# timflannagan/deppy

Hardware: AMD Instinct MI355X
Metric: resolutions/sec (node) on synthetic catalogs at 1/2/4/8 GPUs; BCP HBM GB/s (higher is better)
Workload: dtype int32

## Files before the change

deppy_amd/_lib.py:

```python
from __future__ import annotations

import ctypes
import os

import numpy as np

HERE = os.path.dirname(os.path.abspath(__file__))
LIB_PATH = os.path.join(HERE, "libdeppy_hip.so")
def _hsa_up() -> bool:
    try:
        fds = os.listdir("/proc/self/fd")
    except OSError:
        return False
    for fd in fds:
        try:
            if os.readlink("/proc/self/fd/" + fd) == "/dev/kfd":
                return True
        except OSError:
            pass
    return False


def hw_queue_plan(env_value, hsa_up: bool, keep: bool = False):
    try:
        q = int(env_value) if env_value not in (None, "") else 4
    except ValueError:
        q = 4
    if hsa_up or keep or q >= 8:
        return None, q
    return "8", 8


def _plan_hw_queues() -> None:
    up = _hsa_up()
    env = os.environ.get("GPU_MAX_HW_QUEUES")
    set_to, q = hw_queue_plan(env, up, os.environ.get("DEPPY_KEEP_HW_QUEUES") == "1")
    if set_to is not None:
        os.environ["GPU_MAX_HW_QUEUES"] = set_to
    elif up and q < 8:
        import warnings
        warnings.warn("deppy_amd: HIP was initialised before the binding was imported, with %d hardware "
                      "queues; the pipeline runs %d lane streams per device (import deppy_amd first for 8)"
                      % (q, q), RuntimeWarning, stacklevel=3)
    os.environ["DEPPY_HW_QUEUES"] = "%d@%s" % (q, os.environ.get("GPU_MAX_HW_QUEUES", ""))


_plan_hw_queues()
OPT_FORCE_GROUP = 1 << 0
OPT_FORCE_HBM = 1 << 1
OPT_FORCE_MID = 1 << 2
OPT_TINY_TABLE = 1 << 3
OPT_FORCE_LDSG = 1 << 4
OPT_SHARE_ORDINAL = 1 << 5
F_TRACE_TRUNCATED = 1 << 8
if os.environ.get("DEPPY_STAMPS") == "1":
    LIB_PATH = os.path.join(HERE, os.environ.get("DEPPY_STAMPS_LIB", "libdeppy_hip_stamps.so"))
elif os.environ.get("DEPPY_VARIANT_LIB"):
    LIB_PATH = os.path.join(HERE, os.environ["DEPPY_VARIANT_LIB"])

c_i32p = ctypes.POINTER(ctypes.c_int32)
c_i64p = ctypes.POINTER(ctypes.c_int64)
c_u32p = ctypes.POINTER(ctypes.c_uint32)
c_i8p = ctypes.POINTER(ctypes.c_int8)

EXPORTS = [
    "dp_rec_validate", "dp_lower", "dp_lowered_free", "dp_lowered_num_problems",
    "dp_lowered_rec_off", "dp_lowered_rec", "dp_lowered_ident_off", "dp_lowered_ident_var",
    "dp_lowered_ident_con", "dp_lowered_error", "dp_result_layout", "dp_create", "dp_destroy",
    "dp_last_error", "dp_last_global_error", "dp_num_devices", "dp_lanes", "dp_solve", "dp_upload", "dp_run",
    "dp_launch", "dp_wait", "dp_download", "dp_resident_free", "dp_last_kernel_ms", "dp_gen_catalogs", "dp_gen_wire",
    "dp_gen_free", "dp_upload_traced", "dp_download_trace", "dp_solve_traced", "dp_lowered_errors",
    "dp_device_bytes", "dp_lower_into", "dp_lowered_new", "dp_lowered_exact_count", "dp_lowered_pinned", "dp_rec_widen", "dp_submit", "dp_job_wait", "dp_get_stats", "dp_stage_roundtrip",
    "dp_stitch_selftest", "dp_partition", "dp_build_info", "dp_get_device_stats", "dp_plan_placements",
    "dp_plan_order", "dp_dlower_new", "dp_dlower_free", "dp_lower_device", "dp_dlower_host_count",
    "dp_host_alloc", "dp_host_free",
]


class Wire(ctypes.Structure):
    _fields_ = [
        ("n_problems", ctypes.c_int32),
        ("prob_var_off", c_i64p),
        ("var_id", c_i64p),
        ("var_con_off", c_i64p),
        ("con_kind", c_i32p),
        ("con_n", c_i32p),
        ("con_arg_off", c_i64p),
        ("con_arg", c_i64p),
        ("n_strs", ctypes.c_int64),
        ("str_off", c_i64p),
        ("str_bytes", ctypes.c_char_p),
        ("interned", ctypes.c_int32),
    ]


class Wire32(ctypes.Structure):
    _fields_ = [
        ("n_problems", ctypes.c_int32),
        ("prob_var_off", c_i32p),
        ("prob_con_off", c_i32p),
        ("prob_arg_off", c_i32p),
        ("var_id", c_i32p),
        ("var_ncon", ctypes.POINTER(ctypes.c_uint16)),
        ("con_kn", c_i32p),
        ("con_nargs", ctypes.POINTER(ctypes.c_uint16)),
        ("con_arg", c_i32p),
        ("var_id16", ctypes.POINTER(ctypes.c_uint16)),
        ("con_arg16", ctypes.POINTER(ctypes.c_uint16)),
        ("n_strs", ctypes.c_int64),
        ("str_off", c_i64p),
        ("str_bytes", ctypes.c_char_p),
    ]


class Opts(ctypes.Structure):
    _fields_ = [("first_device", ctypes.c_int32), ("n_devices", ctypes.c_int32),
                ("step_budget", ctypes.c_int64), ("flags", ctypes.c_int32)]


class Stats(ctypes.Structure):
    _fields_ = [("problems", ctypes.c_int64), ("chunks", ctypes.c_int64), ("launches", ctypes.c_int64),
                ("kernel_ms", ctypes.c_double), ("h2d_bytes", ctypes.c_int64), ("d2h_bytes", ctypes.c_int64),
                ("rec_bytes", ctypes.c_int64), ("stage_ms", ctypes.c_double), ("plan_ms", ctypes.c_double), ("wait_ms", ctypes.c_double),
                ("scatter_ms", ctypes.c_double), ("direct_chunks", ctypes.c_int64),
                ("bcp_bytes", ctypes.c_int64), ("allocs", ctypes.c_int64),
                ("placed", ctypes.c_int64 * 5), ("placed_launches", ctypes.c_int64 * 5)]

PLACES = ["lds", "split", "hbm", "split4", "ldsg"]


def _stats_dict(st) -> dict:
    d = {}
    for k, _ in Stats._fields_:
        v = getattr(st, k)
        d[k] = {PLACES[m]: int(v[m]) for m in range(5)} if k.startswith("placed") else v
    return d


class Batch(ctypes.Structure):
    _fields_ = [("n_problems", ctypes.c_int32), ("rec_off", c_i64p), ("rec", c_i32p)]


class Result(ctypes.Structure):
    _fields_ = [("status", c_i8p), ("flags", c_i32p), ("installed", c_u32p),
                ("inst_off", c_i64p), ("core", c_i32p), ("core_off", c_i64p),
                ("core_len", c_i32p), ("steps", c_i64p)]


_lib = None


def build_info(L=None) -> str:
    L = L or lib()
    if not hasattr(L, "dp_build_info"):
        return ""
    L.dp_build_info.restype = ctypes.c_char_p
# ... 12 lines not shown
    got = build_info(L)
    if ("sources=%s " % want) not in got + " ":
        raise RuntimeError("deppy_amd: %s was built from other sources (%s; this tree: sources=%s); run "
                           "__graft_entry__.build() (python -m deppy_amd.build)" % (LIB_PATH, got or "no build info", want))


def lib():
    global _lib
    if _lib is not None:
        return _lib
    if not os.path.exists(LIB_PATH):
        raise RuntimeError("deppy_amd: %s is missing; run __graft_entry__.build() "
                           "(python deppy_amd/build.py)" % LIB_PATH)
    L = ctypes.CDLL(LIB_PATH)
    _check_provenance(L)
    vp = ctypes.c_void_p
    L.dp_rec_validate.argtypes = [c_i32p, ctypes.c_int64]
    L.dp_rec_widen.argtypes = [c_i32p, ctypes.c_int64, c_i32p]
    L.dp_lower.argtypes = [ctypes.POINTER(Wire), ctypes.POINTER(vp)]
    L.dp_lowered_free.argtypes = [vp]
    L.dp_lower_into.argtypes = [ctypes.POINTER(Wire), ctypes.c_int32, vp]
    L.dp_lowered_new.restype = vp
    L.dp_lowered_exact_count.argtypes = [vp]
    L.dp_lowered_exact_count.restype = ctypes.c_int64
    L.dp_lowered_pinned.argtypes = [vp]
    L.dp_lowered_pinned.restype = ctypes.c_int32
    L.dp_lowered_num_problems.argtypes = [vp]
    for f in ("dp_lowered_rec_off", "dp_lowered_ident_off"):
        getattr(L, f).argtypes = [vp]
        getattr(L, f).restype = c_i64p
    for f in ("dp_lowered_rec", "dp_lowered_ident_var", "dp_lowered_ident_con"):
        getattr(L, f).argtypes = [vp]
        getattr(L, f).restype = c_i32p
    L.dp_lowered_error.argtypes = [vp, ctypes.c_int32, ctypes.POINTER(ctypes.c_char_p)]
    L.dp_lowered_errors.argtypes = [vp, c_i32p]
    L.dp_result_layout.argtypes = [ctypes.POINTER(Batch), c_i64p, c_i64p]
    L.dp_create.argtypes = [ctypes.POINTER(Opts)]
    L.dp_create.restype = vp
    L.dp_destroy.argtypes = [vp]
    L.dp_last_error.argtypes = [vp]
    L.dp_last_error.restype = ctypes.c_char_p
    L.dp_last_global_error.restype = ctypes.c_char_p
    L.dp_num_devices.argtypes = [vp]
    if hasattr(L, "dp_lanes"):
        L.dp_lanes.argtypes = [vp]
        L.dp_lanes.restype = ctypes.c_int32
    L.dp_solve.argtypes = [vp, ctypes.POINTER(Batch), ctypes.POINTER(Result)]
    L.dp_upload.argtypes = [vp, ctypes.POINTER(Batch), ctypes.POINTER(vp)]
    L.dp_upload_traced.argtypes = [vp, ctypes.POINTER(Batch), ctypes.c_int32, ctypes.POINTER(vp)]
    L.dp_download_trace.argtypes = [vp, vp, c_i32p, c_i32p]
    L.dp_solve_traced.argtypes = [vp, ctypes.POINTER(Batch), ctypes.c_int32, ctypes.POINTER(Result),
                                  c_i32p, c_i32p]
    L.dp_submit.argtypes = [vp, ctypes.POINTER(Batch), ctypes.POINTER(Result), ctypes.POINTER(vp)]
    L.dp_job_wait.argtypes = [vp, vp]
    L.dp_get_stats.argtypes = [vp, ctypes.POINTER(Stats), ctypes.c_int32]
    L.dp_get_device_stats.argtypes = [vp, ctypes.c_int32, ctypes.POINTER(Stats), ctypes.c_int32]
    L.dp_num_devices.restype = ctypes.c_int32
    L.dp_stage_roundtrip.argtypes = [ctypes.POINTER(Batch), ctypes.c_int32, ctypes.c_int32, ctypes.c_int64,
                                     c_i32p, c_i32p, ctypes.c_int32]
    L.dp_stitch_selftest.argtypes = [ctypes.POINTER(Batch), ctypes.c_int32, ctypes.POINTER(Result)]
    L.dp_partition.argtypes = [c_i64p, ctypes.c_int32, ctypes.c_int32, c_i32p]
    L.dp_run.argtypes = [vp, vp]
    L.dp_launch.argtypes = [vp, vp]
    L.dp_wait.argtypes = [vp, vp]
    L.dp_download.argtypes = [vp, vp, ctypes.POINTER(Result)]
    L.dp_resident_free.argtypes = [vp, vp]
    L.dp_last_kernel_ms.argtypes = [vp, ctypes.POINTER(ctypes.c_double)]
    L.dp_gen_catalogs.argtypes = [ctypes.c_int32, ctypes.c_int32, ctypes.c_uint64]
    L.dp_gen_catalogs.restype = vp
    L.dp_gen_wire.argtypes = [vp]
    L.dp_gen_wire.restype = ctypes.POINTER(Wire)
    L.dp_gen_free.argtypes = [vp]
    L.dp_device_bytes.argtypes = [ctypes.POINTER(Batch), ctypes.c_int32, c_i64p, c_i64p]
    L.dp_dlower_new.argtypes = [vp]
    L.dp_dlower_new.restype = vp
    L.dp_dlower_free.argtypes = [vp]
    L.dp_lower_device.argtypes = [vp, ctypes.POINTER(Wire32), ctypes.c_int32, vp]
    L.dp_dlower_host_count.argtypes = [vp]
    L.dp_dlower_host_count.restype = ctypes.c_int64
    L.dp_host_alloc.argtypes = [ctypes.c_int64]
    L.dp_host_alloc.restype = vp
    L.dp_host_free.argtypes = [vp]
    L.dp_plan_placements.argtypes = [ctypes.POINTER(Batch), ctypes.c_int32, c_i8p]
    L.dp_plan_order.argtypes = [ctypes.POINTER(Batch), ctypes.c_int32, c_i32p, c_i32p]
    _lib = L
    return L


def _p(a, t):
    return a.ctypes.data_as(t)


class WireArrays:

    def __init__(self, prob_var_off, var_id, var_con_off, con_kind, con_n, con_arg_off, con_arg,
                 str_off, str_bytes, interned=True):
        self.a = dict(prob_var_off=np.ascontiguousarray(prob_var_off, np.int64),
                      var_id=np.ascontiguousarray(var_id, np.int64),
                      var_con_off=np.ascontiguousarray(var_con_off, np.int64),
                      con_kind=np.ascontiguousarray(con_kind, np.int32),
                      con_n=np.ascontiguousarray(con_n, np.int32),
                      con_arg_off=np.ascontiguousarray(con_arg_off, np.int64),
                      con_arg=np.ascontiguousarray(con_arg, np.int64),
                      str_off=np.ascontiguousarray(str_off, np.int64),
                      str_bytes=np.frombuffer(bytes(str_bytes) + b"\0", np.uint8))
        self.interned = interned

    @property
    def n_problems(self) -> int:
        return len(self.a["prob_var_off"]) - 1

    def slice(self, p0: int, p1: int) -> "WireArrays":
        w = WireArrays.__new__(WireArrays)
        w.a = dict(self.a)
        w.a["prob_var_off"] = self.a["prob_var_off"][p0:p1 + 1]
        w.interned = self.interned
        return w

    def struct(self) -> Wire:
        a = self.a
        for k in ("var_id", "con_kind", "con_n", "con_arg"):
            if len(a[k]) == 0:
                a[k] = np.zeros(1, a[k].dtype)
        w = Wire()
        w.n_problems = len(a["prob_var_off"]) - 1
        w.prob_var_off = _p(a["prob_var_off"], c_i64p)
        w.var_id = _p(a["var_id"], c_i64p)
        w.var_con_off = _p(a["var_con_off"], c_i64p)
        w.con_kind = _p(a["con_kind"], c_i32p)
        w.con_n = _p(a["con_n"], c_i32p)
        w.con_arg_off = _p(a["con_arg_off"], c_i64p)
        w.con_arg = _p(a["con_arg"], c_i64p)
        w.n_strs = len(a["str_off"]) - 1
        w.str_off = _p(a["str_off"], c_i64p)
        w.str_bytes = ctypes.cast(a["str_bytes"].ctypes.data, ctypes.c_char_p)
        w.interned = 1 if self.interned else 0
        return w


def wire_to_numpy(w: Wire) -> dict:
    P = w.n_problems
    pvo = np.ctypeslib.as_array(w.prob_var_off, (P + 1,)).copy()
    nv = int(pvo[-1])
    vco = np.ctypeslib.as_array(w.var_con_off, (nv + 1,)).copy() if nv else np.zeros(1, np.int64)
    nc = int(vco[-1])
    cao = np.ctypeslib.as_array(w.con_arg_off, (nc + 1,)).copy() if nc else np.zeros(1, np.int64)
    na = int(cao[-1])
    so = np.ctypeslib.as_array(w.str_off, (w.n_strs + 1,)).copy()
    sb = ctypes.string_at(w.str_bytes, int(so[-1]))
    return dict(prob_var_off=pvo,
                var_id=np.ctypeslib.as_array(w.var_id, (nv,)).copy() if nv else np.zeros(0, np.int64),
                var_con_off=vco,
                con_kind=np.ctypeslib.as_array(w.con_kind, (nc,)).copy() if nc else np.zeros(0, np.int32),
                con_n=np.ctypeslib.as_array(w.con_n, (nc,)).copy() if nc else np.zeros(0, np.int32),
                con_arg_off=cao,
                con_arg=np.ctypeslib.as_array(w.con_arg, (na,)).copy() if na else np.zeros(0, np.int64),
                str_off=so, str_bytes=np.frombuffer(sb, np.uint8))


class _LoweredHandle:

    def __init__(self, h):
        self.h = h

    def __del__(self):
        try:
# ... 340 lines not shown
            raise RuntimeError("dp_job_wait: job already waited")
        rc = lib().dp_job_wait(self.ctx.h, h)
        self._batch_arrays = None
        if rc != 0:
            raise RuntimeError("dp_job_wait: " + self.ctx.error())
        out = dict(self.out)
        for k in ("status", "flags", "core_len", "steps"):
            out[k] = out[k][:self.n]
        return out


class Resident:

    def __init__(self, ctx: Context, rec_off, rec, trace_cap: int = 0):
        self.ctx = ctx
        self.trace_cap = trace_cap
        self.rec_off = np.ascontiguousarray(rec_off, np.int64)
        self.rec = np.ascontiguousarray(rec if len(rec) else np.zeros(1, np.int32), np.int32)
        n = len(self.rec_off) - 1
        self.n = n
        b = _batch(self.rec_off, self.rec)
        self.inst_off = np.zeros(n + 1, np.int64)
        self.core_off = np.zeros(n + 1, np.int64)
        lib().dp_result_layout(ctypes.byref(b), _p(self.inst_off, c_i64p), _p(self.core_off, c_i64p))
        h = ctypes.c_void_p()
        if lib().dp_upload_traced(ctx.h, ctypes.byref(b), trace_cap, ctypes.byref(h)) != 0:
            raise RuntimeError("dp_upload: " + ctx.error())
        self.h = h

    def run(self):
        if lib().dp_run(self.ctx.h, self.h) != 0:
            raise RuntimeError("dp_run: " + self.ctx.error())

    def launch(self):
        if lib().dp_launch(self.ctx.h, self.h) != 0:
            raise RuntimeError("dp_launch: " + self.ctx.error())

    def wait(self):
        if lib().dp_wait(self.ctx.h, self.h) != 0:
            raise RuntimeError("dp_wait: " + self.ctx.error())

    def download(self) -> dict:
        n = self.n
        out = result_arrays(self.rec_off, self.rec)
        r = _result_struct(out)
        if lib().dp_download(self.ctx.h, self.h, ctypes.byref(r)) != 0:
            raise RuntimeError("dp_download: " + self.ctx.error())
        for k in ("status", "flags", "core_len", "steps"):
            out[k] = out[k][:n]
        return out

    def download_trace(self) -> dict:
        n = self.n
        tr = np.zeros((max(n, 1), max(self.trace_cap, 1)), np.int32)
        tl = np.zeros(max(n, 1), np.int32)
        if lib().dp_download_trace(self.ctx.h, self.h, _p(tr, c_i32p), _p(tl, c_i32p)) != 0:
            raise RuntimeError("dp_download_trace: " + self.ctx.error())
        return dict(trace=tr[:n], trace_len=tl[:n])

    def free(self):
        if self.h:
            lib().dp_resident_free(self.ctx.h, self.h)
            self.h = None


def device_bytes(rec_off, rec, flags: int = 0) -> tuple[int, int]:
    rec_off = np.ascontiguousarray(rec_off, np.int64)
    rec = np.ascontiguousarray(rec if len(rec) else np.zeros(1, np.int32), np.int32)
    rb, ib = ctypes.c_int64(), ctypes.c_int64()
    if lib().dp_device_bytes(ctypes.byref(_batch(rec_off, rec)), flags, ctypes.byref(rb), ctypes.byref(ib)) != 0:
        raise RuntimeError("dp_device_bytes failed")
    return rb.value, ib.value


def plan_placements(rec_off, rec, flags: int = 0) -> np.ndarray:
    rec_off = np.ascontiguousarray(rec_off, np.int64)
    rec = np.ascontiguousarray(rec if len(rec) else np.zeros(1, np.int32), np.int32)
    place = np.zeros(max(len(rec_off) - 1, 1), np.int8)
    if lib().dp_plan_placements(ctypes.byref(_batch(rec_off, rec)), flags, _p(place, c_i8p)) != 0:
        raise RuntimeError("dp_plan_placements failed")
    return place[:len(rec_off) - 1]


def plan_order(rec_off, rec, flags: int = 0):
    rec_off = np.ascontiguousarray(rec_off, np.int64)
    rec = np.ascontiguousarray(rec if len(rec) else np.zeros(1, np.int32), np.int32)
    order = np.zeros(max(len(rec_off) - 1, 1), np.int32)
    first = np.zeros(32, np.int32)
    nl = lib().dp_plan_order(ctypes.byref(_batch(rec_off, rec)), flags, _p(order, c_i32p), _p(first, c_i32p))
    if nl < 0:
        raise RuntimeError("dp_plan_order failed")
    return order, first[:nl]


def stage_roundtrip(rec_off, rec, flags: int = 0, chunk_problems: int = 0, chunk_bytes: int = 0):
    rec_off = np.ascontiguousarray(rec_off, np.int64)
    rec = np.ascontiguousarray(rec if len(rec) else np.zeros(1, np.int32), np.int32)
    out = np.zeros_like(rec)
    firsts = np.zeros(max(len(rec_off), 1), np.int32)
    k = lib().dp_stage_roundtrip(ctypes.byref(_batch(rec_off, rec)), flags, chunk_problems, chunk_bytes,
                                 _p(out, c_i32p), _p(firsts, c_i32p), len(firsts))
    if k < 0:
        raise ValueError("dp_stage_roundtrip: malformed record")
    return out, firsts[:k]


def stitch_selftest(rec_off, rec, chunk_problems: int) -> dict:
    rec_off = np.ascontiguousarray(rec_off, np.int64)
    rec = np.ascontiguousarray(rec, np.int32)
    out = result_arrays(rec_off, rec)
    out["installed"][:] = 0xdeadbeef
    r = _result_struct(out)
    if lib().dp_stitch_selftest(ctypes.byref(_batch(rec_off, rec)), chunk_problems, ctypes.byref(r)) < 0:
        raise ValueError("dp_stitch_selftest failed")
    return out


def partition(rec_off, nd: int) -> np.ndarray:
    rec_off = np.ascontiguousarray(rec_off, np.int64)
    cut = np.zeros(nd + 1, np.int32)
    if lib().dp_partition(_p(rec_off, c_i64p), len(rec_off) - 1, nd, _p(cut, c_i32p)) != 0:
        raise ValueError("dp_partition failed")
    return cut


def generate(config: int, n: int, seed: int) -> dict:
    L = lib()
    g = L.dp_gen_catalogs(config, n, seed)
    if not g:
        raise ValueError(L.dp_last_global_error().decode())
    try:
        return wire_to_numpy(L.dp_gen_wire(g).contents)
    finally:
        L.dp_gen_free(g)


def trace_events(res: dict, p: int) -> list:
    t = res["trace"][p][:int(res["trace_len"][p])]
    ev, i = [], 0
    while i < len(t):
        n = int(t[i])
        vs = [int(x) for x in t[i + 1:i + 1 + n]]
        i += 1 + n
        m = int(t[i])
        ev.append((vs, [int(x) for x in t[i + 1:i + 1 + m]]))
        i += 1 + m
    return ev


def installed_list(res: dict, p: int, nv: int) -> list[int]:
    base = int(res["inst_off"][p])
    words = res["installed"][base:base + (nv + 31) // 32]
    bits = np.unpackbits(words.view(np.uint8), bitorder="little")[:nv]
    return [int(i) for i in np.flatnonzero(bits)]


def core_list(res: dict, p: int) -> list[int]:
    base = int(res["core_off"][p])
    return [int(x) for x in res["core"][base:base + int(res["core_len"][p])]]
```

deppy_amd/csrc/kernel_api.hpp:

```cpp
#pragma once
#include <hip/hip_runtime.h>

#include <cstdint>

namespace dp {

constexpr int DP_NSTAMP = 56;

struct alignas(32) ProblemOut {
  int8_t status;
  int8_t pad[3];
  int32_t flags;
  int32_t core_len;
  int32_t core_at;
  int64_t steps;
  uint64_t bcp;
};
static_assert(sizeof(ProblemOut) == 32, "two 16-byte stores");

struct alignas(16) WorkItem {
  int64_t rec_off;
  int32_t inst_off;
  int32_t pid;
};
static_assert(sizeof(WorkItem) == 16, "one 16-byte read");

struct KernelArgs {
  const int32_t* rec;
  const WorkItem* items;
  ProblemOut* out;
  uint32_t* installed;
  int32_t* core;
  int32_t* core_pool_len;
  int64_t budget;
  int32_t* scratch;
  const int64_t* scratch_off;
  int64_t* stamps;
  int32_t* trace;
  int32_t* trace_len;
  int32_t trace_cap;
  int32_t* queue;
  int32_t n_items;
  int32_t table_cap;
  int32_t grid_cap;
};
constexpr int kQueueWords = 64;

hipError_t launch_solve(const KernelArgs& a, int mode, int n_blocks, int lds_bytes, hipStream_t stream);
hipError_t launch_watch_build(const KernelArgs& a, int mode, int n_items, hipStream_t stream);
hipError_t configure_solve_kernel(int max_lds_bytes);

}
```

deppy_amd/csrc/layout.hpp:

```cpp
#pragma once
#include <hip/hip_runtime.h>

#include <cstdint>
#include <type_traits>

#include "../../include/deppy_hip.h"

namespace dp {

__host__ __device__ inline int32_t bits_words(int32_t n) { return (n + 31) >> 5; }

constexpr int32_t L_MAX = 64;

enum Mode { M_LDS = 0, M_SPLIT = 1, M_HBM = 2, M_SPLIT4 = 3, M_LDSG = 4 };
static_assert((int)M_LDS == DP_PLACE_LDS && (int)M_SPLIT == DP_PLACE_SPLIT && (int)M_HBM == DP_PLACE_HBM &&
                  (int)M_SPLIT4 == DP_PLACE_SPLIT4 && (int)M_LDSG == DP_PLACE_LDSG,
              "enum dp_place (include/deppy_hip.h) names the placements");
__host__ __device__ constexpr bool mode_n16(int mode) { return mode == M_LDS || mode == M_LDSG; }
#ifndef DP_BIG_WAVES
#define DP_BIG_WAVES 8
#endif
constexpr int32_t BIG_WAVES = DP_BIG_WAVES;

#ifndef DP_MID_WAVES
#define DP_MID_WAVES 4
#endif
constexpr int32_t MID_WAVES = DP_MID_WAVES;
#ifndef DP_LDSG_WAVES
#define DP_LDSG_WAVES 4
#endif
constexpr int32_t LDSG_WAVES = DP_LDSG_WAVES;
__host__ __device__ constexpr int32_t mode_waves(int mode) {
  return mode == M_LDS ? 1 : mode == M_SPLIT4 ? MID_WAVES : mode == M_LDSG ? LDSG_WAVES : BIG_WAVES;
}
__host__ __device__ constexpr int32_t mode_wbuf(int mode) {
  return mode == M_LDS ? 128 : mode == M_LDSG ? 1024 : 4096;
}
__host__ __device__ constexpr int32_t mode_cq(int mode) { return mode == M_LDS ? 64 : mode == M_LDSG ? 256 : 512; }

constexpr int32_t NSCAL = 64;
__host__ __device__ constexpr int32_t mode_nscal(int mode) {
#ifdef DP_STAMPS
  return (mode == M_LDS ? 8 : NSCAL) + 64;
#else
  return mode == M_LDS ? 8 : NSCAL;
#endif
}

__host__ __device__ inline bool fmt_derived(int32_t fmt) { return fmt == DP_FMT_P16D || fmt == DP_FMT_P8D; }
__host__ __device__ inline bool fmt_packed(int32_t fmt) { return fmt == DP_FMT_P16 || fmt_derived(fmt); }
__host__ __device__ inline int64_t p16_tail_at(const int32_t* h) {
  const int64_t ch = fmt_derived(h[DP_H_FMT]) ? 0 : h[DP_H_NCHL];
  return (2 * ((int64_t)h[DP_H_NCL] + h[DP_H_NKL] + h[DP_H_NK] + ch + h[DP_H_NA]) + 15) & ~(int64_t)15;
}
__host__ __device__ inline int64_t p16_tail_bytes(const int32_t* h) {
  const int64_t vc = fmt_derived(h[DP_H_FMT]) ? 0 : (int64_t)h[DP_H_NV];
  return (int64_t)h[DP_H_NC] + h[DP_H_NK] + h[DP_H_NCH] + vc + ((int64_t)h[DP_H_NID] + 7) / 8;
}
__host__ __device__ inline int32_t p8_bytes(const int32_t* h) { return (int32_t)((uint32_t)h[DP_H_P8] >> 8); }
__host__ __device__ inline int32_t id_mask_words16(const int32_t* h) {
  return 3 * bits_words(h[DP_H_NID]) + 2;
}
__host__ __device__ inline int32_t lds_body_words(const int32_t* h) {
  int32_t b = h[DP_H_WORDS] - DP_H_SIZE;
  if (fmt_packed(h[DP_H_FMT])) b += id_mask_words16(h) - h[DP_H_NC] - h[DP_H_NK];
  return fmt_derived(h[DP_H_FMT]) ? b - 1 - h[DP_H_NCHL] : b;
}
__host__ __device__ inline int32_t p16_tail_copy(const int32_t* h) {
  return (2 * lds_body_words(h) + 15) & ~15;
}
__host__ __device__ inline int32_t p8_tail(const int32_t* h) {
  return p16_tail_copy(h) + ((p8_bytes(h) + 15) & ~15);
}

__host__ __device__ inline dp_rec_layout rec_layout(const int32_t* h) {
  dp_rec_layout L;
  int32_t o = DP_H_SIZE;
  L.clause_off = o;     o += h[DP_H_NC] + 1;
  L.clause_lits = o;    o += h[DP_H_NCL];
  L.clause_id = o;      o += h[DP_H_NC];
  L.card_off = o;       o += h[DP_H_NK] + 1;
  L.card_lits = o;      o += h[DP_H_NKL];
  L.card_bound = o;     o += h[DP_H_NK];
  L.card_id = o;        o += h[DP_H_NK];
  L.var_choice_off = o; o += h[DP_H_NV] + 1;
  L.choice_off = o;     o += h[DP_H_NCH] + 1;
  L.choice_lits = o;    o += h[DP_H_NCHL];
  L.anchors = o;        o += h[DP_H_NA];
  L.words = o;
  return L;
}


enum { DP_FMT_REJECT = 2, DP_FMT_U16_CHECKED = 16, DP_FMT_I32_CHECKED = 17 };

constexpr int32_t DEV_WATCH_VARS = 2048;
__host__ __device__ inline bool device_watches(const int32_t* h) { return h[DP_H_NV] <= DEV_WATCH_VARS; }
static_assert(2 * DEV_WATCH_VARS + 1 <= mode_wbuf(M_SPLIT) + mode_cq(M_SPLIT) &&
                  2 * DEV_WATCH_VARS + 1 <= mode_wbuf(M_SPLIT4) + mode_cq(M_SPLIT4) &&
                  2 * DEV_WATCH_VARS + 1 <= mode_wbuf(M_HBM) + mode_cq(M_HBM) && mode_wbuf(M_SPLIT) % 4 == 0,
              "build_watches_wide: the counters fit wbuf + cardq");

constexpr uint32_t ROW_INFO_NONE = 0xffffffffu;
__host__ __device__ inline uint32_t row_info(int32_t a, int32_t len) {
  return a >= 0 && a < (1 << 24) && len >= 0 && len < 255 ? ((uint32_t)a << 8) | (uint32_t)len : ROW_INFO_NONE;
}

struct ImgLayout {
  int32_t w_off, w, words;
};

__host__ __device__ inline ImgLayout img_layout(const int32_t* h) {
  ImgLayout X;
  int32_t o = h[DP_H_WORDS];
  X.w_off = o; o += 2 * h[DP_H_NV] + 1;
  X.w = o;     o += h[DP_H_NCL] + h[DP_H_NKL];
  X.words = o;
  return X;
}

__host__ __device__ inline int64_t staged_words(const int32_t* h, bool narrow) {
  const int64_t body = (int64_t)h[DP_H_WORDS] - DP_H_SIZE;
  const int64_t w = narrow ? DP_H_SIZE + (body + 1) / 2 : (int64_t)img_layout(h).words;
  return (w + 3) & ~3LL;
}

struct Layout {
  int32_t body;
  int32_t val;
  int32_t reason;
  int32_t rs;
  int32_t trail;
  int32_t touched;
  int32_t d_mark;
  int32_t imp;
  int32_t d_flip;
  int32_t inS;
  int32_t extra;
  int32_t seen;
  int32_t model;
  int32_t dset;
  int32_t fg;
  int32_t used;
  int32_t en;
  int32_t en2;
  int32_t crit;
  int32_t idt;
  int32_t l_off;
  int32_t l_lits;
  int32_t dq;
  int32_t stk;
  int32_t wbuf;
  int32_t cardq;
  int32_t scal;
  int32_t hkey;
  int32_t hrp, hrn;
  int32_t tl;
  int32_t fr;
  int32_t hc;
  int32_t wl;
  int32_t bytes;
  int32_t lds_bytes;
  int32_t cap, lcap;
};

enum Scalar { S_NTOUCHED = 0, S_NWORK = 1, S_POSROWS = 2, S_APP = 3, S_NTB = 4, S_CVB = 6, S_OVB = 8, S_SLOT = 32 };

__host__ __device__ constexpr bool mode_lds_rounds(int mode) { return mode == M_SPLIT || mode == M_SPLIT4; }
__host__ __device__ inline int32_t round_slots(int32_t nv) {
  int32_t c = 64;
  while (c < 1024 && c < nv / 8) c <<= 1;
  return c;
}

template <int MODE>
__host__ __device__ inline Layout layout_hc(const int32_t* h, int32_t hc) {
  constexpr bool N16 = mode_n16(MODE);
  using IX = typename std::conditional<N16, uint16_t, int32_t>::type;
  Layout L;
  const int32_t nv = h[DP_H_NV], nid = h[DP_H_NID];
  const int32_t nbv = bits_words(nv), nbi = bits_words(nid);
  const int32_t ix = (int32_t)sizeof(IX);
  int32_t og = 0, ol = 0;
  auto take = [&](int32_t nbytes, int kind) {
    const bool lds = N16 || kind == 2 || (kind == 1 && (MODE == M_SPLIT || MODE == M_SPLIT4));
    int32_t& o = lds ? ol : og;
    const int32_t at = o;
    o += (nbytes + 15) & ~15;
    return at;
  };
  enum { COLD = 0, HOT = 1, WORK = 2 };
  L.cap = h[DP_H_NA] + h[DP_H_NCH] + 2;
  L.lcap = nv + 64;
  const ImgLayout X = img_layout(h);
  int32_t body_bytes = (X.words - DP_H_SIZE + 8) * ix;
  if (N16) body_bytes = (lds_body_words(h) + (X.words - h[DP_H_WORDS]) + 8) * ix;
  if (N16 && fmt_packed(h[DP_H_FMT])) {
    const int32_t tail = h[DP_H_FMT] == DP_FMT_P8D ? p8_tail(h) : p16_tail_copy(h);
    const int32_t need = tail + (int32_t)((p16_tail_bytes(h) + 15) & ~15);
    body_bytes = body_bytes > need ? body_bytes : need;
  }
  L.body = N16 ? take(body_bytes, COLD) : 0;
  L.scal = take(mode_nscal(MODE) * 4, WORK);
  L.wbuf = take(mode_wbuf(MODE) * ix, WORK);
  L.cardq = take(mode_cq(MODE) * ix * (N16 ? 1 : 2), WORK);
  L.hc = mode_lds_rounds(MODE) ? hc : 0;
  L.hkey = take(L.hc * 4, WORK);
  L.hrp = take(L.hc * 4, WORK);
  L.hrn = take(L.hc * 4, WORK);
  L.tl = take(L.hc * 4, WORK);
  L.fr = take(L.hc * 4, WORK);
  L.val = take(nv, HOT);
  L.d_flip = take(nbv * 4, HOT);
  L.inS = take(nbv * 4, HOT);
  L.extra = take(nbv * 4, HOT);
  L.seen = take(nbv * 4, HOT);
  L.model = take(nbv * 4, HOT);
  L.dset = take(nbv * 4, HOT);
  L.fg = take(nbv * 4, HOT);
  L.used = take(nbi * 4, HOT);
  L.en = take(nbi * 4, HOT);
  L.en2 = take(nbi * 4, HOT);
  L.crit = take(nbi * 4, HOT);
  L.idt = N16 ? take(nbi * 4, HOT) : 0;
  L.reason = take(nv * ix, COLD);
  L.rs = take(nv * ix, COLD);
  L.trail = take(nv * ix, COLD);
  L.touched = take(2 * nv * ix, COLD);
  L.d_mark = take(nv * ix, COLD);
  L.imp = take(2 * nv * (N16 ? 2 : 4), COLD);
  L.l_off = take((L_MAX + 1) * ix, COLD);
  L.l_lits = take(L.lcap * ix, COLD);
  L.dq = take(2 * L.cap * ix, COLD);
  L.stk = take(3 * L.cap * ix, COLD);
  L.wl = !N16 && h[DP_H_FMT] == DP_FMT_I32 ? take((2 * nv + 2) * 4 + (h[DP_H_NCL] + h[DP_H_NKL]) * 8, COLD) : 0;
  L.bytes = og;
  L.lds_bytes = ol;
  return L;
}

constexpr int32_t kLdsLimitBytes = 160 * 1024;
template <int MODE>
__host__ __device__ inline Layout layout(const int32_t* h) {
  if (!mode_lds_rounds(MODE)) return layout_hc<MODE>(h, 0);
  int32_t hc = round_slots(h[DP_H_NV]);
  Layout L = layout_hc<MODE>(h, hc);
  while (hc > 64 && L.lds_bytes > kLdsLimitBytes) L = layout_hc<MODE>(h, hc >>= 1);
  return L;
}

inline bool fits16(const int32_t* h) { return dp_rec_fits16(h) != 0; }

}
```

deppy_amd/csrc/lower_device.hip:

```cpp
#include <hip/hip_runtime.h>

#include <algorithm>
#include <chrono>
#include <cstdio>
#include <cstdlib>
#include <cstring>
#include <mutex>
#include <string>
#include <vector>

#include "common.hpp"
#include "dlower.hpp"
#include "hostmem.hpp"
#include "layout.hpp"
#include "placement.hpp"
#include "pool.hpp"

namespace {

constexpr int DL_NV = 512;
constexpr int DL_C = 512;
constexpr int DL_A = 1536;
constexpr int DL_VH = 1024;
constexpr int DL_KH = 1024;
// ... 354 lines not shown
    const int crow = nc + __popcll(__ballot(isc) & lt_mask());
    const int cat = ncl + excl_scan(isc ? rlen : 0, tot);
    nc += __popcll(__ballot(isc));
    ncl += tot;
    const int krow = nk + __popcll(__ballot(isk) & lt_mask());
    const int kat = nkl + excl_scan(isk ? rlen : 0, tot);
    nk += __popcll(__ballot(isk));
    nkl += tot;
    const bool isl = act && m_list(m);
    const int k = nch + __popcll(__ballot(isl) & lt_mask());
    if (isl) S.clist[c] = (int16_t)k;
    nch += __popcll(__ballot(isl));
    (void)excl_scan(isl ? ns : 0, tot);
    nchl += tot;
    __syncthreads();
    bool far = false;
    if (isl) {
      const int d = isf || s < 0 ? 0 : k - S.clist[first];
      far = d > 255;
      S.src[k] = (uint8_t)d;
    }
    if (__ballot(far) && lane == 0) S.p16 = 1;
    if (isc) {
      S.clen[crow] = (uint8_t)rlen;
      if (kind == DP_DEPENDENCY && ns > 0) {
        S.clit[cat] = (int16_t)(2 * vi + 1);
        for (int j = 0, o = 1; j < ns; ++j) {
          const int d = S.ca[a0 + j];
          bool rep = false;
          for (int q = 0; q < j && !rep; ++q) rep = S.ca[a0 + q] == d;
          if (!rep) S.clit[cat + o++] = (int16_t)(2 * d);
        }
      } else if (rlen == 1) {
        const uint64_t key = S.kkey[s] - 1ull;
        S.clit[cat] = (int16_t)(2 * (int)(key & 0x3fffffffULL) + ((key >> 60) == K_NEG ? 1 : 0));
      } else if (rlen == 2) {
        S.clit[cat] = (int16_t)(2 * vi + 1);
        S.clit[cat + 1] = (int16_t)(2 * S.ca[a0] + 1);
      }
    }
    bool kb1 = true;
    if (isk) {
      const int n = a.ckn[cb + c] >> 3;
      S.klen[krow] = (uint8_t)rlen;
      S.kb[krow] = (int16_t)n;
      kb1 = n == 1;
      for (int j = 0; j < ns; ++j) S.kv[kat + j] = S.ca[a0 + j];
      atomicOr(&S.mask[id >> 5], 1u << (id & 31));
    }
    b1 = b1 && __ballot(!kb1) == 0;
    nib = nib && __ballot((isc || isk) && rlen > 15) == 0;
    if (isf) {
      const int last = S.klast[s];
      const int ov = S.cs[last];
      a.ivs[(int64_t)p * DL_C + id] = ov;
      a.ics[(int64_t)p * DL_C + id] = last - S.vstart[ov];
    }
  }
  __syncthreads();
  if (S.fb) return give_up();
  int na = 0;
  for (int i0 = 0; i0 < nv; i0 += DL_T) {
    const int i = i0 + lane;
    const bool f = i < nv && ((S.aflag[i >> 5] >> (i & 31)) & 1u);
    const uint64_t bm = __ballot(f);
    if (f) S.av[na + __popcll(bm & lt_mask())] = (int16_t)i;
    na += __popcll(bm);
  }

  int32_t h[DP_H_SIZE];
#pragma unroll
  for (int i = 0; i < DP_H_SIZE; ++i) h[i] = 0;
  h[DP_H_MAGIC] = DP_REC_MAGIC;
  h[DP_H_NV] = nv;
  h[DP_H_NC] = nc;
  h[DP_H_NK] = nk;
  h[DP_H_NCH] = nch;
  h[DP_H_NA] = na;
  h[DP_H_NID] = nid;
  h[DP_H_NCL] = ncl;
  h[DP_H_NKL] = nkl;
  h[DP_H_NCHL] = nchl;
  h[DP_H_WORDS] = DP_H_SIZE + (nc + 1) + ncl + nc + (nk + 1) + nkl + 2 * nk + (nv + 1) + (nch + 1) + nchl + na;
  if (!fits16_dev(h) || (int64_t)dp::layout<dp::M_LDS>(h).lds_bytes > a.group_above) return give_up();
  auto put_header = [&]() {
    for (int i = lane; i < DL_SLOT; i += DL_T) S.rec[i] = 0u;
    __syncthreads();
    if (lane < DP_H_SIZE) {
      int32_t x = 0;
#pragma unroll
      for (int i = 0; i < DP_H_SIZE; ++i)
        if (i == lane) x = h[i];
      S.rec[lane] = (uint32_t)x;
    }
  };
  auto put_out = [&](int padded) {
    __syncthreads();
    int32_t* out = a.slots + (int64_t)p * DL_SLOT;
    for (int i = lane; i < padded; i += DL_T) out[i] = (int32_t)S.rec[i];
    if (lane == 0) {
      a.words[p] = padded;
      a.nid[p] = nid;
    }
  };
  if (S.p16) {
    bool bad16 = false;
    for (int i = lane; i < nv; i += DL_T) {
      int cnt = 0;
      for (int c = S.vstart[i]; c < S.vstart[i + 1]; ++c) cnt += m_list(S.cmeta[c]) ? 1 : 0;
      bad16 = bad16 || cnt > 255;
      S.vcl[i] = (uint8_t)cnt;
    }
    const int tb = nc + nk + nv + nch + (nid + 7) / 8;
    const int at = (2 * (ncl + nkl + nk + nchl + na) + 15) & ~15;
    const int phys = DP_H_SIZE + (at + tb + 3) / 4, padded = (phys + 3) & ~3;
    if (__ballot(bad16) || tb > DP_P16_TAIL_MAX || padded > DL_SLOT) return give_up();
    h[DP_H_FMT] = DP_FMT_P16;
    put_header();
    uint16_t* const u = reinterpret_cast<uint16_t*>(S.rec + DP_H_SIZE);
    uint8_t* const t = reinterpret_cast<uint8_t*>(S.rec + DP_H_SIZE) + at;
    for (int j = lane; j < ncl; j += DL_T) u[j] = (uint16_t)S.clit[j];
    for (int j = lane; j < nkl; j += DL_T) u[ncl + j] = (uint16_t)S.kv[j];
    for (int j = lane; j < nk; j += DL_T) u[ncl + nkl + j] = (uint16_t)S.kb[j];
    int run = 0;
    for (int c0 = 0; c0 < C; c0 += DL_T) {
      const int c = c0 + lane;
      const bool isl = c < C && m_list(S.cmeta[c]);
      const int ns = isl ? S.castart[c + 1] - S.castart[c] : 0;
      int tot;
      const int ex = excl_scan(ns, tot);
      if (isl) {
        for (int j = 0; j < ns; ++j) u[ncl + nkl + nk + run + ex + j] = (uint16_t)S.ca[S.castart[c] + j];
        t[nc + nk + nv + S.clist[c]] = (uint8_t)ns;
      }
      run += tot;
    }
    for (int j = lane; j < na; j += DL_T) u[ncl + nkl + nk + nchl + j] = (uint16_t)S.av[j];
    for (int i = lane; i < nc; i += DL_T) t[i] = S.clen[i];
    for (int i = lane; i < nk; i += DL_T) t[nc + i] = S.klen[i];
    for (int i = lane; i < nv; i += DL_T) t[nc + nk + i] = S.vcl[i];
    for (int b = lane; b < ((nid + 7) >> 3); b += DL_T)
      t[nc + nk + nv + nch + b] = (uint8_t)(S.mask[b >> 2] >> ((b & 3) * 8));
    put_out(padded);
    return;
  }
  if ((int64_t)nc + nk + nch + (nid + 7) / 8 > DP_P16_TAIL_MAX) return give_up();
  const int f = (nv > 256 ? DP_P8_HI : 0) | (b1 ? DP_P8_B1 : 0) | (nib ? DP_P8_NIB : 0);
  const bool hi = f & DP_P8_HI;
  int o = 0;
  const int L_cvar = o; o += ncl;
  const int L_kvar = o; o += nkl;
  const int L_avar = o; o += na;
  const int L_bound = o; o += b1 ? 0 : nk;
  const int L_neg = o; o += (ncl + 7) >> 3;
  const int L_chi = o; o += hi ? (ncl + 7) >> 3 : 0;
  const int L_khi = o; o += hi ? (nkl + 7) >> 3 : 0;
  const int L_ahi = o; o += hi ? (na + 7) >> 3 : 0;
  const int rows = nc + nk;
  const int L_lens = o; o += nib ? (rows + 1) / 2 : rows;
  const int L_srcnz = o; o += (nch + 7) >> 3;
  const int L_srcval = o;
  int nnz = 0;
  for (int k0 = 0; k0 < nch; k0 += DL_T) nnz += __popcll(__ballot(k0 + lane < nch && S.src[k0 + lane] != 0));
  const int L_mask = L_srcval + nnz;
  const int bytes = L_mask + ((nid + 7) >> 3);
  const int phys = DP_H_SIZE + (bytes + 3) / 4, padded = (phys + 3) & ~3;
  if (padded > DL_SLOT) return give_up();
// ... 517 lines not shown
```

deppy_amd/csrc/placement.hpp:

```cpp
#pragma once
#include <algorithm>
#include <cstdint>
#include <cstdlib>
#include <vector>

#include "layout.hpp"

namespace dp {

constexpr int kMaxLdsBytes = kLdsLimitBytes;

constexpr int64_t kGroupAbove = 64 << 10;

inline int64_t group_above() {
  static const int64_t v = [] {
    const char* e = std::getenv("DEPPY_GROUP_ABOVE");
    const int64_t x = e && *e ? std::atoll(e) : 0;
    return x > 0 ? std::min<int64_t>(x, kMaxLdsBytes) : kGroupAbove;
  }();
  return v;
}

inline bool one_wave(const int32_t* h) {
  return fits16(h) && (int64_t)layout<M_LDS>(h).lds_bytes <= group_above();
}

constexpr int32_t kLdsgMaxProblems = 256;
enum { LDSG_NEVER = 0, LDSG_ALWAYS = 1, LDSG_AUTO = 2 };
inline int ldsg_env() {
  const char* e = std::getenv("DEPPY_LDSG");
  return e && *e == '0' ? LDSG_NEVER : e && *e == '1' ? LDSG_ALWAYS : LDSG_AUTO;
}
inline bool ldsg_fits(const int32_t* h) { return fits16(h) && (int64_t)layout<M_LDSG>(h).lds_bytes <= kMaxLdsBytes; }
inline bool lds_image(const int32_t* h, int ldsg) { return one_wave(h) || (ldsg == LDSG_ALWAYS && ldsg_fits(h)); }

inline int64_t build_watches_host(int32_t* r) {
  const dp_rec_layout R = dp_rec_layout_of(r);
  const ImgLayout X = img_layout(r);
  const int32_t nv = r[DP_H_NV], nc = r[DP_H_NC], nk = r[DP_H_NK];
  const int32_t* clause_off = r + R.clause_off;
  const int32_t* clause_lits = r + R.clause_lits;
  const int32_t* card_off = r + R.card_off;
  const int32_t* card_lits = r + R.card_lits;
  int32_t* wo = r + X.w_off;
  int32_t* w = r + X.w;
  std::fill(wo, wo + 2 * (int64_t)nv + 1, 0);
  for (int32_t j = 0; j < r[DP_H_NCL]; ++j) wo[(clause_lits[j] ^ 1) + 1]++;
  for (int32_t k = 0; k < nk; ++k)
    for (int32_t j = card_off[k]; j < card_off[k + 1]; ++j)
      if (j == card_off[k] || card_lits[j] != card_lits[j - 1]) wo[2 * card_lits[j] + 1]++;
  for (int64_t l = 0; l < 2 * (int64_t)nv; ++l) wo[l + 1] += wo[l];
  static thread_local std::vector<int32_t> cur;
  cur.assign(wo, wo + 2 * (int64_t)nv);
  for (int32_t rr = 0; rr < nc; ++rr)
    for (int32_t j = clause_off[rr]; j < clause_off[rr + 1]; ++j) w[cur[(size_t)(clause_lits[j] ^ 1)]++] = rr;
  for (int32_t k = 0; k < nk; ++k)
    for (int32_t j = card_off[k]; j < card_off[k + 1]; ++j)
      if (j == card_off[k] || card_lits[j] != card_lits[j - 1]) w[cur[(size_t)(2 * card_lits[j])]++] = nc + k;
  return X.words;
}

}
```

deppy_amd/csrc/runtime.cpp:

```cpp
#include <hip/hip_runtime.h>

#include <algorithm>
#include <atomic>
#include <chrono>
#include <climits>
#include <condition_variable>
#include <deque>
#include <cstdlib>
#include <cstring>
#include <fstream>
#include <functional>
#include <mutex>
#include <string>
#include <thread>
#include <vector>

#include "common.hpp"
#include "dlower.hpp"
#include "kernel_api.hpp"
#include "layout.hpp"
#include "hostmem.hpp"
#include "placement.hpp"
#include "pool.hpp"

namespace {

using dp::kMaxLdsBytes;
constexpr int64_t kDefaultBudget = 1 << 16;
constexpr int kNBuckets = 16;
struct Ceilings {
  int c[kNBuckets];
  int n;
};
const Ceilings& ceilings() {
  static const Ceilings t = [] {
    Ceilings x{};
    const char* e = std::getenv("DEPPY_CEILINGS");
    if (!e || std::strcmp(e, "fine") != 0) {
      const int coarse[] = {16 << 10, 32 << 10, 53 << 10, 80 << 10, 160 << 10};
      x.n = 5;
      for (int i = 0; i < 5; ++i) x.c[i] = coarse[i];
    } else {
      x.n = kNBuckets;
      for (int k = kNBuckets; k >= 1; --k) x.c[kNBuckets - k] = (160 * 1024 / k) / 512 * 512;
      x.c[kNBuckets - 1] = 160 * 1024;
    }
    return x;
  }();
  return t;
}
constexpr int kXcds = 8;
constexpr int kStreams = 4;
constexpr int kMaxStreams = 16;
constexpr int kMaxLanes = 2 * kMaxStreams;
constexpr double kMergeRatio = 0.5;
constexpr int32_t kMinLaunch = 512;
constexpr int32_t kMidMaxVars = 8192;
constexpr int32_t kChunkProblems = 65536;
constexpr int64_t kChunkBytes = 1ll << 30;
constexpr int32_t kChunksPerDevice = 3;
constexpr int kCostClasses = 16;
constexpr int32_t kMinSharedChunk = 4096;
constexpr int64_t kCoreWordsPerProblem = 8;

double now_ms() {
  return std::chrono::duration<double, std::milli>(std::chrono::steady_clock::now().time_since_epoch()).count();
}

int64_t env_i64(const char* name, int64_t dflt) {
  const char* e = std::getenv(name);
  return e && *e ? std::atoll(e) : dflt;
}

bool forced_of(int32_t opt_flags) {
  return opt_flags & (DP_OPT_FORCE_GROUP | DP_OPT_FORCE_HBM | DP_OPT_FORCE_MID | DP_OPT_FORCE_LDSG);
}

bool header_ok(const int32_t* h, int64_t avail) {
  if (avail < DP_H_SIZE || h[DP_H_MAGIC] != DP_REC_MAGIC) return false;
  for (int i = DP_H_NV; i <= DP_H_NCHL; ++i)
    if (h[i] < 0 || h[i] > (1 << 28)) return false;
  const int32_t fmt = h[DP_H_FMT];
  if (fmt != DP_FMT_I32 && fmt != DP_FMT_I32W && ((fmt != DP_FMT_U16 && !dp_fmt_packed(fmt)) || !dp_rec_fits16(h)))
    return false;
  if (dp_fmt_packed(fmt) && dp_p16_tail_bytes(h) > DP_P16_TAIL_MAX) return false;
  const int64_t w = dp_rec_layout_of(h).words;
  return w == h[DP_H_WORDS] && dp_rec_phys_words(h) <= avail;
}

}

namespace dp {

struct Launch {
  int first, count, mode, lds;
  bool dev_lists;
};

struct Head {
  int8_t place;
  bool ldsg_ok;
  int8_t bucket;
  bool direct;
  int32_t lds, inst_words, nid;
  int64_t sw, rec_bytes;
  uint8_t cls;
};

constexpr int32_t kPlanBlock = 512;
constexpr int32_t kPlanPoolMin = 32768;
struct PlanBlock {
  int64_t img = 0, inst = 0, core = 0, rbytes = 0, other = 0;
  int32_t ndirect = 0, nother = 0, nok = 0;
  int32_t bcount[kNBuckets] = {}, bmax[kNBuckets] = {};
};

struct Plan {
  int32_t n = 0;
  int32_t n_ldsg = 0;
  std::vector<int64_t> img_off;
  std::vector<uint8_t> narrow;
  std::vector<int32_t> order;
  std::vector<Launch> launches;
  int big_base = 0;
  std::vector<int64_t> scratch_off;
  int64_t scratch_words = 0;
  std::vector<int32_t> skip;
  std::vector<int32_t> skip_flags;
  std::vector<int64_t> inst_off;
  int64_t core_cap = 0;
  int64_t rec_bytes = 0;
  std::vector<int64_t> dev_off;
  int64_t img_words = 0;
  std::vector<uint8_t> direct;
  int32_t n_direct = 0;
  int64_t other_words = 0;
  std::vector<Head> head;
  std::vector<PlanBlock> blk;
  std::vector<int32_t> segcnt;
  std::vector<int64_t> segpos, segxs;
  std::vector<int32_t> big[5], cnt, tmp, grp;
};

void place_ldsg(Head& H, const int32_t* h, bool aligned) {
  H.lds = layout<M_LDSG>(h).lds_bytes;
  H.sw = staged_words(h, true);
  H.rec_bytes = dp_fmt_packed(h[DP_H_FMT]) ? 4 * dp_rec_phys_words(h)
                                           : 4 * DP_H_SIZE + 2 * ((int64_t)h[DP_H_WORDS] - DP_H_SIZE);
  H.place = M_LDSG;
  H.direct = aligned && (h[DP_H_FMT] == DP_FMT_U16 || dp_fmt_packed(h[DP_H_FMT]));
}

void read_head(Head& H, const int32_t* h, int64_t avail, int32_t opt_flags, bool aligned) {
  H = Head{};
  if (!header_ok(h, avail)) { H.place = -1; return; }
  H.inst_words = bits_words(h[DP_H_NV]);
  H.nid = h[DP_H_NID];
  H.cls = (uint8_t)std::min<int32_t>(h[DP_H_NA], kCostClasses - 1);
  bool nar = false;
  if (dp::fits16(h)) {
    if (!forced_of(opt_flags)) {
      H.lds = layout<M_LDS>(h).lds_bytes;
      nar = H.lds <= dp::group_above();
    }
    if (!nar && (!forced_of(opt_flags) || (opt_flags & DP_OPT_FORCE_LDSG)) && dp::ldsg_fits(h)) {
      if (opt_flags & DP_OPT_FORCE_LDSG) {
        place_ldsg(H, h, aligned);
        return;
      }
      H.ldsg_ok = true;
    }
  }
  H.sw = staged_words(h, nar);
  H.rec_bytes = nar ? (dp_fmt_packed(h[DP_H_FMT]) ? 4 * dp_rec_phys_words(h)
                                                 : 4 * DP_H_SIZE + 2 * ((int64_t)h[DP_H_WORDS] - DP_H_SIZE))
                    : 4 * (int64_t)h[DP_H_WORDS];
  if (nar) {
    H.place = M_LDS;
    int k = 0;
    const Ceilings& C = ceilings();
    while (k < C.n - 1 && H.lds > C.c[k]) ++k;
    H.bucket = (int8_t)k;
    H.direct = aligned && (h[DP_H_FMT] == DP_FMT_U16 || dp_fmt_packed(h[DP_H_FMT]));
    return;
  }
  H.direct = aligned && (h[DP_H_FMT] == DP_FMT_I32W || h[DP_H_FMT] == DP_FMT_I32);
  const bool forced = forced_of(opt_flags);
  const bool sized = h[DP_H_NV] < (1 << 24) && h[DP_H_NID] < (1 << 26) && h[DP_H_WORDS] < (1 << 28);
  if (sized && layout<M_SPLIT>(h).lds_bytes <= kMaxLdsBytes && !(opt_flags & DP_OPT_FORCE_HBM))
    H.place = (opt_flags & DP_OPT_FORCE_MID) || (!forced && h[DP_H_NV] < kMidMaxVars) ? M_SPLIT4 : M_SPLIT;
  else if (sized && layout<M_HBM>(h).lds_bytes <= kMaxLdsBytes)
    H.place = M_HBM;
  else
    H.place = -2;
}

void plan_chunk(Plan& P, const int32_t* rec, const int64_t* rec_off, int32_t p0, int32_t n,
                int32_t opt_flags, std::vector<uint8_t>* bad, Pool* pool = nullptr, int32_t ldsg_busy = 0) {
  P.n = n;
  P.n_ldsg = 0;
  P.img_off.resize((size_t)n + 1);
  P.inst_off.resize((size_t)n + 1);
  P.narrow.resize((size_t)n);
  P.direct.resize((size_t)n);
  P.head.resize((size_t)n);
  P.order.clear();
  P.launches.clear();
  P.scratch_off.clear();
  P.skip.clear();
  P.skip_flags.clear();
  P.scratch_words = P.core_cap = P.rec_bytes = P.other_words = 0;
  P.n_direct = 0;
  P.big_base = 0;
  Head* head = P.head.data();
  const int32_t nblk = (n + kPlanBlock - 1) / kPlanBlock;
  P.blk.resize((size_t)std::max(nblk, 1));
  auto over_blocks_if = [&](bool par, const std::function<void(int64_t)>& fn) {
    if (pool && nblk > 1 && par) pool->run(nblk, fn, 1);
    else for (int32_t b = 0; b < nblk; ++b) fn(b);
  };
  const bool wide = n >= kPlanPoolMin;
  auto over_blocks = [&](const std::function<void(int64_t)>& fn) { over_blocks_if(wide, fn); };
  over_blocks_if(n > 256, [&](int64_t b) {
    const int32_t i0 = (int32_t)b * kPlanBlock, i1 = std::min(n, i0 + kPlanBlock);
    int32_t nok = 0;
    for (int32_t i = i0; i < i1; ++i) {
      if (i + 8 < i1) {
        const int32_t* h8 = rec + rec_off[p0 + i + 8];
        __builtin_prefetch(h8);
        __builtin_prefetch(h8 + 15);
      }
      read_head(head[i], rec + rec_off[p0 + i], rec_off[p0 + i + 1] - rec_off[p0 + i], opt_flags,
                (rec_off[p0 + i] & 3) == 0);
      nok += head[i].ldsg_ok;
    }
    P.blk[(size_t)b].nok = nok;
  });
  {
    const int lm = dp::ldsg_env();
    int32_t n_ok = 0;
    for (int32_t b = 0; b < nblk; ++b) n_ok += P.blk[(size_t)b].nok;
    if (n_ok > 0 && (lm == dp::LDSG_ALWAYS || (lm == dp::LDSG_AUTO && n_ok + ldsg_busy <= dp::kLdsgMaxProblems))) {
      for (int32_t i = 0; i < n; ++i)
        if (head[i].ldsg_ok) place_ldsg(head[i], rec + rec_off[p0 + i], (rec_off[p0 + i] & 3) == 0);
      P.n_ldsg = n_ok;
    }
  }
  const bool rec_aligned = ((uintptr_t)rec & 15) == 0;
  over_blocks([&](int64_t b) {
    PlanBlock& B = P.blk[(size_t)b];
    const int32_t nok = B.nok;
    B = PlanBlock{};
    B.nok = nok;
    const int32_t i0 = (int32_t)b * kPlanBlock, i1 = std::min(n, i0 + kPlanBlock);
    for (int32_t i = i0; i < i1; ++i) {
      const Head& H = head[i];
      const bool d = rec_aligned && H.direct;
      B.ndirect += d;
      B.other += d ? 0 : rec_off[p0 + i + 1] - rec_off[p0 + i];
      if (H.place == M_LDS) {
        B.bcount[H.bucket]++;
        B.bmax[H.bucket] = std::max(B.bmax[H.bucket], H.lds);
      } else {
        B.nother++;
      }
      if (H.place != -1) {
        B.img += H.sw;
        B.inst += H.inst_words;
        B.core += H.nid;
        B.rbytes += H.rec_bytes;
      }
    }
  });
  for (auto& v : P.big) v.clear();
  int32_t bcount[kNBuckets] = {}, bmax[kNBuckets] = {};
  int64_t img = 0, inst = 0;
  bool others = false;
  for (int32_t b = 0; b < nblk; ++b) {
    PlanBlock& B = P.blk[(size_t)b];
    const int64_t bi = B.img, bn = B.inst;
    B.img = img;
    B.inst = inst;
    img += bi;
    inst += bn;
    P.n_direct += B.ndirect;
    P.other_words += B.other;
    P.core_cap += B.core;
    P.rec_bytes += B.rbytes;
    others |= B.nother > 0;
    for (int k = 0; k < kNBuckets; ++k) {
      bcount[k] += B.bcount[k];
      bmax[k] = std::max(bmax[k], B.bmax[k]);
    }
  }
  P.dev_off.resize((size_t)n);
  P.img_off[0] = P.inst_off[0] = 0;
  over_blocks([&](int64_t b) {
    const PlanBlock& B = P.blk[(size_t)b];
    int64_t im = B.img, in = B.inst;
    const int32_t i0 = (int32_t)b * kPlanBlock, i1 = std::min(n, i0 + kPlanBlock);
    for (int32_t i = i0; i < i1; ++i) {
      const Head& H = head[i];
      P.direct[(size_t)i] = rec_aligned && H.direct;
      P.narrow[(size_t)i] = H.place == M_LDS || H.place == M_LDSG;
      P.dev_off[(size_t)i] = im;
      if (H.place != -1) {
        im += H.sw;
        in += H.inst_words;
      }
      P.img_off[(size_t)i + 1] = im;
      P.inst_off[(size_t)i + 1] = in;
    }
  });
  if (others)
    for (int32_t i = 0; i < n; ++i) {
      const Head& H = head[i];
      if (H.place == M_LDS) continue;
      if (H.place >= 0) {
        P.big[(size_t)H.place].push_back(i);
      } else {
        if (H.place == -1 && bad) (*bad)[(size_t)i] = 1;
        P.skip.push_back(i);
        P.skip_flags.push_back(H.place == -1 ? DP_F_MALFORMED : DP_F_TOO_LARGE);
      }
    }
  P.img_words = img;
  auto cost = [&](int32_t i) { return P.img_off[(size_t)i + 1] - P.img_off[(size_t)i]; };
  auto lpt = [&](int32_t* v, size_t m) {
    if (m < 2) return;
    int64_t lo = INT64_MAX, hi = 0;
    for (size_t j = 0; j < m; ++j) { lo = std::min(lo, cost(v[j])); hi = std::max(hi, cost(v[j])); }
    if (hi - lo > 4 * (int64_t)m + 65536) {
      std::stable_sort(v, v + m, [&](int32_t x, int32_t y) { return cost(x) > cost(y); });
      return;
    }
    P.cnt.assign((size_t)(hi - lo) + 2, 0);
    for (size_t j = 0; j < m; ++j) P.cnt[(size_t)(hi - cost(v[j])) + 1]++;
    for (size_t k = 1; k < P.cnt.size(); ++k) P.cnt[k] += P.cnt[k - 1];
    P.tmp.resize(m);
    for (size_t j = 0; j < m; ++j) P.tmp[(size_t)P.cnt[(size_t)(hi - cost(v[j]))]++] = v[j];
    std::copy(P.tmp.begin(), P.tmp.begin() + (int64_t)m, v);
  };
  for (int mode : {(int)M_LDSG, (int)M_SPLIT4, (int)M_SPLIT, (int)M_HBM}) {
    auto& bg = P.big[(size_t)mode];
    if (bg.empty()) continue;
    lpt(bg.data(), bg.size());
    int mx = 0;
    Launch L{(int)P.order.size(), (int)bg.size(), mode, 0, false};
    for (int32_t i : bg) {
      const int32_t* h = rec + rec_off[p0 + i];
      L.dev_lists |= h[DP_H_FMT] == DP_FMT_I32 && !dp::device_watches(h);
      const Layout Y = mode == M_SPLIT    ? layout<M_SPLIT>(h)
                       : mode == M_SPLIT4 ? layout<M_SPLIT4>(h)
                       : mode == M_LDSG   ? layout<M_LDSG>(h)
                                          : layout<M_HBM>(h);
      mx = std::max(mx, Y.lds_bytes);
      if (P.scratch_words == 0) P.scratch_words = dp::kQueueWords;
      P.scratch_off.push_back(P.scratch_words);
      P.scratch_words += ((int64_t)Y.bytes + 15) / 16 * 4;
    }
    L.lds = mx;
    P.launches.push_back(L);
    P.order.insert(P.order.end(), bg.begin(), bg.end());
  }
  P.big_base = 0;
  static const double merge = [] {
    const char* m = std::getenv("DEPPY_BUCKET_MERGE");
    return m ? std::atof(m) : kMergeRatio;
  }();
  int group_of[kNBuckets];
  Launch bl[kNBuckets];
  int64_t gsize[kNBuckets] = {};
  int ng = 0;
  for (int k = kNBuckets - 1; k >= 0; --k) {
    if (!bcount[k]) continue;
    const bool join = ng > 0 && (bcount[k] < kMinLaunch ||
                                 (merge > 0 && (double)(kMaxLdsBytes / bl[ng - 1].lds) >=
                                                   merge * (double)(kMaxLdsBytes / bmax[k])));
    if (!join) bl[ng++] = Launch{0, 0, M_LDS, bmax[k]};
    group_of[k] = ng - 1;
    gsize[ng - 1] += bcount[k];
  }
  int ix[kNBuckets];
  for (int g = 0; g < ng; ++g) ix[g] = g;
  std::stable_sort(ix, ix + ng, [&](int x, int y) { return gsize[x] > gsize[y]; });
  int64_t o = (int64_t)P.order.size();
  for (int r = 0; r < ng; ++r) {
    const int g = ix[r];
    bl[g].first = (int)o;
    bl[g].count = (int)gsize[g];
    o += gsize[g];
  }
  P.order.resize((size_t)o);
  static const int64_t xcd_order = env_i64("DEPPY_XCD_ORDER", kMaxLdsBytes);
  static const bool anchor_order = env_i64("DEPPY_ANCHOR_ORDER", 1) != 0;
  if (ng > 0) {
    int rank_of[kNBuckets];
    bool xo[kNBuckets];
    for (int r = 0; r < ng; ++r) {
      rank_of[ix[r]] = r;
      xo[ix[r]] = xcd_order && bl[ix[r]].lds <= xcd_order;
    }
    const int nseg = ng * kCostClasses;
    auto seg_of = [&](const Head& H) {
      const int g = group_of[H.bucket];
      const int c = anchor_order && xo[g] ? H.cls : 0;
      return rank_of[g] * kCostClasses + (kCostClasses - 1 - c);
    };
    P.segcnt.assign((size_t)nblk * nseg, 0);
    over_blocks([&](int64_t b) {
      int32_t* c = P.segcnt.data() + (size_t)b * nseg;
      const int32_t i0 = (int32_t)b * kPlanBlock, i1 = std::min(n, i0 + kPlanBlock);
      for (int32_t i = i0; i < i1; ++i)
        if (head[i].place == M_LDS) c[seg_of(head[i])]++;
    });
    P.segpos.resize((size_t)nseg + 1);
    int64_t run = bl[ix[0]].first;
    for (int sg = 0; sg < nseg; ++sg) {
      P.segpos[(size_t)sg] = run;
      for (int32_t b = 0; b < nblk; ++b) {
        int32_t& c = P.segcnt[(size_t)b * nseg + sg];
        const int32_t x = c;
        c = (int32_t)run;
        run += x;
      }
    }
    P.segpos[(size_t)nseg] = run;
    P.tmp.resize((size_t)o);
    over_blocks([&](int64_t b) {
      int32_t* c = P.segcnt.data() + (size_t)b * nseg;
      const int32_t i0 = (int32_t)b * kPlanBlock, i1 = std::min(n, i0 + kPlanBlock);
      for (int32_t i = i0; i < i1; ++i)
        if (head[i].place == M_LDS) P.tmp[(size_t)c[seg_of(head[i])]++] = i;
    });
    P.segxs.resize((size_t)nseg * kXcds);
    auto first_on = [&](int sg, int64_t pos, int x) {
      const int64_t rel = pos - bl[ix[sg / kCostClasses]].first;
      return pos + ((x - rel % kXcds) % kXcds + kXcds) % kXcds;
    };
    for (int sg = 0; sg < nseg; ++sg) {
      const int64_t pos = P.segpos[(size_t)sg], end = P.segpos[(size_t)sg + 1];
      int64_t st = pos;
      for (int x = 0; x < kXcds; ++x) {
        P.segxs[(size_t)sg * kXcds + x] = st;
        const int64_t first = first_on(sg, pos, x);
        st += first < end ? (end - 1 - first) / kXcds + 1 : 0;
      }
    }
    const int64_t o0 = bl[ix[0]].first, nslot = o - o0;
    const int32_t sblk = (int32_t)((nslot + kPlanBlock - 1) / kPlanBlock);
    auto deal = [&](int64_t b) {
      const int64_t s0 = o0 + b * kPlanBlock, s1 = std::min<int64_t>(o, s0 + kPlanBlock);
      int sg = (int)(std::upper_bound(P.segpos.begin(), P.segpos.end(), s0) - P.segpos.begin()) - 1;
      for (int64_t t = s0; t < s1; ++t) {
        while (P.segpos[(size_t)sg + 1] <= t) ++sg;
        const int g = ix[sg / kCostClasses];
        if (!xo[g]) {
          P.order[(size_t)t] = P.tmp[(size_t)t];
          continue;
        }
        const int x = (int)((t - bl[g].first) % kXcds);
        const int64_t first = first_on(sg, P.segpos[(size_t)sg], x);
        P.order[(size_t)t] = P.tmp[(size_t)(P.segxs[(size_t)sg * kXcds + x] + (t - first) / kXcds)];
      }
    };
    if (pool && sblk > 1 && wide) pool->run(sblk, std::function<void(int64_t)>(deal), 1);
    else for (int32_t b = 0; b < sblk; ++b) deal(b);
    for (int r = 0; r < ng; ++r) {
      const int g = ix[r];
      if (!xo[g]) lpt(P.order.data() + bl[g].first, (size_t)bl[g].count);
      P.launches.push_back(bl[g]);
    }
  }
  static const int pad_kb = (int)env_i64("DEPPY_LDS_PAD_KB", 0);
  if (pad_kb > 0)
    for (auto& L : P.launches)
// ... 284 lines not shown
  return a;
}

std::atomic<int64_t> g_buf_allocs{0};

struct Buf {
  char* p = nullptr;
  size_t cap = 0;
  bool host = false;
  hipError_t reserve(size_t n) {
    if (n <= cap) return hipSuccess;
    release();
    n = std::max<size_t>(al(n + n / 8), 4096);
    hipError_t e = host ? hipHostMalloc(reinterpret_cast<void**>(&p), n,
                                        hipHostMallocPortable | hipHostMallocMapped | hipHostMallocCoherent)
                        : hipMalloc(reinterpret_cast<void**>(&p), n);
    if (e != hipSuccess) { p = nullptr; cap = 0; return e; }
    g_buf_allocs.fetch_add(1, std::memory_order_relaxed);
    dev = p;
    if (host && hipHostGetDevicePointer(reinterpret_cast<void**>(&dev), p, 0) != hipSuccess) dev = p;
    cap = n;
    return hipSuccess;
  }
  char* dev = nullptr;
  void release() {
    if (p) (void)(host ? hipHostFree(p) : hipFree(p));
    p = nullptr;
    cap = 0;
  }
};

}

struct dp_job;

constexpr int kMaxSpread = 4;
struct Spread {
  hipStream_t s[kMaxSpread] = {};
  int n = 0;
  hipEvent_t start = nullptr, fin[kMaxSpread] = {};
  int create() {
    if (hipEventCreateWithFlags(&start, hipEventDisableTiming) != hipSuccess) return -1;
    for (auto& e : fin)
      if (hipEventCreateWithFlags(&e, hipEventDisableTiming) != hipSuccess) return -1;
    return 0;
  }
  void destroy() {
    if (start) (void)hipEventDestroy(start);
    for (auto& e : fin)
      if (e) (void)hipEventDestroy(e);
    start = nullptr;
    for (auto& e : fin) e = nullptr;
  }
};

struct Lane {
  int device = 0;
  hipStream_t s = nullptr;
  hipEvent_t k0 = nullptr, k1 = nullptr, done = nullptr;
  hipStream_t cs = nullptr;
  hipEvent_t copied = nullptr;
  Spread spread;
  Buf h_in{nullptr, 0, true}, d_in, h_out{nullptr, 0, true}, d_out, scratch;
  bool zc_out = false;
  dp_job* job = nullptr;
  int32_t p0 = 0;
  dp_job* fjob = nullptr;
  bool scattering = false;
  Plan plan;
  OutLayout ol{};
  std::vector<uint8_t> bad;
};

struct Task {
  dp_job* job;
  int32_t p0, n;
};

struct FastLane {
  std::mutex mu;
  hipStream_t s = nullptr;
  hipEvent_t done = nullptr;
  Buf h_in{nullptr, 0, true}, h_out{nullptr, 0, true};
  Plan plan;
  std::vector<uint8_t> bad;
};
constexpr int32_t kFastProblems = 16;
constexpr int64_t kFastWords = 1 << 16;

struct Device {
  int ordinal = 0;
  Lane lanes[kMaxLanes];
  int nstreams = kStreams, nlanes = 2 * kStreams;
  hipEvent_t last_copied = nullptr;
  int fill_left = 0;
  int next = 0;
  FastLane fast;
  std::thread worker;
  std::mutex qmu;
  std::condition_variable qcv;
  std::deque<Task> q;
  bool stop = false;
  int cursor = 0;
  std::deque<Lane*> inflight;
  dp::Pool* pool = nullptr;
  bool own_pool = false;
  std::thread finisher;
  std::mutex fmu;
  std::condition_variable fcv;
  std::deque<Lane*> fq;
  bool fstop = false;
  dp::Pool* fpool = nullptr;
  std::mutex smu;
  dp_stats st{};
};

struct dp_job {
  int32_t n = 0;
  const int32_t* rec = nullptr;
  const int64_t* rec_off = nullptr;
  bool pinned = false;
  dp_result res{};
  std::mutex m;
  std::condition_variable cv;
  int chunks_left = 0;
  std::atomic<bool> waiting{false};
  int rc = 0;
  std::string err;
};

struct dp_ctx {
  std::deque<Device> dev;
  int64_t budget = kDefaultBudget;
  int32_t flags = 0;
  std::string err;
  std::atomic<double> last_ms{0.0};
  std::mutex mu;
  dp::Pool* pool = nullptr;
  mutable std::mutex err_mu;
  int next_dev = 0;
  bool zc_in = false, zc_out = true;
  bool copy_streams = false;
  bool direct = true;
  int32_t chunk_problems = kChunkProblems;
  int64_t chunk_bytes = kChunkBytes;
  int32_t min_shared_chunk = kMinSharedChunk;
  int32_t grid_cap = 0;
  bool fast_path = true;
  bool spread = false;
  std::mutex sqmu;
  std::deque<Task> sq;
  dp_stats st{};
  ~dp_ctx() { delete pool; }
};

struct Slice {
  int d = 0;
  int ordinal = 0;
  int32_t p0 = 0, p1 = 0;
  Plan plan;
  InLayout il{};
  OutLayout ol{};
  Buf d_in, d_out, scratch;
  int32_t* trace = nullptr;
  int32_t* trace_len = nullptr;
  int64_t* stamps = nullptr;
  hipStream_t stream = nullptr;
  hipEvent_t k0 = nullptr, k1 = nullptr;
  Spread spread;
};

struct dp_resident {
  int32_t n = 0;
  int32_t trace_cap = 0;
  bool inflight = false;
  std::vector<Slice> slices;
};

namespace {

thread_local std::string t_err;
#define HIP_OK(expr)                                                         \
  do {                                                                       \
    hipError_t e_ = (expr);                                                  \
    if (e_ != hipSuccess) {                                                  \
      (void)ctx;                                                             \
      t_err = std::string(#expr) + ": " + hipGetErrorString(e_);             \
      return -1;                                                             \
    }                                                                        \
  } while (0)
void set_err(dp_ctx* ctx, std::string e) {
  std::lock_guard<std::mutex> lk(ctx->err_mu);
  ctx->err = std::move(e);
}
int api_fail(dp_ctx* ctx) {
  set_err(ctx, t_err);
  return -1;
}
#define API_OK(expr)                                                         \
  do {                                                                       \
    if (hipError_t e_ = (expr); e_ != hipSuccess) {                          \
      set_err(ctx, std::string(#expr) + ": " + hipGetErrorString(e_));       \
      return -1;                                                             \
    }                                                                        \
  } while (0)

void add_stats(dp_stats& a, const dp_stats& b) {
  a.problems += b.problems; a.chunks += b.chunks; a.launches += b.launches; a.kernel_ms += b.kernel_ms;
  a.h2d_bytes += b.h2d_bytes; a.d2h_bytes += b.d2h_bytes; a.rec_bytes += b.rec_bytes; a.stage_ms += b.stage_ms;
  a.plan_ms += b.plan_ms; a.wait_ms += b.wait_ms; a.scatter_ms += b.scatter_ms; a.direct_chunks += b.direct_chunks;
  a.bcp_bytes += b.bcp_bytes; a.allocs += b.allocs;
  for (int m = 0; m < 5; ++m) {
    a.placed[m] += b.placed[m];
    a.placed_launches[m] += b.placed_launches[m];
  }
}
void add_device_stats(Device& D, const dp_stats& b) {
  std::lock_guard<std::mutex> lk(D.smu);
  add_stats(D.st, b);
}

int enqueue_launches(dp_ctx* ctx, const Plan& P, const dp::KernelArgs& base, hipStream_t s, dp_stats& st,
                     Spread* sp = nullptr) {
  static const bool no_queue = [] {
    const char* e = std::getenv("DEPPY_NO_QUEUE");
    return e && *e && *e != '0';
  }();
  if (!P.scratch_off.empty()) HIP_OK(hipMemsetAsync(base.scratch, 0, 4 * dp::kQueueWords, s));
  int nlds = 0;
  for (const auto& L : P.launches) nlds += L.mode == dp::M_LDS;
  const bool spread = sp && sp->n > 0 && nlds > 1;
  if (spread) HIP_OK(hipEventRecord(sp->start, s));
  int q = 0, jl = 0, nf = 0;
  for (const auto& L : P.launches) {
    hipStream_t t = s;
    if (spread && L.mode == dp::M_LDS && jl++ > 0 && nf < kMaxSpread) {
      t = sp->s[(jl - 2) % sp->n];
      HIP_OK(hipStreamWaitEvent(t, sp->start, 0));
    }
    dp::KernelArgs a = base;
    a.items = base.items + L.first;
    if (L.mode != dp::M_LDS) {
      a.scratch_off = base.scratch_off + (L.first - P.big_base);
      a.queue = no_queue ? nullptr : base.scratch + q;
      a.n_items = L.count;
      if (ctx->flags & DP_OPT_TINY_TABLE) a.table_cap = 4;
      a.grid_cap = ctx->grid_cap;
      ++q;
      if (L.dev_lists) HIP_OK(dp::launch_watch_build(a, L.mode, L.count, s));
    }
    HIP_OK(dp::launch_solve(a, L.mode, L.count, L.lds, t));
    if (t != s) {
      HIP_OK(hipEventRecord(sp->fin[nf], t));
      HIP_OK(hipStreamWaitEvent(s, sp->fin[nf], 0));
      ++nf;
    }
    st.launches++;
    st.placed[L.mode] += L.count;
    st.placed_launches[L.mode]++;
  }
  return 0;
}

void set_siblings(const Device& D, int i, Spread& sp, bool on) {
  sp.n = 0;
  if (!on) return;
  for (int j = 1; j < D.nstreams && sp.n < kMaxSpread; ++j) sp.s[sp.n++] = D.lanes[(i + j) % D.nstreams].s;
}

int finish_lane(dp_ctx* ctx, Device& D, Lane& L) {
  if (!L.job) return 0;
  dp_job* job = L.job;
  L.job = nullptr;
  dp_stats st{};
  HIP_OK(hipSetDevice(L.device));
  const double t0 = now_ms();
  HIP_OK(hipEventSynchronize(L.done));
  const double t1 = now_ms();
  st.wait_ms += t1 - t0;
  float ms = 0.f;
  if (!L.plan.launches.empty() && hipEventElapsedTime(&ms, L.k0, L.k1) == hipSuccess) {
    st.kernel_ms += ms;
    ctx->last_ms.store(ms);
  }
  const int32_t used = L.zc_out ? 0 : *at<int32_t>(L.h_out.p, L.ol.pool_len);
  const size_t need = L.ol.pool + (size_t)used * 4;
  if (!L.zc_out && need > L.ol.d2h) {
    HIP_OK(hipMemcpyAsync(L.h_out.p + L.ol.d2h, L.d_out.p + L.ol.d2h, need - L.ol.d2h, hipMemcpyDeviceToHost, L.s));
    HIP_OK(hipStreamSynchronize(L.s));
    st.d2h_bytes += (int64_t)(need - L.ol.d2h);
  }
  add_device_stats(D, st);
  {
    std::lock_guard<std::mutex> lk(D.fmu);
    L.fjob = job;
    L.scattering = true;
    D.fq.push_back(&L);
  }
  D.fcv.notify_all();
  return 0;
}

void chunk_done(dp_job* job, int rc);

void wait_scatter(Device& D, Lane& L) {
  std::unique_lock<std::mutex> lk(D.fmu);
  D.fcv.wait(lk, [&] { return !L.scattering; });
}

void finisher_main(dp_ctx* ctx, Device* Dp) {
  Device& D = *Dp;
  std::unique_lock<std::mutex> lk(D.fmu);
  for (;;) {
    if (D.fq.empty()) {
      if (D.fstop) return;
      D.fcv.wait(lk);
      continue;
    }
    Lane* L = D.fq.front();
    D.fq.pop_front();
    lk.unlock();
    dp_stats st{};
    const double t0 = now_ms();
    dp_job* job = L->fjob;
    st.bcp_bytes += (int64_t)scatter(L->plan, L->ol, L->h_out.p, L->p0, &job->res, D.fpool);
    st.scatter_ms += now_ms() - t0;
    add_device_stats(D, st);
    lk.lock();
    L->scattering = false;
    L->fjob = nullptr;
    lk.unlock();
    D.fcv.notify_all();
    chunk_done(job, 0);
    lk.lock();
// ... 209 lines not shown
  bool failed;
  {
    std::lock_guard<std::mutex> lk(job->m);
    failed = job->rc != 0;
  }
  if (failed) {
    chunk_done(job, 0);
    return;
  }
  Lane& L = D.lanes[D.cursor];
  D.cursor = (D.cursor + 1) % D.nlanes;
  deliver(ctx, D, L);
  wait_scatter(D, L);
  if (start_chunk(ctx, D, L, job, t.p0, t.n)) {
    L.job = nullptr;
    chunk_done(job, -1);
    return;
  }
  D.inflight.push_back(&L);
}

bool take_shared(dp_ctx* ctx, Device& D, Task& t) {
  if ((int)D.inflight.size() >= D.nlanes) return false;
  std::lock_guard<std::mutex> g(ctx->sqmu);
  if (ctx->sq.empty()) return false;
  t = ctx->sq.front();
  ctx->sq.pop_front();
  return true;
}

void worker_main(dp_ctx* ctx, Device* Dp) {
  Device& D = *Dp;
  (void)hipSetDevice(D.ordinal);
  std::unique_lock<std::mutex> lk(D.qmu);
  for (;;) {
    Task t;
    if (!D.q.empty()) {
      t = D.q.front();
      D.q.pop_front();
      lk.unlock();
      run_task(ctx, D, t);
      lk.lock();
      continue;
    }
    if (take_shared(ctx, D, t)) {
      lk.unlock();
      run_task(ctx, D, t);
      lk.lock();
      continue;
    }
    if (!D.inflight.empty()) {
      Lane* o = D.inflight.front();
      const bool now = D.stop || o->job->waiting.load(std::memory_order_acquire) ||
                       hipEventQuery(o->done) != hipErrorNotReady;
      if (now) {
        lk.unlock();
        deliver(ctx, D, *o);
        lk.lock();
      } else {
        D.qcv.wait_for(lk, std::chrono::microseconds(50));
      }
      continue;
    }
    if (D.stop) {
      std::lock_guard<std::mutex> g(ctx->sqmu);
      if (ctx->sq.empty()) return;
      continue;
    }
    D.qcv.wait(lk);
  }
}

int fast_solve(dp_ctx* ctx, Device& D, const dp_batch* b, dp_result* res) {
  FastLane& F = D.fast;
  std::lock_guard<std::mutex> lk(F.mu);
  const int32_t n = b->n_problems;
  F.bad.assign((size_t)n, 0);
  dp::plan_chunk(F.plan, b->rec, b->rec_off, 0, n, ctx->flags, &F.bad, nullptr);
  const Plan& P = F.plan;
  if (!P.skip.empty() || !P.scratch_off.empty()) return 1;
  if (hipSetDevice(D.ordinal) != hipSuccess) return 1;
  const InLayout il = in_layout(P);
  const OutLayout ol = out_layout(P);
  if (F.h_in.reserve(il.end) != hipSuccess || F.h_out.reserve(ol.end) != hipSuccess) return 1;
  int32_t* img = at<int32_t>(F.h_in.p, il.img);
  for (int32_t i = 0; i < n; ++i)
    if (!dp::stage_one(P, b->rec, b->rec_off, 0, i, img, true)) F.bad[(size_t)i] = 1;
  fill_in_tables(P, il, F.h_in.p);
  *at<int32_t>(F.h_out.p, ol.pool_len) = 0;
  dp::KernelArgs a = kernel_args(il, ol, F.h_in.dev, F.h_out.dev, nullptr, ctx->budget);
  dp_stats st{};
  if (enqueue_launches(ctx, P, a, F.s, st) || hipEventRecord(F.done, F.s) != hipSuccess) return api_fail(ctx);
  hipError_t e;
  while ((e = hipEventQuery(F.done)) == hipErrorNotReady) __builtin_ia32_pause();
  if (e != hipSuccess) {
    set_err(ctx, std::string("dp_solve (latency path): ") + hipGetErrorString(e));
    return -1;
  }
  scatter(P, ol, F.h_out.p, 0, res);
  return 0;
}

void cut_chunks(const dp_ctx* ctx, const dp_job* job, std::vector<std::pair<int32_t, int32_t>>& out) {
  const int32_t P = job->n;
  const int nd = (int)ctx->dev.size();
  int32_t cp = ctx->chunk_problems;
  if (nd > 1 && P >= nd)
    cp = std::min<int32_t>(cp, std::max<int32_t>((P + kChunksPerDevice * nd - 1) / (kChunksPerDevice * nd),
                                                 std::min<int32_t>(ctx->min_shared_chunk, (P + nd - 1) / nd)));
  for (int32_t p = 0; p < P;) {
    const int32_t q = next_chunk(job->rec_off, p, P, cp, ctx->chunk_bytes);
    out.emplace_back(p, q - p);
    p = q;
  }
}

int lane_streams() {
  int64_t hwq = env_i64("GPU_MAX_HW_QUEUES", kStreams);
  if (const char* e = std::getenv("DEPPY_HW_QUEUES")) {
    const char* at = std::strchr(e, '@');
    const char* g = std::getenv("GPU_MAX_HW_QUEUES");
    if (!at || std::strcmp(at + 1, g ? g : "") == 0) hwq = std::atoll(e);
  }
  return (int)std::min<int64_t>(kMaxStreams,
                                std::max<int64_t>(1, env_i64("DEPPY_STREAMS", std::min<int64_t>(hwq, 8))));
}

}

namespace dp {
int ctx_first_ordinal(const dp_ctx* ctx) { return ctx && !ctx->dev.empty() ? ctx->dev[0].ordinal : -1; }
}

extern "C" {

dp_ctx* dp_create(const dp_opts* opts) {
  int n = 0;
  hipError_t e = hipGetDeviceCount(&n);
  if (e != hipSuccess || n == 0) {
    dp::set_global_error(std::string("dp_create: no HIP device (") + hipGetErrorString(e) + ")");
    return nullptr;
  }
  int first = opts ? opts->first_device : 0;
  int cnt = opts && opts->n_devices > 0 ? opts->n_devices : n - first;
  const bool share = opts && (opts->flags & DP_OPT_SHARE_ORDINAL) && opts->n_devices > 0;
  if (first < 0 || cnt <= 0 || (share ? first >= n || cnt > 8 : first + cnt > n)) {
    dp::set_global_error("dp_create: device range out of bounds");
    return nullptr;
  }
  auto* ctx = new dp_ctx;
  for (int i = 0; i < cnt; ++i) ctx->dev.emplace_back();
  for (int i = 0; i < cnt; ++i) {
    const int d = share ? first : first + i;
    hipDeviceProp_t prop;
    if (hipGetDeviceProperties(&prop, d) != hipSuccess || std::strncmp(prop.gcnArchName, "gfx950", 6) != 0) {
      dp::set_global_error(std::string("dp_create: device ") + std::to_string(d) + " is not gfx950 (" +
                           prop.gcnArchName + ")");
      dp_destroy(ctx);
      return nullptr;
    }
    if (hipSetDevice(d) != hipSuccess || dp::configure_solve_kernel(kMaxLdsBytes) != hipSuccess) {
      dp::set_global_error("dp_create: cannot configure the solve kernel");
      dp_destroy(ctx);
      return nullptr;
    }
    Device& D = ctx->dev[(size_t)i];
    D.ordinal = d;
    ctx->copy_streams = env_i64("DEPPY_COPY_STREAM", 0) != 0;
    D.nstreams = lane_streams();
    D.nlanes = 2 * D.nstreams;
    for (int li = 0; li < D.nlanes; ++li) {
      Lane& L = D.lanes[li];
      L.device = d;
      if (li >= D.nstreams) {
        L.s = D.lanes[li % D.nstreams].s;
        L.cs = D.lanes[li % D.nstreams].cs;
      }
      if ((li < D.nstreams && (hipStreamCreateWithFlags(&L.s, hipStreamNonBlocking) != hipSuccess ||
                             (ctx->copy_streams && hipStreamCreateWithFlags(&L.cs, hipStreamNonBlocking) != hipSuccess))) ||
          hipEventCreateWithFlags(&L.copied, hipEventDisableTiming) != hipSuccess ||
          hipEventCreate(&L.k0) != hipSuccess || hipEventCreate(&L.k1) != hipSuccess ||
          hipEventCreateWithFlags(&L.done, hipEventDisableTiming) != hipSuccess || L.spread.create() != 0) {
        dp::set_global_error("dp_create: cannot create streams");
        dp_destroy(ctx);
        return nullptr;
      }
    }
  }
  if (opts && opts->step_budget > 0) ctx->budget = opts->step_budget;
  if (opts) ctx->flags = opts->flags;
  ctx->chunk_problems = (int32_t)std::max<int64_t>(1, env_i64("DEPPY_CHUNK_PROBLEMS", kChunkProblems));
  ctx->chunk_bytes = std::max<int64_t>(1, env_i64("DEPPY_CHUNK_BYTES", kChunkBytes));
  ctx->min_shared_chunk = (int32_t)std::max<int64_t>(1, env_i64("DEPPY_MIN_SHARED_CHUNK", kMinSharedChunk));
  ctx->zc_in = env_i64("DEPPY_ZC_IN", 0) != 0;
  ctx->zc_out = env_i64("DEPPY_ZC_OUT", 1) != 0;
  ctx->direct = env_i64("DEPPY_DIRECT", 1) != 0;
  ctx->grid_cap = (int32_t)std::max<int64_t>(0, env_i64("DEPPY_GRID_CAP", 0));
  ctx->fast_path = env_i64("DEPPY_FAST_PATH", 1) != 0;
  ctx->spread = env_i64("DEPPY_SPREAD", 0) != 0;
  const int ht = dp::host_threads();
  ctx->pool = new dp::Pool(ht);
  const int per = std::max(2, ht / cnt);
  for (auto& D : ctx->dev) {
    if (hipSetDevice(D.ordinal) != hipSuccess || hipStreamCreateWithFlags(&D.fast.s, hipStreamNonBlocking) != hipSuccess ||
        hipEventCreateWithFlags(&D.fast.done, hipEventDisableTiming) != hipSuccess) {
      dp::set_global_error("dp_create: cannot create the latency stream");
      dp_destroy(ctx);
      return nullptr;
    }
    D.own_pool = cnt > 1;
    D.pool = D.own_pool ? new dp::Pool(per) : ctx->pool;
    D.fpool = new dp::Pool(std::max(2, std::min(4, per / 4)));
    D.worker = std::thread(worker_main, ctx, &D);
    D.finisher = std::thread(finisher_main, ctx, &D);
  }
  return ctx;
}

void dp_destroy(dp_ctx* ctx) {
  if (!ctx) return;
  for (auto& D : ctx->dev) {
    if (!D.worker.joinable()) continue;
    {
      std::lock_guard<std::mutex> lk(D.qmu);
      D.stop = true;
    }
    D.qcv.notify_all();
    D.worker.join();
    if (D.finisher.joinable()) {
      {
        std::lock_guard<std::mutex> lk(D.fmu);
        D.fstop = true;
      }
      D.fcv.notify_all();
      D.finisher.join();
    }
    delete D.fpool;
    D.fpool = nullptr;
    if (D.own_pool) delete D.pool;
    D.pool = nullptr;
  }
  for (auto& D : ctx->dev) {
    (void)hipSetDevice(D.ordinal);
    if (D.fast.s) (void)hipStreamSynchronize(D.fast.s);
    D.fast.h_in.release();
    D.fast.h_out.release();
    if (D.fast.done) (void)hipEventDestroy(D.fast.done);
    if (D.fast.s) (void)hipStreamDestroy(D.fast.s);
  }
  for (auto& D : ctx->dev) {
    (void)hipSetDevice(D.ordinal);
    for (int li = 0; li < D.nstreams; ++li)
      if (D.lanes[li].s) (void)hipStreamSynchronize(D.lanes[li].s);
    for (int li = 0; li < D.nlanes; ++li) {
      Lane& L = D.lanes[li];
      for (Buf* b : {&L.h_in, &L.d_in, &L.h_out, &L.d_out, &L.scratch}) b->release();
      if (L.k0) (void)hipEventDestroy(L.k0);
      if (L.k1) (void)hipEventDestroy(L.k1);
      if (L.done) (void)hipEventDestroy(L.done);
      if (L.copied) (void)hipEventDestroy(L.copied);
      L.spread.destroy();
    }
    for (int li = 0; li < D.nstreams; ++li) {
      if (D.lanes[li].s) (void)hipStreamDestroy(D.lanes[li].s);
      if (D.lanes[li].cs) (void)hipStreamDestroy(D.lanes[li].cs);
    }
  }
  delete ctx;
}

const char* dp_last_error(const dp_ctx* ctx) {
  if (!ctx) return dp_last_global_error();
  static thread_local std::string copy;
  std::lock_guard<std::mutex> lk(ctx->err_mu);
  copy = ctx->err;
  return copy.c_str();
}
int32_t dp_num_devices(const dp_ctx* ctx) { return ctx ? (int32_t)ctx->dev.size() : 0; }
int32_t dp_lanes(const dp_ctx* ctx) { return ctx && !ctx->dev.empty() ? (int32_t)ctx->dev[0].nlanes : 0; }
void* dp_host_alloc(int64_t bytes) { return bytes > 0 ? dp::pinned_alloc((size_t)bytes) : nullptr; }
void dp_host_free(void* p) {
  if (p) dp::pinned_free(p);
}

int dp_result_layout(const dp_batch* b, int64_t* inst_off, int64_t* core_off) {
  if (!b || !inst_off || !core_off || b->n_problems < 0) return -1;
  inst_off[0] = core_off[0] = 0;
  for (int32_t i = 0; i < b->n_problems; ++i) {
    const int32_t* r = b->rec + b->rec_off[i];
    inst_off[i + 1] = inst_off[i] + dp::bits_words(r[DP_H_NV]);
    core_off[i + 1] = core_off[i] + r[DP_H_NID];
  }
  return 0;
}

int dp_device_bytes(const dp_batch* b, int32_t opt_flags, int64_t* rec_bytes, int64_t* img_bytes) {
  if (!b || (b->n_problems > 0 && (!b->rec || !b->rec_off))) return -1;
  Plan P;
  dp::plan_chunk(P, b->rec, b->rec_off, 0, b->n_problems, opt_flags, nullptr);
  if (rec_bytes) *rec_bytes = P.rec_bytes;
  if (img_bytes) *img_bytes = 4 * P.img_words;
  return 0;
}

int dp_plan_order(const dp_batch* b, int32_t opt_flags, int32_t* order, int32_t* launch_first) {
  if (!b || !order || b->n_problems < 0 || (b->n_problems > 0 && (!b->rec || !b->rec_off))) return -1;
  static thread_local Plan P;
  dp::plan_chunk(P, b->rec, b->rec_off, 0, b->n_problems, opt_flags, nullptr, &dp::host_pool());
  std::copy(P.order.begin(), P.order.end(), order);
  if (launch_first)
    for (size_t k = 0; k < P.launches.size(); ++k) launch_first[k] = P.launches[k].first;
  return (int)P.launches.size();
}

int dp_plan_placements(const dp_batch* b, int32_t opt_flags, int8_t* place) {
  if (!b || !place || b->n_problems < 0 || (b->n_problems > 0 && (!b->rec || !b->rec_off))) return -1;
  static thread_local Plan P;
  dp::plan_chunk(P, b->rec, b->rec_off, 0, b->n_problems, opt_flags, nullptr, &dp::host_pool());
  for (int32_t i = 0; i < b->n_problems; ++i) place[i] = (int8_t)P.head[(size_t)i].place;
  return 0;
}


int dp_submit(dp_ctx* ctx, const dp_batch* b, dp_result* res, dp_job** out) {
  if (!ctx || !b || !res || !out || b->n_problems < 0 || (b->n_problems > 0 && (!b->rec || !b->rec_off)))
    return -1;
  auto* job = new dp_job;
  job->n = b->n_problems;
  job->rec = b->rec;
  job->rec_off = b->rec_off;
  job->pinned = ctx->direct && job->n > 0 && pinned_range(b->rec, 4 * (size_t)b->rec_off[job->n]);
  job->res = *res;
  std::vector<std::pair<int32_t, int32_t>> chunks;
  cut_chunks(ctx, job, chunks);
  job->chunks_left = (int)chunks.size();
  const int nd = (int)ctx->dev.size();
  if (nd == 1) {
    Device& D = ctx->dev[0];
    {
      std::lock_guard<std::mutex> lk(D.qmu);
      for (const auto& c : chunks) D.q.push_back(Task{job, c.first, c.second});
    }
    D.qcv.notify_one();
    *out = job;
    return 0;
  }
  std::stable_sort(chunks.begin(), chunks.end(), [&](const auto& x, const auto& y) {
    return b->rec_off[x.first + x.second] - b->rec_off[x.first] > b->rec_off[y.first + y.second] - b->rec_off[y.first];
  });
  {
    std::lock_guard<std::mutex> g(ctx->sqmu);
    for (const auto& c : chunks) ctx->sq.push_back(Task{job, c.first, c.second});
  }
  for (auto& D : ctx->dev) {
    { std::lock_guard<std::mutex> lk(D.qmu); }
    D.qcv.notify_one();
  }
  *out = job;
  return 0;
}

int dp_job_wait(dp_ctx* ctx, dp_job* job) {
  if (!ctx || !job) return -1;
  job->waiting.store(true, std::memory_order_release);
  for (auto& D : ctx->dev) {
    std::lock_guard<std::mutex> lk(D.qmu);
    D.qcv.notify_all();
  }
  int rc;
  {
    std::unique_lock<std::mutex> lk(job->m);
    job->cv.wait(lk, [&] { return job->chunks_left == 0; });
    rc = job->rc;
  }
  if (rc) {
    std::lock_guard<std::mutex> lk(ctx->mu);
    set_err(ctx, job->err);
  }
  delete job;
  return rc;
}

int dp_solve(dp_ctx* ctx, const dp_batch* b, dp_result* res) {
  if (!ctx || !b || !res || b->n_problems < 0 || (b->n_problems > 0 && (!b->rec || !b->rec_off))) return -1;
  if (b->n_problems > 0 && b->n_problems <= kFastProblems && b->rec_off[b->n_problems] <= kFastWords &&
      ctx->fast_path) {
    const int r = fast_solve(ctx, ctx->dev[0], b, res);
    if (r <= 0) return r;
  }
  dp_job* job = nullptr;
  if (dp_submit(ctx, b, res, &job)) return -1;
  return dp_job_wait(ctx, job);
}

int dp_get_device_stats(dp_ctx* ctx, int32_t device, dp_stats* out, int32_t reset) {
  if (!ctx || !out || device < 0 || device >= (int32_t)ctx->dev.size()) return -1;
  Device& D = ctx->dev[(size_t)device];
  std::lock_guard<std::mutex> dl(D.smu);
  *out = D.st;
  if (reset) D.st = dp_stats{};
  return 0;
}

int dp_get_stats(dp_ctx* ctx, dp_stats* out, int32_t reset) {
// ... 343 lines not shown
```

deppy_amd/csrc/solve_kernel.hpp:

```cpp
#pragma once
#include <hip/hip_runtime.h>

#include <cstdio>
#include <cstdlib>
#include <map>
#include <mutex>
#include <type_traits>
#include <utility>

#include "kernel_api.hpp"
#include "layout.hpp"

namespace dp {


namespace {

constexpr int32_t INF = 0x7fffffff;
constexpr int32_t R_DEC = -1;
constexpr int32_t R_EXTRA = -2;
enum { CK_NONE = 0, CK_ROW, CK_VAR, CK_ASSUME, CK_EXTRA };
enum { RS_SAT = 1, RS_UNSAT = -1, RS_BUDGET = 2 };

#define DP_VIS_ADD(x) vis_add(x)
// ... 20 lines not shown

__device__ __forceinline__ int wave_incl_max(int x) {
  int y = x;
  y = max(y, __builtin_amdgcn_update_dpp(0, x, 0x111, 0xf, 0xf, true));
  y = max(y, __builtin_amdgcn_update_dpp(0, x, 0x112, 0xf, 0xf, true));
  y = max(y, __builtin_amdgcn_update_dpp(0, x, 0x113, 0xf, 0xf, true));
  y = max(y, __builtin_amdgcn_update_dpp(0, y, 0x114, 0xf, 0xe, false));
  y = max(y, __builtin_amdgcn_update_dpp(0, y, 0x118, 0xf, 0xc, false));
  y = max(y, __builtin_amdgcn_update_dpp(0, y, 0x142, 0xa, 0xf, false));
  y = max(y, __builtin_amdgcn_update_dpp(0, y, 0x143, 0xc, 0xf, false));
  return y;
}

__device__ __forceinline__ int wave_min(int x) {
  constexpr int I = 0x7fffffff;
  int y = x;
  y = min(y, __builtin_amdgcn_update_dpp(I, x, 0x111, 0xf, 0xf, false));
  y = min(y, __builtin_amdgcn_update_dpp(I, x, 0x112, 0xf, 0xf, false));
  y = min(y, __builtin_amdgcn_update_dpp(I, x, 0x113, 0xf, 0xf, false));
  y = min(y, __builtin_amdgcn_update_dpp(I, y, 0x114, 0xf, 0xe, false));
  y = min(y, __builtin_amdgcn_update_dpp(I, y, 0x118, 0xf, 0xc, false));
  y = min(y, __builtin_amdgcn_update_dpp(I, y, 0x142, 0xa, 0xf, false));
  y = min(y, __builtin_amdgcn_update_dpp(I, y, 0x143, 0xc, 0xf, false));
  return __builtin_amdgcn_readlane(y, 63);
}
__device__ __forceinline__ int wave_sum(int x) { return __builtin_amdgcn_readlane(wave_incl_scan(x), 63); }

__device__ __forceinline__ bool getb(const uint32_t* b, int i) { return (b[i >> 5] >> (i & 31)) & 1u; }

}
#ifdef DP_STAMPS
__device__ __forceinline__ int64_t stamp() {
  int64_t t;
  __builtin_amdgcn_sched_barrier(0);
  asm volatile("s_memtime %0\n\ts_waitcnt lgkmcnt(0)" : "=s"(t)::"memory");
  __builtin_amdgcn_sched_barrier(0);
  return t;
}
__device__ __forceinline__ int64_t wallclock() {
  int64_t t;
  asm volatile("s_memrealtime %0\n\ts_waitcnt lgkmcnt(0)" : "=s"(t)::"memory");
  return t;
}
#define DP_STAMP(i) t[i] = stamp()
#else
#define DP_STAMP(i) (void)0
#endif
#if defined(DP_STAMPS) && defined(DP_CHECKS)
#define DP_CHK(x, lo, hi, code) chk((x), (lo), (hi), (code))
#else
#define DP_CHK(x, lo, hi, code) (x)
#endif
namespace {

template <int MODE, int MINW = 1>
struct Group {
  static constexpr bool N16 = mode_n16(MODE);
  using IX = typename std::conditional<N16, uint16_t, int32_t>::type;
  static constexpr bool NO_VIS = MODE == M_LDS && MINW > 1;
  static constexpr int NW = mode_waves(MODE);
  static constexpr int NT = 64 * NW;
  static constexpr int WBUF = mode_wbuf(MODE);
  static constexpr int CQ = mode_cq(MODE);

  static constexpr bool IMP16 = N16;
  using IMP = typename std::conditional<IMP16, uint16_t, uint32_t>::type;
  static constexpr uint32_t IMP_NONE = IMP16 ? 0xffffu : (uint32_t)INF;
  static constexpr int G_SKIP = N16 ? 0x8000 : 0x40000000;

  __device__ __forceinline__ int dec(IX x) const {
    if constexpr (!N16) return x;
    else return (int)x >= dthr ? (int)x - 0x10000 : (int)x;
  }
  __device__ __forceinline__ static IX enc(int x) { return (IX)x; }

  __device__ __forceinline__ static uint32_t ld_imp(const IMP* p) {
    if constexpr (N16) return *p;
    else return __hip_atomic_load(p, __ATOMIC_RELAXED, __HIP_MEMORY_SCOPE_AGENT);
  }
  __device__ __forceinline__ static uint32_t ld_bits(const uint32_t* p) {
    if constexpr (MODE != M_HBM) return *p;
    else return __hip_atomic_load(p, __ATOMIC_RELAXED, __HIP_MEMORY_SCOPE_AGENT);
  }

  int nv, nc, nk, nid, nrows, nbv, nbi, na, nch, ncl, nkl, nchl;
  const IX *clause_off, *clause_lits, *clause_id;
  const IX *card_off, *card_lits, *card_bound, *card_id;
  const IX *var_choice_off, *choice_off, *choice_lits, *anchors;
  const IX* rowref;
  bool rowspace;
  const uint32_t* idmask;
  const uint16_t* idpc;
  uint32_t* idt;
  __device__ __forceinline__ int row_of(int id) const {
    const uint32_t m = idmask[id >> 5];
    const int sh = id & 31;
    const int r1 = (int)idpc[id >> 5] + __popc(m & ((1u << sh) - 1u));
    return (m >> sh) & 1u ? nc + r1 : id - r1;
  }
  __device__ __forceinline__ int row_key(int r) const { return rowspace ? r : row_ident(r); }
  const IX *w_off, *w;
  const int2* w8;
  int nwatch, dthr;
  uint32_t vis;
  __device__ __forceinline__ void vis_add(uint32_t x) {
    if constexpr (!NO_VIS) vis += x;
  }
  __device__ __forceinline__ uint32_t vis_total() {
    if constexpr (NO_VIS) return 0u;
    else return (uint32_t)g_sum((int)vis);
  }
  int8_t* val;
  IX *reason, *rs, *trail, *touched, *d_mark, *l_off, *l_lits, *dq, *stk;
  IMP* imp;
  uint32_t *d_flip, *inS, *extra, *seen, *model, *used, *en, *en2, *crit, *dset, *fg;
  IX *wbuf, *cardq;
  int32_t* scal;
  static constexpr bool LR = mode_lds_rounds(MODE);
  int32_t *hkey, *fr;
  uint32_t *hrp, *hrn;
  uint16_t* tl;
  int hmask;
  bool hmode;
  int rb;
  int cap, lcap;
  int tid, lane, wid;
  int tlen, qhead;
  int64_t steps, budget;
  bool budget_hit;
  int ck, c_row, c_var, c_rp, c_rn;
  bool collect_guess;
  int learn_lo;
  int nl;
  const uint32_t* enabled;
  bool extra_mode;
  int extra_w;
  int32_t* tr;
  int tr_cap, tr_len;
  bool tr_stop;
#ifdef DP_STAMPS
  unsigned long long* lacc;
  int64_t sub[6];
  unsigned long long* dbg;
  __device__ __noinline__ int chk_fail(int x, int hi, int code) {
    if (dbg) {
      if (atomicCAS(&dbg[0], 0ull, (unsigned long long)code) == 0ull) {
        dbg[1] = (unsigned long long)(long long)x;
        dbg[2] = (unsigned long long)(long long)hi;
      }
      atomicAdd(&dbg[3], 1ull);
    }
    return 0;
  }
  __device__ __forceinline__ int chk(int x, int lo, int hi, int code) {
    return (x < lo || x >= hi) ? (chk_fail(x, hi, code), lo) : x;
  }
#define DP_ACC(i, x) do { if (tid == 0) atomicAdd(&lacc[i], (unsigned long long)(x)); } while (0)
#else
#define DP_ACC(i, x) (void)0
#endif

  bool lds_sync;
  __device__ __forceinline__ void bar() const {
    if constexpr (mode_lds_rounds(MODE)) {
      if (lds_sync) {
        __syncthreads();
        return;
      }
    }
    __builtin_amdgcn_s_waitcnt(0);
    __syncthreads();
  }
  __device__ __forceinline__ void gsync() {
    if constexpr (NW == 1) wsync();
    else bar();
  }
  int sbank;
  static_assert(NW == 1 || S_SLOT + 2 * NW <= NSCAL, "two banks of per-wave slots");
  __device__ __forceinline__ const int32_t* exchange(int v, bool writer) {
    int32_t* sl = scal + S_SLOT + sbank * NW;
    if (writer) sl[wid] = v;
    bar();
    sbank ^= 1;
    return sl;
  }
  __device__ __forceinline__ bool g_any(bool b) {
    const bool w = __ballot(b) != 0;
    if constexpr (NW == 1) {
      return w;
    } else {
      const int32_t* sl = exchange(w, lane == 0);
      int r = 0;
#pragma unroll
      for (int i = 0; i < NW; ++i) r |= sl[i];
      return r != 0;
    }
  }
  __device__ __forceinline__ int g_min(int x) {
    x = wave_min(x);
    if constexpr (NW == 1) {
      return x;
    } else {
      const int32_t* sl = exchange(x, lane == 0);
      int r = INF;
#pragma unroll
      for (int i = 0; i < NW; ++i) r = min(r, sl[i]);
      return r;
    }
  }
  __device__ __forceinline__ int g_sum(int x) {
    x = wave_sum(x);
    if constexpr (NW == 1) {
      return x;
    } else {
      const int32_t* sl = exchange(x, lane == 0);
      int r = 0;
#pragma unroll
      for (int i = 0; i < NW; ++i) r += sl[i];
      return r;
    }
  }
  __device__ __forceinline__ int claim(bool f, int& run) {
    const uint64_t m = __ballot(f);
    if constexpr (NW == 1) {
      const int at = run + __popcll(m & lanemask_lt());
      run += __popcll(m);
      return at;
    } else {
      int b = 0;
      if (m && lane == 0) b = atomicAdd(&scal[S_APP], __popcll(m));
      b = __builtin_amdgcn_readlane(b, 0);
      return run + b + __popcll(m & lanemask_lt());
    }
  }
  __device__ __forceinline__ void claim_end(int& run) {
    if constexpr (NW > 1) {
      bar();
      run += scal[S_APP];
      bar();
      if (tid == 0) scal[S_APP] = 0;
      bar();
    }
  }

  __device__ __forceinline__ bool init(char* lds, char* hbm, const int32_t* __restrict__ grec) {
    tid = (int)threadIdx.x;
    lane = lane_id();
    wid = tid >> 6;
    int4 hv = make_int4(0, 0, 0, 0);
    if (lane < 4) hv = reinterpret_cast<const int4*>(grec)[lane];
    int32_t h[DP_H_SIZE];
#pragma unroll
    for (int q = 0; q < 4; ++q) {
      h[4 * q + 0] = __builtin_amdgcn_readlane(hv.x, q);
      h[4 * q + 1] = __builtin_amdgcn_readlane(hv.y, q);
      h[4 * q + 2] = __builtin_amdgcn_readlane(hv.z, q);
      h[4 * q + 3] = __builtin_amdgcn_readlane(hv.w, q);
    }
    if (h[DP_H_FMT] == DP_FMT_REJECT) return false;
#ifdef DP_STAMPS
    const int64_t ti0 = stamp();
#endif
    const Layout L = layout<MODE>(h);
    const dp_rec_layout R = rec_layout(h);
    const ImgLayout X = img_layout(h);
    scal = reinterpret_cast<int32_t*>(lds + L.scal);
    sbank = 0;
    ncl = h[DP_H_NCL]; nkl = h[DP_H_NKL]; nchl = h[DP_H_NCHL];
    nv = h[DP_H_NV]; nc = h[DP_H_NC]; nk = h[DP_H_NK]; nid = h[DP_H_NID]; na = h[DP_H_NA];
    nch = h[DP_H_NCH];
    nrows = nc + nk;
    nbv = bits_words(nv); nbi = bits_words(nid);
    const IX* body;
    bool packed = false;
    rowref = nullptr;
    rowspace = false;
    if constexpr (N16) {
      IX* b = reinterpret_cast<IX*>(lds + L.body);
      const int4* src = reinterpret_cast<const int4*>(grec + DP_H_SIZE);
      const int fmt = h[DP_H_FMT];
      packed = fmt_packed(fmt);
      if (!packed && fmt != DP_FMT_U16 && fmt != DP_FMT_U16_CHECKED) return false;
      const bool p8 = fmt == DP_FMT_P8D;
      const int land = p8 ? p16_tail_copy(h) : 0;
      const int groups = p8 ? (p8_bytes(h) + 15) >> 4
                            : packed ? (int)((p16_tail_at(h) + p16_tail_bytes(h) + 15) >> 4)
                                     : (h[DP_H_WORDS] - DP_H_SIZE + 7) >> 3;
      if (L.body == 0 && land + ((groups + 63) >> 6) * 1024 <= L.lds_bytes) {
        for (int c = 64 * wid; c < groups; c += NT) {
          const int i = min(c + lane, groups - 1);
          __builtin_amdgcn_global_load_lds((__attribute__((address_space(1))) void*)(src + i),
                                           (__attribute__((address_space(3))) void*)(lds + land + 16 * c), 16, 0, 0);
        }
        __builtin_amdgcn_s_waitcnt(0);
        gsync();
      } else {
        for (int i = tid; i < groups; i += NT) reinterpret_cast<int4*>(reinterpret_cast<char*>(b) + land)[i] = src[i];
        gsync();
      }
      body = b;
      if (packed) {
        const bool derived = fmt_derived(fmt);
        IX* q = b;
        clause_lits = q; q += ncl;
        card_lits = q;   q += nkl;
        card_bound = q;  q += nk;
        if (!derived) { choice_lits = q; q += nchl; }
        anchors = q;     q += na;
        clause_off = q;  q += nc + 1;
        card_off = q;    q += nk + 1;
        var_choice_off = q; q += nv + 1;
        if (derived) { rowref = q; q += nch; }
        else { choice_off = q; q += nch + 1; }
        q += (q - b) & 1;
        idmask = reinterpret_cast<const uint32_t*>(q); q += 2 * nbi;
        idpc = reinterpret_cast<const uint16_t*>(q);   q += nbi + 1;
        rowspace = true;
        auto decode = [&] {
          uint8_t* raw = reinterpret_cast<uint8_t*>(b) + land;
          uint8_t* ex = reinterpret_cast<uint8_t*>(b) + p8_tail(h);
          const bool ok8 = !p8 || expand8(raw, h[DP_H_P8] & 0xff, p8_bytes(h), ex);
          const bool ok16 = unpack16(p8 ? reinterpret_cast<const char*>(ex)
                                        : reinterpret_cast<const char*>(b) + p16_tail_at(h),
                                     (int)p16_tail_bytes(h), derived, lds + L.reason,
                                     p8 ? ex : reinterpret_cast<uint8_t*>(b) + p16_tail_copy(h));
          return ok8 && ok16;
        };
        bool ok;
        if constexpr (NW == 1) {
          ok = decode();
        } else {
          ok = true;
          if (wid == 0) ok = decode();
          ok = !g_any(!ok);
        }
        if (!ok) return false;
      }
    } else {
      body = reinterpret_cast<const IX*>(grec + DP_H_SIZE);
    }
    auto rv = [&](int32_t word_off) { return body + (word_off - DP_H_SIZE); };
    if (!packed) {
      clause_off = rv(R.clause_off); clause_lits = rv(R.clause_lits); clause_id = rv(R.clause_id);
      card_off = rv(R.card_off); card_lits = rv(R.card_lits); card_bound = rv(R.card_bound);
      card_id = rv(R.card_id); var_choice_off = rv(R.var_choice_off); choice_off = rv(R.choice_off);
      choice_lits = rv(R.choice_lits); anchors = rv(R.anchors);
    }
    nwatch = h[DP_H_NCL] + h[DP_H_NKL];
    dthr = nrows + L_MAX;
    char* hot = MODE == M_HBM ? hbm : lds;
    char* cold = N16 ? lds : hbm;
    val = reinterpret_cast<int8_t*>(hot + L.val);
    reason = reinterpret_cast<IX*>(cold + L.reason);
    rs = reinterpret_cast<IX*>(cold + L.rs);
    trail = reinterpret_cast<IX*>(cold + L.trail);
    touched = reinterpret_cast<IX*>(cold + L.touched);
    d_mark = reinterpret_cast<IX*>(cold + L.d_mark);
    imp = reinterpret_cast<IMP*>(cold + L.imp);
    w8 = nullptr;
    d_flip = reinterpret_cast<uint32_t*>(hot + L.d_flip);
    inS = reinterpret_cast<uint32_t*>(hot + L.inS);
    extra = reinterpret_cast<uint32_t*>(hot + L.extra);
    seen = reinterpret_cast<uint32_t*>(hot + L.seen);
    model = reinterpret_cast<uint32_t*>(hot + L.model);
    dset = reinterpret_cast<uint32_t*>(hot + L.dset);
    fg = reinterpret_cast<uint32_t*>(hot + L.fg);
    used = reinterpret_cast<uint32_t*>(hot + L.used);
    en = reinterpret_cast<uint32_t*>(hot + L.en);
    en2 = reinterpret_cast<uint32_t*>(hot + L.en2);
    crit = reinterpret_cast<uint32_t*>(hot + L.crit);
    idt = reinterpret_cast<uint32_t*>(lds + L.idt);
    l_off = reinterpret_cast<IX*>(cold + L.l_off);
    l_lits = reinterpret_cast<IX*>(cold + L.l_lits);
    dq = reinterpret_cast<IX*>(cold + L.dq);
    stk = reinterpret_cast<IX*>(cold + L.stk);
    wbuf = reinterpret_cast<IX*>(lds + L.wbuf);
    cardq = reinterpret_cast<IX*>(lds + L.cardq);
    hkey = reinterpret_cast<int32_t*>(lds + L.hkey);
    hrp = reinterpret_cast<uint32_t*>(lds + L.hrp);
    hrn = reinterpret_cast<uint32_t*>(lds + L.hrn);
    tl = reinterpret_cast<uint16_t*>(lds + L.tl);
    fr = reinterpret_cast<int32_t*>(lds + L.fr);
    hmask = L.hc - 1;
    hmode = LR;
    lds_sync = false;
    rb = 0;
#ifdef DP_STAMPS
    lacc = reinterpret_cast<unsigned long long*>(scal + (MODE == M_LDS ? 8 : NSCAL));
#endif
    cap = L.cap; lcap = L.lcap;
    tlen = qhead = 0;
    pre_lo = -1;
    steps = 0;
    vis = 0;
    budget_hit = false;
    ck = CK_NONE; c_row = c_var = c_rp = c_rn = 0;
    collect_guess = false;
    learn_lo = 0;
    nl = 0;
    enabled = nullptr;
    extra_mode = false;
    extra_w = 0;
    tr = nullptr;
    tr_cap = tr_len = 0;
    tr_stop = false;
#ifdef DP_STAMPS
    dbg = nullptr;
#endif
#ifdef DP_STAMPS
    const int64_t ti1 = stamp();
    sub[0] = ti1 - ti0;
#endif
    if constexpr (N16)
      if ((h[DP_H_FMT] == DP_FMT_U16 || packed) && !valid_record(body, packed, fmt_derived(h[DP_H_FMT]))) return false;
    if constexpr (!N16)
      if ((h[DP_H_FMT] == DP_FMT_I32W || h[DP_H_FMT] == DP_FMT_I32) && !valid_wide(R, X, h[DP_H_FMT] == DP_FMT_I32W))
        return false;
#ifdef DP_STAMPS
    const int64_t ti2 = stamp();
    sub[1] = ti2 - ti1;
#endif
    if constexpr (N16) {
      IX* wo = const_cast<IX*>(body) + lds_body_words(h);
      build_watches(wo, wo + 2 * nv + 1, reinterpret_cast<uint32_t*>(lds + L.reason));
      w_off = wo; w = wo + 2 * nv + 1;
    } else {
      if (h[DP_H_FMT] == DP_FMT_I32) {
        IX* wo = reinterpret_cast<IX*>(hbm + L.wl);
        if (device_watches(h)) build_watches_wide(wo, wo + 2 * nv + 2, reinterpret_cast<uint32_t*>(lds + L.wbuf));
        w_off = wo; w = nullptr;
        w8 = reinterpret_cast<const int2*>(wo + 2 * nv + 2);
      } else {
        w_off = rv(X.w_off); w = rv(X.w);
      }
    }
#ifdef DP_STAMPS
    sub[2] = stamp() - ti2;
#endif

    if constexpr (N16) {
      for (int v = tid; v < nv; v += NT) val[v] = 0;
    } else {
      for (int v = tid; v < (nv + 3) / 4; v += NT) reinterpret_cast<uint32_t*>(val)[v] = 0;
    }
    for (int l = tid; l < 2 * nv; l += NT) imp[l] = (IMP)IMP_NONE;
    if constexpr (LR)
      for (int i = tid; i <= hmask; i += NT) { hkey[i] = -1; hrp[i] = (uint32_t)INF; hrn[i] = (uint32_t)INF; }
    for (int i = tid; i < nbv; i += NT) {
      d_flip[i] = 0; inS[i] = 0; extra[i] = 0; seen[i] = 0; model[i] = 0; dset[i] = 0; fg[i] = 0;
    }
    for (int i = tid; i < mode_nscal(MODE); i += NT) scal[i] = 0;
    if (tid == 0) {
      l_off[0] = 0;
      scal[S_POSROWS] = h[DP_H_NVU] > 0;
    }
    gsync();
    return true;
  }

  __device__ __forceinline__ bool valid_record(const IX* base, bool packed, bool derived) {
    static_assert(N16, "16-bit records run on the LDS image");
    const uint32_t* b32 = reinterpret_cast<const uint32_t*>(base);
    bool bad = false;
    auto range = [&](const IX* arr, int n, int hi) {
      const int a = (int)(arr - base), e = a + n;
      for (int q0 = (a >> 1); 2 * q0 < e; q0 += 4 * NT) {
        uint32_t x[4];
#pragma unroll
        for (int i = 0; i < 4; ++i) {
          const int q = q0 + i * NT + tid;
          x[i] = 2 * q < e ? b32[q] : 0u;
        }
#pragma unroll
        for (int i = 0; i < 4; ++i) {
          const int q = q0 + i * NT + tid;
          bad |= 2 * q < e && ((2 * q >= a && (int)(x[i] & 0xffffu) >= hi) || (2 * q + 1 < e && (int)(x[i] >> 16) >= hi));
        }
      }
    };
    auto offsets = [&](const IX* arr, int n, int total) {
      const int a = (int)(arr - base), e = a + n + 1;
      for (int q = (a >> 1) + tid; 2 * q < e; q += NT) {
        const uint32_t x = b32[q];
        const int i0 = 2 * q, x0 = (int)(x & 0xffffu), x1 = (int)(x >> 16);
        const int prev = i0 > a ? (int)(b32[q - 1] >> 16) : 0;
        if (i0 >= a) bad |= i0 == a ? x0 != 0 : x0 < prev;
        if (i0 + 1 < e) bad |= i0 + 1 == a ? x1 != 0 : x1 < x0;
        bad |= (i0 == e - 1 && x0 != total) || (i0 + 1 == e - 1 && x1 != total);
      }
    };
    if (packed) {
      if (tid == 0)
        bad = (int)clause_off[nc] != ncl || (int)card_off[nk] != nkl || (int)var_choice_off[nv] != nch ||
              (!derived && (int)choice_off[nch] != nchl);
    } else {
      offsets(clause_off, nc, ncl);
      range(clause_id, nc, nid);
      offsets(card_off, nk, nkl);
      range(card_id, nk, nid);
      offsets(var_choice_off, nv, nch);
      offsets(choice_off, nch, nchl);
    }
    range(clause_lits, ncl, 2 * nv);
    range(card_lits, nkl, nv);
    if (!derived) range(choice_lits, nchl, nv);
    range(anchors, na, nv);
    if (g_any(bad)) return false;
    for (int k = tid; k < nk; k += NT) {
      const int a = card_off[k], len = (int)card_off[k + 1] - a;
      if (len <= 16) {
        int v[16];
#pragma unroll
        for (int i = 0; i < 16; ++i) v[i] = i < len ? (int)card_lits[a + i] : -1 - i;
#pragma unroll
        for (int j = 2; j < 16; ++j) {
          bool dup = false;
#pragma unroll
          for (int i = 0; i < j - 1; ++i) dup |= v[i] == v[j];
          bad |= dup && v[j] != v[j - 1];
        }
      } else {
        for (int j = a + 1; j < a + len; ++j) {
          const int x = card_lits[j];
          if (x != (int)card_lits[j - 1])
            for (int i = a; i < j - 1; ++i) bad |= (int)card_lits[i] == x;
        }
      }
    }
    return !g_any(bad);
  }

  __device__ __forceinline__ bool valid_wide(const dp_rec_layout& R, const ImgLayout& X, bool watches) {
    static_assert(!N16, "the int32 form runs on the HBM-read multi-wave groups");
    const int32_t* r = reinterpret_cast<const int32_t*>(clause_off) - R.clause_off;
    bool bad = false;
    constexpr int VU = 8;
    auto offsets = [&](int at, int n, int total, bool exact) {
      for (int i0 = tid; i0 <= n; i0 += VU * NT) {
// ... 400 lines not shown
    }
  }
  __device__ __forceinline__ void note_lds(int l, int r) {
    const int v = l >> 1;
    int h = (int)(((uint32_t)v * 2654435761u) >> 16) & hmask;
    for (int probe = 0;; ++probe) {
      const int k = hkey[h];
      if (k == v) break;
      if (k < 0) {
        const int old = atomicCAS(&hkey[h], -1, v);
        if (old < 0 || old == v) break;
      }
      if (probe == 32 || probe == hmask) {
        scal[S_OVB + rb] = 1;
        return;
      }
      h = (h + 1) & hmask;
    }
    uint32_t* rr = (l & 1) ? hrn : hrp;
    if (atomicMin(&rr[h], (uint32_t)r) == (uint32_t)INF) {
      tl[atomicAdd(&scal[S_NTB + rb], 1)] = (uint16_t)((h << 1) | (l & 1));
      const uint32_t* ro = (l & 1) ? hrp : hrn;
      if (ro[h] != (uint32_t)INF) atomicMax(&scal[S_CVB + rb], INF - v);
    }
  }
  __device__ __forceinline__ int slot_of(int v) const {
    int h = (int)(((uint32_t)v * 2654435761u) >> 16) & hmask;
    while (hkey[h] != v) h = (h + 1) & hmask;
    return h;
  }
  __device__ __forceinline__ void put_trail(int i, int l) {
    trail[DP_CHK(i, 0, nv, 9)] = enc(l);
    if constexpr (LR) fr[i & hmask] = l;
  }

  __device__ __forceinline__ void note(int l, int r) {
    l = DP_CHK(l, 0, 2 * nv, 1);
    if constexpr (LR) {
      if (hmode) {
        note_lds(l, r);
        return;
      }
    }
    if (imp_min(l, r))
      touched[DP_CHK(atomicAdd(&scal[S_NTOUCHED], 1), 0, 2 * nv, 2)] = enc(l);
  }

  __device__ __forceinline__ void note_all(int l, int r) {
    if (l >= 0) note(l, r);
  }

#ifndef DP_EVAL_UNROLL
#define DP_EVAL_UNROLL 4
#endif
  __device__ __forceinline__ int eval_clause(int r, const IX* lits, int a, int b, int& crow) {
    int nun = 0, ul = -1;
    DP_VIS_ADD(2 * sizeof(IX) + (uint32_t)(b - a) * (sizeof(IX) + 1));
    constexpr int U = DP_EVAL_UNROLL;
    for (int j = a; j < b; j += U) {
      int l[U];
#pragma unroll
      for (int k = 0; k < U; ++k) l[k] = j + k < b ? (int)lits[j + k] : -1;
      int x[U];
#pragma unroll
      for (int k = 0; k < U; ++k) x[k] = l[k] >= 0 ? lit_val(l[k]) : -1;
#pragma unroll
      for (int k = 0; k < U; ++k) {
        if (x[k] > 0) return -1;
        if (x[k] == 0) { ++nun; ul = l[k]; }
      }
    }
    if (nun == 0) crow = min(crow, r);
    return nun == 1 ? ul : -1;
  }
  __device__ __forceinline__ int clause_unit(int r, int& crow, uint32_t info = ROW_INFO_NONE) {
    if constexpr (!N16) {
      if (r < nc && info != ROW_INFO_NONE) {
        const int a = (int)(info >> 8);
        return eval_clause(r, clause_lits, a, a + (int)(info & 255u), crow);
      }
    }
    if (r < nc) return eval_clause(r, clause_lits, clause_off[r], clause_off[r + 1], crow);
    const int j = r - nrows;
    return eval_clause(r, l_lits, DP_CHK((int)l_off[j], 0, lcap + 1, 33), DP_CHK((int)l_off[j + 1], 0, lcap + 1, 34), crow);
  }

  __device__ __forceinline__ void card_serial(int r, int& crow) {
    const int k = r - nc, a = card_off[k], b = card_off[k + 1];
    int cnt = 0, nun = 0;
    DP_VIS_ADD(3 * sizeof(IX) + (uint32_t)(b - a) * (sizeof(IX) + 1));
    for (int j = a; j < b; ++j) {
      const int x = val[card_lits[j]];
      cnt += (x > 0);
      nun += (x == 0);
    }
    const int bound = card_bound[k];
    if (cnt > bound) crow = min(crow, r);
    else if (nun > 0) {
      for (int j = a; j < b;) {
        const int v = card_lits[j];
        int e = j + 1;
        while (e < b && (int)card_lits[e] == v) ++e;
        if (val[v] == 0 && cnt + (e - j) > bound) note(2 * v + 1, r);
        j = e;
      }
    }
  }

  static constexpr int CQW = CQ / NW;
  __device__ __forceinline__ void visit(int r, int& crow, int& ncq, uint32_t info = ROW_INFO_NONE) {
    DP_VIS_ADD(r >= 0 ? sizeof(IX) : 0);
    const bool ok = r >= 0 && row_on(r);
    const bool card = ok && r >= nc && r < nrows;
    const uint64_t m = __ballot(card);
    const bool q = ncq + __popcll(m) <= CQW;
    const int pos = wid * CQW + ncq + __popcll(m & lanemask_lt());
    if (card && q) {
      cardq[pos] = enc(r);
      if constexpr (NW > 1 && !N16) cardq[CQ + pos] = (IX)info;
    } else if (card) card_serial(r, crow);
    else if (ok) {
      const int ul = clause_unit(r, crow, info);
      if (ul >= 0) note(ul, r);
    }
    if (q) ncq += __popcll(m);
  }

  __device__ __forceinline__ void flush_cards(int& crow, int ncq) {
    if (ncq == 0) return;
    wsync();
    for (int q = wid * CQW; q < wid * CQW + ncq; ++q) {
      const int r = DP_CHK((int)cardq[q], nc, nrows, 3), k = r - nc;
      int a, len;
      const uint32_t info = NW > 1 && !N16 ? (uint32_t)cardq[CQ + q] : ROW_INFO_NONE;
      if (info != ROW_INFO_NONE) {
        a = (int)(info >> 8);
        len = (int)(info & 255u);
      } else {
        a = card_off[k];
        len = (int)card_off[k + 1] - a;
      }
      const int bound = card_bound[k];
      if (len > 64) {
        card_long(r, a, len, bound, crow);
        continue;
      }
      const int v = lane < len ? (int)card_lits[a + lane] : -1;
      const int x = v >= 0 ? val[v] : 0;
      DP_VIS_ADD((v >= 0 ? sizeof(IX) + 1 : 0) + (lane == 0 ? 3 * sizeof(IX) : 0));
      const int cnt = __popcll(__ballot(v >= 0 && x > 0));
      if (cnt > bound) { crow = min(crow, r); continue; }
      if (!__ballot(v >= 0 && x == 0)) continue;
      const bool start = v >= 0 && (lane == 0 || (int)card_lits[a + lane - 1] != v);
      const uint64_t ms = __ballot(start);
      const uint64_t after = lane < 63 ? ms >> (lane + 1) : 0ull;
      const int run = (after ? lane + 1 + __ffsll((unsigned long long)after) - 1 : len) - lane;
      note_all(start && x == 0 && cnt + run > bound ? 2 * v + 1 : -1, r);
    }
  }
  __device__ __forceinline__ void card_long(int r, int a, int len, int bound, int& crow) {
    int cnt = 0;
    bool any = false;
    for (int j0 = 0; j0 < len; j0 += 64) {
      const int j = j0 + lane;
      const int v = j < len ? (int)card_lits[a + j] : -1;
      const int x = v >= 0 ? val[v] : 0;
      DP_VIS_ADD(v >= 0 ? sizeof(IX) + 1 : 0);
// ... 349 lines not shown
        best = max(best, run);
      }
      return best > bound;
    }
    for (int j = a; j < b;) {
      int e = j + 1;
      while (e < b && card_lits[e] == card_lits[j]) ++e;
      if (e - j > bound) return true;
      j = e;
    }
    return false;
  }

  __device__ __forceinline__ int base_propagate() {
    const int r = run_round([&](int& crow) {
      int ncq = 0;
      for (int i0 = 0; i0 < nrows; i0 += NT) {
        const int row = i0 + tid;
        const bool f = row < nc ? (int)clause_off[row + 1] - (int)clause_off[row] <= 1
                                : row < nrows && card_fires(row - nc);
        visit(f ? row : -1, crow, ncq);
      }
      flush_cards(crow, ncq);
      eval_learned(crow);
    });
    if (r < 0) return -1;
    return propagate();
  }

  __device__ __forceinline__ void truncate_to(int mark) {
#ifdef DP_STAMPS
    const int64_t t0 = stamp();
    truncate_to_(mark);
    DP_ACC(19, stamp() - t0);
  }
  __device__ __forceinline__ void truncate_to_(int mark) {
#endif
    gsync();
    for (int i = mark + tid; i < tlen; i += NT) val[DP_CHK((int)trail[i], 0, 2 * nv, 14) >> 1] = 0;
    tlen = qhead = mark;
    gsync();
  }

  __device__ __forceinline__ int untest_to(int mark) {
    truncate_to(mark);
    if (nl > learn_lo) {
      if (run_round([&](int& crow) { eval_learned(crow); }) < 0) return -1;
      return propagate();
    }
    return tlen == nv ? 1 : 0;
  }

  __device__ __forceinline__ void assign_one(int l, int why, int decision) {
    if constexpr (NW > 1) bar();
    if (tid == 0) {
      const int v = DP_CHK(l, 0, 2 * nv, 30) >> 1;
      val[v] = (l & 1) ? -1 : 1; reason[v] = enc(decision >= 0 ? -3 - decision : why);
      rs[v] = enc(tlen); put_trail(tlen, l);
    }
    ++tlen;
    gsync();
  }

  __device__ __forceinline__ int test_assume(int l, int xv = 2, int wa = 0, int we = -1) {
    ++steps;
    const int x = xv == 2 ? lit_val(l) : ((l & 1) ? -xv : xv);
    if (x > 0) return propagate();
    if (x < 0) { ck = CK_ASSUME; c_var = l >> 1; return -1; }
    if (we >= 0) { pre_lo = tlen; pre_a = wa; pre_e = we; }
    assign_one(l, R_DEC, -1);
    return propagate();
  }

  __device__ __forceinline__ void mark_push(int v) {
    const uint32_t bit = 1u << (v & 31);
    const uint32_t old = atomicOr(&seen[v >> 5], bit);
    if (!(old & bit)) touched[atomicAdd(&scal[S_NWORK], 1)] = enc(v);
  }
  __device__ __forceinline__ void set_bit_atomic(uint32_t* b, int i) { atomicOr(&b[i >> 5], 1u << (i & 31)); }

  __device__ __forceinline__ void ante_serial(int r, int u, int bound) {
    r = DP_CHK(r, 0, nrows + nl, 15);
    if (r < nc || r >= nrows) {
      const IX* lits = clause_lits;
      int a, b;
      if (r < nc) { a = clause_off[r]; b = clause_off[r + 1]; set_bit_atomic(used, row_key(r)); }
      else {
        lits = l_lits;
        a = DP_CHK((int)l_off[r - nrows], 0, lcap + 1, 35);
        b = DP_CHK((int)l_off[r - nrows + 1], 0, lcap + 1, 36);
      }
      for (int j = a; j < b; ++j) {
        const int v = (int)lits[j] >> 1;
        if (v != u) mark_push(v);
      }
    } else {
      const int k = r - nc;
      set_bit_atomic(used, row_key(r));
      for (int j = card_off[k]; j < card_off[k + 1]; ++j) {
        const int v = card_lits[j];
        if (v != u && val[v] > 0 && (int)rs[v] < bound) mark_push(v);
      }
    }
  }
  __device__ __forceinline__ void extra_serial(int u, int bound) {
    for (int v = 0; v < nv; ++v)
      if (v != u && getb(extra, v) && val[v] > 0 && (int)rs[v] < bound) mark_push(v);
  }

  __device__ __forceinline__ void analyze() {
#ifdef DP_STAMPS
    const int64_t t0 = stamp();
    analyze_();
    DP_ACC(17, stamp() - t0);
    DP_ACC(22, 1);
  }
  __device__ __forceinline__ void analyze_() {
#endif
    gsync();
    if (tid == 0) {
      scal[S_NWORK] = 0;
      if (ck == CK_ROW) ante_serial(c_row, -1, INF);
      else if (ck == CK_VAR) { ante_serial(c_rp, c_var, c_row); ante_serial(c_rn, c_var, c_row); }
      else if (ck == CK_EXTRA) extra_serial(-1, INF);
      else if (ck == CK_ASSUME) mark_push(c_var);
    }
    gsync();
    int head = 0;
    for (;;) {
      const int nw = scal[S_NWORK];
      if constexpr (NW > 1) bar();
      if (head >= nw) break;
      for (int i = head + tid; i < nw; i += NT) {
        const int u = DP_CHK((int)touched[i], 0, nv, 16);
        const int r = dec(reason[u]);
        if (r >= 0) ante_serial(r, u, rs[u]);
        else if (r == R_EXTRA) extra_serial(u, rs[u]);
        else if (r <= -3) set_bit_atomic(dset, DP_CHK(-3 - r, 0, nv, 32));
        else if (collect_guess && getb(inS, u)) set_bit_atomic(fg, u);
      }
      head = nw;
      gsync();
    }
    const int nw = scal[S_NWORK];
    for (int i = tid; i < nw; i += NT) {
      const int v = touched[i];
      atomicAnd(&seen[v >> 5], ~(1u << (v & 31)));
    }
    gsync();
  }

  __device__ __forceinline__ bool violated(int c, int& fu, uint32_t info = ROW_INFO_NONE) const {
    fu = -1;
    int ja, jb;
    if (!N16 && info != ROW_INFO_NONE) {
      ja = (int)(info >> 8);
      jb = ja + (int)(info & 255u);
    } else {
      ja = clause_off[c];
      jb = clause_off[c + 1];
    }
    for (int j = ja; j < jb; ++j) {
      const int l = clause_lits[j];
      const int x = val[l >> 1];
      if (l & 1) {
        if (x != 1) return false;
      } else {
        if (x == 1) return false;
        if (x == 0 && fu < 0) fu = l;
      }
    }
    return true;
  }

  __device__ __forceinline__ int first_violated() {
#ifdef DP_STAMPS
    const int64_t t0 = stamp();
    const int r = first_violated_();
    DP_ACC(16, stamp() - t0);
    DP_ACC(18, 1);
    return r;
  }
  __device__ __forceinline__ int first_violated_() {
#endif
    int best = INF;
    if (nc <= 4 * NT || scal[S_POSROWS]) {
      for (int c = tid; c < nc; c += NT) {
        int fu;
        if (row_on(c) && violated(c, fu)) { best = c; break; }
      }
      best = g_min(best);
      if (best == INF) return -1;
      int fu;
      violated(best, fu);
      return fu;
    }
    for (int i0 = 64 * wid; i0 < tlen; i0 += NT) {
      const int i = i0 + lane;
      const int l = i < tlen ? (int)trail[i] : 1;
      int s = 0, n = 0;
      if (!(l & 1)) { s = (int)w_off[l]; n = (int)w_off[l + 1] - s; }
      const int inc = wave_incl_scan(n);
      const int total = __builtin_amdgcn_readlane(inc, 63);
      for (int base = 0; base < total; base += 64) {
        const int f = base + lane;
        int j = 0;
        for (int step = 32; step; step >>= 1)
          if (__shfl(inc, j + step - 1) <= f) j += step;
        const int sj = __shfl(s, j), ej = __shfl(inc, j) - __shfl(n, j);
        if (f < total) {
          const int2 e = went(sj + f - ej);
          const int c = e.x;
          int fu;
          if (c < nc && c < best && row_on(c) && violated(c, fu, (uint32_t)e.y)) best = c;
        }
      }
    }
    best = g_min(best);
    if (best == INF) return -1;
    int fu;
    violated(best, fu);
    return fu;
  }

  __device__ __forceinline__ void save_model() {
#ifdef DP_STAMPS
    const int64_t t0 = stamp();
    save_model_();
    DP_ACC(20, stamp() - t0);
  }
  __device__ __forceinline__ void save_model_() {
#endif
    for (int b = 0; b < nv; b += NT) {
      const int v = b + tid;
      const uint64_t m = __ballot(v < nv && val[v] > 0);
      const int wd = (b + 64 * wid) >> 5;
      if (lane == 0 && wd < nbv) {
        model[wd] = (uint32_t)m;
        if (wd + 1 < nbv) model[wd + 1] = (uint32_t)(m >> 32);
      }
    }
    gsync();
  }

  __device__ __forceinline__ void clear_bits(uint32_t* bs, int n) {
    for (int i = tid; i < bits_words(n); i += NT) bs[i] = 0;
    gsync();
  }

  __device__ __forceinline__ int dlit(int i) const {
    return (int)trail[(int)d_mark[i]] ^ (int)getb(d_flip, i);
  }

  __device__ __forceinline__ int dpll() {
    const int root = tlen, nl0 = nl;
    int nd = 0, r;
    bool decide = true;
    for (;;) {
      if (decide) {
        const int l = first_violated();
        if (l < 0) { save_model(); r = RS_SAT; break; }
        if (++steps > budget) { budget_hit = true; r = RS_BUDGET; break; }
        if (tid == 0) {
          d_mark[nd] = enc(tlen);
          d_flip[nd >> 5] &= ~(1u << (nd & 31));
        }
        assign_one(l, R_DEC, nd);
        ++nd;
      }
      if (propagate() >= 0) { decide = true; continue; }
      decide = false;
      clear_bits(dset, nd);
      analyze();
      int h = -1, b = -1, n = 0;
      for (int wi = bits_words(nd) - 1; wi >= 0 && b < 0; --wi) {
        uint32_t x = ld_bits(&dset[wi]);
        while (x && b < 0) {
          const int i = wi * 32 + 31 - __clz(x);
          x &= ~(1u << (i & 31));
          if (h < 0) h = i; else b = i;
        }
      }
      for (int wi = 0; wi < bits_words(nd); ++wi) n += __popc(ld_bits(&dset[wi]));
      if (h < 0) { r = RS_UNSAT; break; }
      if (++steps > budget) { budget_hit = true; r = RS_BUDGET; break; }
      const int lat = DP_CHK((int)l_off[nl], 0, lcap + 1, 26);
      if (nl < L_MAX && lat + n <= lcap) {
        int run = lat;
        for (int base = 0; base < nd; base += NT) {
          const int i = base + tid;
          const bool in = i < nd && ((ld_bits(&dset[i >> 5]) >> (i & 31)) & 1u);
          const int at = claim(in, run);
          if (in) l_lits[DP_CHK(at, 0, lcap, 27)] = enc(dlit(i) ^ 1);
        }
        claim_end(run);
        if (tid == 0) l_off[nl + 1] = enc(run);
        ++nl;
        gsync();
        const int lh = dlit(h);
        nd = b + 1;
        truncate_to(DP_CHK((int)d_mark[nd], 0, nv + 1, 24));
        assign_one(lh ^ 1, nrows + nl - 1, -1);
      } else {
        while (nd > 0 && getb(d_flip, nd - 1)) --nd;
        if (nd == 0) { r = RS_UNSAT; break; }
        const int lf = dlit(nd - 1);
        truncate_to(DP_CHK((int)d_mark[nd - 1], 0, nv + 1, 25));
        if (tid == 0) d_flip[(nd - 1) >> 5] |= 1u << ((nd - 1) & 31);
        gsync();
        assign_one(lf ^ 1, R_DEC, nd - 1);
      }
    }
    truncate_to(root);
    nl = nl0;
    return r;
  }

  int dq_head, dq_n, ng, result;
  int pre_lo, pre_a, pre_e;
  bool class_b, solve_unsat, last_solve;
  bool final_from_solve;

  __device__ __forceinline__ int list_len(int list) const {
    if (list >= nch) return 1;
    if (rowref) {
      const int r = rowref[list];
      return (int)clause_off[r + 1] - (int)clause_off[r] - 1;
    }
    return (int)choice_off[list + 1] - (int)choice_off[list];
  }
  __device__ __forceinline__ int list_at(int list, int i) const {
    if (list >= nch) return list - nch;
    if (rowref) return (int)clause_lits[(int)clause_off[rowref[list]] + 1 + i] >> 1;
    return (int)choice_lits[(int)choice_off[list] + i];
  }
  __device__ __forceinline__ void dq_push_back(int list, int idx) {
    int at = dq_head + dq_n;
    if (at >= cap) at -= cap;
    if (tid == 0) { dq[2 * at] = enc(list); dq[2 * at + 1] = enc(idx); }
    ++dq_n;
  }
  __device__ __forceinline__ void dq_push_front(int list, int idx) {
    dq_head = dq_head == 0 ? cap - 1 : dq_head - 1;
    if (tid == 0) { dq[2 * dq_head] = enc(list); dq[2 * dq_head + 1] = enc(idx); }
    ++dq_n;
  }

  __device__ __forceinline__ int guess_m(int list, int idxf) const {
    const int idx = idxf & ~G_SKIP;
    return !(idxf & G_SKIP) && idx < list_len(list) ? list_at(list, idx) : -1;
  }

  __device__ __forceinline__ void push_guess() {
#ifdef DP_STAMPS
    const int64_t tpg = stamp();
#endif
    gsync();
    const int list = DP_CHK((int)dq[2 * dq_head], 0, nch + nv, 17), idx = DP_CHK((int)dq[2 * dq_head + 1], 0, nv + 1, 18);
    dq_head = dq_head + 1 == cap ? 0 : dq_head + 1;
    --dq_n;
    const bool single = list >= nch;
    int len = 1, base = 0, sh = 0;
    const IX* src = clause_lits;
    if (!single) {
      if (rowref) {
        const int r = rowref[list];
        base = (int)clause_off[r] + 1;
        len = (int)clause_off[r + 1] - base;
        sh = 1;
      } else {
        base = choice_off[list];
        len = (int)choice_off[list + 1] - base;
        src = choice_lits;
      }
    }
    auto entry = [&](int i) { return single ? list - nch : (int)src[base + i] >> sh; };
    int m = idx < len ? entry(idx) : -1;
    const int mc = m >= 0 ? m : 0;
    const int c0 = var_choice_off[mc], c1 = var_choice_off[mc + 1], xm = val[mc];
    const int wa = w_off[2 * mc], we = w_off[2 * mc + 1];
    bool any = false;
    for (int i = tid; i < len; i += NT) any |= getb(inS, entry(i));
    const bool skip = g_any(any);
    if (skip) m = -1;
    else if (idx >= len) class_b = true;
    const int nchild = m >= 0 ? c1 - c0 : 0;
    for (int k = tid; k < nchild; k += NT) {
      int at = dq_head + dq_n + k;
      if (at >= cap) at -= cap;
      dq[2 * at] = enc(c0 + k); dq[2 * at + 1] = enc(0);
    }
    dq_n += nchild;
    if (tid == 0) {
      IX* g = stk + 3 * ng;
      g[0] = enc(list); g[1] = enc(idx | (skip ? G_SKIP : 0)); g[2] = enc(tlen);
      if (m >= 0) atomicOr(&inS[m >> 5], 1u << (m & 31));
    }
    ++ng;
    gsync();
    if (m < 0) return;
    if (steps >= budget) { budget_hit = true; result = 0; return; }
#ifdef DP_STAMPS
    DP_ACC(21, stamp() - tpg);
#endif
    result = test_assume(2 * m, xm, wa, we);
    last_solve = false;
  }

  __device__ __forceinline__ void pop_guess() {
    gsync();
    --ng;
    const IX* g = stk + 3 * ng;
    const int list = DP_CHK((int)g[0], 0, nch + nv, 19), idxf = (int)g[1],
              mark = DP_CHK((int)g[2], 0, nv + 1, 23);
    const int idx = DP_CHK(idxf & ~G_SKIP, 0, nv + 1, 20);
    int m = -1;
    if (!(idxf & G_SKIP)) {
      if (list >= nch) {
        m = idx < 1 ? list - nch : -1;
      } else if (rowref) {
        const int r = rowref[list];
        const int a = (int)clause_off[r] + 1, len = (int)clause_off[r + 1] - a;
        if (idx < len) m = (int)clause_lits[a + idx] >> 1;
      } else {
        const int a = choice_off[list], len = (int)choice_off[list + 1] - a;
        if (idx < len) m = choice_lits[a + idx];
      }
    }
    m = DP_CHK(m, -1, nv, 21);
    const int children = m >= 0 ? (int)var_choice_off[m + 1] - (int)var_choice_off[m] : 0;
    gsync();
    if (m >= 0) {
      if (tid == 0) inS[m >> 5] &= ~(1u << (m & 31));
      gsync();
      result = untest_to(mark);
      last_solve = false;
    }
    dq_n -= children;
    dq_push_front(list, idx + (m >= 0 ? 1 : 0));
    gsync();
  }

  __device__ __forceinline__ int search_solve() {
    clear_bits(fg, nv);
    collect_guess = true;
    const int r = dpll();
    collect_guess = false;
    if (r == RS_UNSAT) {
      int n = 0;
      for (int wi = tid; wi < nbv; wi += NT) n += __popc(ld_bits(&fg[wi]));
      n = g_sum(n);
      const int lat = l_off[nl];
      if (nl < L_MAX && lat + n <= lcap) {
        int run = lat;
        for (int b = 0; b < nv; b += NT) {
          const int v = b + tid;
          const bool in = v < nv && ((ld_bits(&fg[v >> 5]) >> (v & 31)) & 1u);
          const int at = claim(in, run);
          if (in) l_lits[at] = enc(2 * v + 1);
        }
        claim_end(run);
        if (tid == 0) l_off[nl + 1] = enc(run);
        ++nl;
        gsync();
      }
    }
    return r;
  }

  __device__ __forceinline__ int search() {
    dq_head = dq_n = ng = 0;
    result = 0;
    class_b = solve_unsat = last_solve = false;
    for (int i = 0; i < na; ++i) dq_push_back(nch + (int)anchors[i], 0);
    fill_bits(used, nid, false);
    fill_bits(en, nid, false);
    bool from_solve = false;
#ifdef DP_STAMPS
    const int64_t tloop = stamp();
    int64_t tgap = tloop;
#endif
    for (;;) {
#ifdef DP_STAMPS
      DP_ACC(24, stamp() - tgap);
#endif
      if (dq_n == 0 && result == 0) {
        if (tr) {
          or_bits(en, used, nid);
          fill_bits(used, nid, false);
        }
#ifdef DP_STAMPS
        const int64_t ts = stamp();
        const int r = search_solve();
        DP_ACC(5, stamp() - ts);
#else
        const int r = search_solve();
#endif
        from_solve = true;
        if (r == RS_BUDGET) { result = RS_BUDGET; break; }
        result = r;
        last_solve = (r == RS_SAT);
        if (r == RS_UNSAT) solve_unsat = true;
      }
      if (result < 0) {
        if (tr) trace_event(from_solve);
        if (ng == 0) break;
#ifdef DP_STAMPS
        const int64_t tq = stamp();
        pop_guess();
        DP_ACC(6, stamp() - tq);
#else
        pop_guess();
#endif
        from_solve = false;
        continue;
      }
      if (dq_n == 0) break;
#ifdef DP_STAMPS
      const int64_t tp = stamp();
      push_guess();
      tgap = stamp();
      DP_ACC(4, tgap - tp);
      DP_ACC(7, 1);
#else
      push_guess();
#endif
      from_solve = false;
      if (budget_hit) { result = RS_BUDGET; break; }
    }
#ifdef DP_STAMPS
    DP_ACC(23, stamp() - tloop);
#endif
    final_from_solve = from_solve;
    or_bits(used, en, nid);
    if (result == 1 && !last_solve) save_model();
    return result;
  }

  __device__ __forceinline__ void reset_all() { truncate_to(0); }

  __device__ __forceinline__ int emit_bits(const uint32_t* bits, int nw, int32_t* out) {
    int len = 0;
    for (int b = 0; b < nw; b += NT) {
      const int i = b + tid;
      const uint32_t x = i < nw ? ld_bits(&bits[i]) : 0u;
      const int c = __popc(x);
// ... 267 lines not shown
    if (base_propagate() < 0) return DP_ERROR;
    const int start = tlen;
    bool bad = false;
    int run = tlen;
    for (int b = 0; b < nv; b += NT) {
      const int v = b + tid;
      bool f = false;
      int l = 0;
      if (v < nvu && !getb(extra, v)) {
        const int want = getb(inS, v) ? 1 : -1;
        if (val[v] == -want) bad = true;
        if (val[v] == 0) { f = true; l = 2 * v + (want < 0 ? 1 : 0); }
      }
      const int at = claim(f, run);
      if (f) {
        val[v] = (l & 1) ? -1 : 1; reason[v] = enc(R_DEC); rs[v] = enc(start);
        put_trail(at, l);
      }
    }
    claim_end(run);
    tlen = run;
    gsync();
    if (g_any(bad)) return DP_ERROR;
    if (propagate() < 0) return DP_ERROR;
    const int mark = tlen;
    int f = 0;
    for (int v = tid; v < nv; v += NT) f += getb(extra, v) && val[v] > 0;
    f = g_sum(f);
    extra_mode = true;
    for (int wv = f; wv <= ne; ++wv) {
      truncate_to(mark);
      extra_w = wv;
      if (propagate() < 0) continue;
      const int r = dpll();
      if (r == RS_SAT) {
        extra_mode = false;
        for (int i = tid; i < nbv; i += NT) out[i] = model[i] & ubits(i);
        return DP_SAT;
      }
      if (r == RS_BUDGET) { extra_mode = false; return DP_INCOMPLETE; }
    }
    extra_mode = false;
    return DP_ERROR;
  }
};

}

#ifndef DP_LDS_MIN_WAVES
#define DP_LDS_MIN_WAVES 5
#endif
__device__ __forceinline__ void put_out(ProblemOut* o, int status, int32_t flags, int32_t clen, int32_t cat,
                                        int64_t steps, uint64_t bcp) {
  uint4 x, y;
  x.x = (uint32_t)(uint8_t)(int8_t)status;
  x.y = (uint32_t)flags;
  x.z = (uint32_t)clen;
  x.w = (uint32_t)cat;
  y.x = (uint32_t)(uint64_t)steps;
  y.y = (uint32_t)((uint64_t)steps >> 32);
  y.z = (uint32_t)bcp;
  y.w = (uint32_t)(bcp >> 32);
  uint4* p = reinterpret_cast<uint4*>(o);
  p[0] = x;
  p[1] = y;
}

__device__ __forceinline__ int nvu_of(const int32_t* grec, int nv) {
  const int u = grec[DP_H_NVU];
  return u > 0 && u < nv ? u : nv;
}

template <int MODE, int MINW>
__device__ __forceinline__ void solve_item(const KernelArgs& a, int k, int4* lds4) {
#ifdef DP_STAMPS
  int64_t t[6];
  const int64_t wall0 = wallclock();
#endif
  DP_STAMP(0);
  const WorkItem it = a.items[k];
  const int pid = it.pid;
  const int32_t* grec = a.rec + it.rec_off;
  Group<MODE, MINW> W;
  char* hbm = mode_n16(MODE) ? nullptr : reinterpret_cast<char*>(a.scratch + a.scratch_off[k]);
  if (!W.init(reinterpret_cast<char*>(lds4), hbm, grec)) {
    if (threadIdx.x == 0) {
      put_out(a.out + pid, DP_ERROR, DP_F_MALFORMED, 0, 0, 0, 0);
      if (a.trace) a.trace_len[pid] = 0;
    }
    uint32_t* inst0 = a.installed + it.inst_off;
    for (int i = threadIdx.x; i < bits_words(grec[DP_H_NV]); i += blockDim.x) inst0[i] = 0;
    return;
  }
#ifdef DP_STAMPS
  if (a.stamps) W.dbg = reinterpret_cast<unsigned long long*>(a.stamps + (int64_t)DP_NSTAMP * pid + 12);
#endif
  W.budget = a.budget;
  if constexpr (Group<MODE, MINW>::LR)
    if (a.table_cap > 0 && a.table_cap - 1 < W.hmask) W.hmask = a.table_cap - 1;
  if (a.trace) {
    W.tr = a.trace + (int64_t)a.trace_cap * pid;
    W.tr_cap = a.trace_cap;
  }
  uint32_t* inst = a.installed + it.inst_off;
  int32_t flags = 0;
  int status;
  for (int i = W.tid; i < W.nbv; i += Group<MODE, MINW>::NT) inst[i] = 0;
  DP_STAMP(1);
  const int base = W.base_propagate();
  DP_STAMP(2);
  DP_STAMP(3);
  if (base < 0) {
    flags |= DP_F_BASE_UNSAT;
    status = DP_UNSAT;
    W.fill_bits(W.used, W.nid, false);
    W.analyze();
  } else if (base == 1) {
    flags |= DP_F_SEARCH_SKIPPED;
    W.save_model();
    status = W.epilogue(flags, inst, nvu_of(grec, W.nv));
  } else {
    const int r = W.search();
    DP_STAMP(3);
    if (W.class_b) flags |= DP_F_CLASS_B;
    if (W.solve_unsat) flags |= DP_F_SOLVE_UNSAT;
    if (r == RS_BUDGET) {
      flags |= DP_F_BUDGET;
      status = DP_INCOMPLETE;
    } else if (r < 0) {
      status = DP_UNSAT;
      if (!W.final_from_solve) W.analyze();
    } else {
      status = W.epilogue(flags, inst, nvu_of(grec, W.nv));
      if (status == DP_INCOMPLETE) flags |= DP_F_BUDGET;
    }
  }
  DP_STAMP(4);
  int clen = 0, cat = 0;
  if (status == DP_UNSAT) clen = W.core(a.core, a.core_pool_len, flags, cat);
  DP_STAMP(5);
#ifdef DP_STAMPS
  if (W.tid == 0 && a.stamps) {
    int64_t* o = a.stamps + (int64_t)DP_NSTAMP * pid;
    for (int i = 0; i < 5; ++i) o[i] = t[i + 1] - t[i];
    for (int i = 0; i < 5; ++i) o[5 + i] = (int64_t)W.lacc[i];
    o[10] = wall0;
    o[11] = wallclock();
    for (int i = 5; i < 16; ++i) o[11 + i] = (int64_t)W.lacc[i];
    for (int i = 0; i < 3; ++i) o[27 + i] = W.sub[i];
    for (int i = 3; i < 6; ++i) o[45 + i] = W.sub[i];
    for (int i = 16; i < 32; ++i) o[16 + i] = (int64_t)W.lacc[i];
  }
#endif
  if (W.tr_stop) flags |= DP_F_TRACE_TRUNCATED;
  const uint64_t bcp = W.vis_total();
  if (W.tid == 0) {
    if (a.trace) a.trace_len[pid] = W.tr_len;
    put_out(a.out + pid, status, flags, clen, cat, W.steps, bcp);
  }
}

template <int MODE, int MINW>
__global__ void __launch_bounds__(64 * mode_waves(MODE), MINW)
solve_kernel(KernelArgs a) {
  extern __shared__ int4 lds4[];
  if constexpr (MODE != M_LDS) {
    if (a.queue) {
      int32_t* slot = reinterpret_cast<int32_t*>(lds4);
      for (;;) {
        __syncthreads();
        if (threadIdx.x == 0) *slot = atomicAdd(a.queue, 1);
        __syncthreads();
        const int k = *slot;
        __syncthreads();
        if (k >= a.n_items) return;
        solve_item<MODE, MINW>(a, k, lds4);
      }
    }
  }
  solve_item<MODE, MINW>(a, (int)blockIdx.x, lds4);
}

struct GridCache {
  std::mutex mu;
  std::map<std::pair<int, int>, int> per_cu;
  int cus[64] = {};
};
template <int MODE, int MINW>
int resident_grid(int lds_bytes) {
  static GridCache c;
  int dev = 0;
  if (hipGetDevice(&dev) != hipSuccess || dev < 0 || dev >= 64) return 0;
  std::lock_guard<std::mutex> lk(c.mu);
  if (c.cus[dev] == 0 && hipDeviceGetAttribute(&c.cus[dev], hipDeviceAttributeMultiprocessorCount, dev) != hipSuccess)
    c.cus[dev] = 0;
  auto it = c.per_cu.find({dev, lds_bytes});
  if (it == c.per_cu.end()) {
    int per = 0;
    if (hipOccupancyMaxActiveBlocksPerMultiprocessor(&per, solve_kernel<MODE, MINW>, 64 * mode_waves(MODE),
                                                     lds_bytes) != hipSuccess)
      per = 0;
    it = c.per_cu.emplace(std::make_pair(dev, lds_bytes), per).first;
  }
  return it->second * c.cus[dev];
}
inline bool debug_grid() {
  static const bool on = std::getenv("DEPPY_DEBUG_GRID") != nullptr;
  return on;
}

#define DP_DEFINE_MODE(MODE, MINW, NAME)                                                    \
  hipError_t NAME(const KernelArgs& a, int n_blocks, int lds_bytes, hipStream_t stream) {   \
    if (n_blocks <= 0) return hipSuccess;                                                   \
    int grid = n_blocks;                                                                    \
    if (a.queue) {                                                                          \
      const int res = resident_grid<MODE, MINW>(lds_bytes);                                 \
      if (res > 0 && res < grid) grid = res;                                                \
      if (a.grid_cap > 0 && a.grid_cap < grid) grid = a.grid_cap;                           \
      if (debug_grid())                                                                     \
        fprintf(stderr, "solve launch mode %d: %d items, resident %d -> grid %d\n", MODE, n_blocks, res, grid); \
    }                                                                                       \
    hipLaunchKernelGGL((solve_kernel<MODE, MINW>), dim3((unsigned)grid), dim3(64 * mode_waves(MODE)), \
                       (size_t)lds_bytes, stream, a);                                       \
    return hipGetLastError();                                                               \
  }                                                                                         \
  hipError_t NAME##_configure(int max_lds_bytes) {                                          \
    return hipFuncSetAttribute(reinterpret_cast<const void*>(&solve_kernel<MODE, MINW>),          \
                               hipFuncAttributeMaxDynamicSharedMemorySize, max_lds_bytes);  \
  }

}
```

deppy_amd/csrc/solve_launch.cpp:

```cpp
#include <cstdlib>

#include "kernel_api.hpp"
#include "layout.hpp"

namespace dp {

hipError_t launch_lds(const KernelArgs&, int, int, hipStream_t);
hipError_t launch_lds_dense(const KernelArgs&, int, int, hipStream_t);
hipError_t launch_split(const KernelArgs&, int, int, hipStream_t);
hipError_t launch_split4(const KernelArgs&, int, int, hipStream_t);
hipError_t launch_hbm(const KernelArgs&, int, int, hipStream_t);
hipError_t launch_ldsg(const KernelArgs&, int, int, hipStream_t);
hipError_t launch_lds_configure(int);
hipError_t launch_lds_dense_configure(int);
hipError_t launch_split_configure(int);
hipError_t launch_split4_configure(int);
hipError_t launch_hbm_configure(int);
hipError_t launch_ldsg_configure(int);

constexpr int kUnboundedWavesPerCU = 16;
constexpr int kLdsPerCU = 160 * 1024;

hipError_t launch_solve(const KernelArgs& a, int mode, int n_blocks, int lds_bytes, hipStream_t stream) {
  if (mode == M_LDS) {
    static const bool no_dense = [] {
      const char* e = std::getenv("DEPPY_NO_DENSE");
      return e && *e && *e != '0';
    }();
    const bool dense = !no_dense && lds_bytes > 0 && kLdsPerCU / lds_bytes > kUnboundedWavesPerCU;
    return dense ? launch_lds_dense(a, n_blocks, lds_bytes, stream) : launch_lds(a, n_blocks, lds_bytes, stream);
  }
  if (mode == M_SPLIT) return launch_split(a, n_blocks, lds_bytes, stream);
  if (mode == M_SPLIT4) return launch_split4(a, n_blocks, lds_bytes, stream);
  if (mode == M_LDSG) return launch_ldsg(a, n_blocks, lds_bytes, stream);
  return launch_hbm(a, n_blocks, lds_bytes, stream);
}

hipError_t configure_solve_kernel(int max_lds_bytes) {
  hipError_t e = launch_lds_configure(max_lds_bytes);
  if (e == hipSuccess) e = launch_lds_dense_configure(max_lds_bytes);
  if (e == hipSuccess) e = launch_split_configure(max_lds_bytes);
  if (e == hipSuccess) e = launch_split4_configure(max_lds_bytes);
  if (e == hipSuccess) e = launch_hbm_configure(max_lds_bytes);
  if (e == hipSuccess) e = launch_ldsg_configure(max_lds_bytes);
  return e;
}

}
```

include/deppy_hip.h:

```cpp
#ifndef DEPPY_HIP_H
#define DEPPY_HIP_H

#include <stdint.h>

#ifdef __cplusplus
extern "C" {
#endif

#define DP_ABI_VERSION 1


enum dp_kind {
  DP_MANDATORY = 1,
  DP_PROHIBITED = 2,
  DP_DEPENDENCY = 3,
  DP_CONFLICT = 4,
  DP_ATMOST = 5
};

typedef struct dp_wire {
  int32_t n_problems;
  const int64_t* prob_var_off;
  const int64_t* var_id;
  const int64_t* var_con_off;
// ... 200 lines not shown
typedef struct dp_ctx dp_ctx;

typedef struct dp_batch {
  int32_t n_problems;
  const int64_t* rec_off;
  const int32_t* rec;
} dp_batch;

typedef struct dp_result {
  int8_t* status;
  int32_t* flags;
  uint32_t* installed;
  const int64_t* inst_off;
  int32_t* core;
  const int64_t* core_off;
  int32_t* core_len;
  int64_t* steps;
} dp_result;

int dp_result_layout(const dp_batch* b, int64_t* inst_off, int64_t* core_off);

dp_ctx* dp_create(const dp_opts* opts);
void dp_destroy(dp_ctx* ctx);
const char* dp_last_error(const dp_ctx* ctx);
const char* dp_last_global_error(void);
int32_t dp_num_devices(const dp_ctx* ctx);
int32_t dp_lanes(const dp_ctx* ctx);

int dp_solve(dp_ctx* ctx, const dp_batch* b, dp_result* res);

typedef struct dp_job dp_job;
int dp_submit(dp_ctx* ctx, const dp_batch* b, dp_result* res, dp_job** job);
int dp_job_wait(dp_ctx* ctx, dp_job* job);

typedef struct dp_stats {
  int64_t problems;
  int64_t chunks;
  int64_t launches;
  double kernel_ms;
  int64_t h2d_bytes;
  int64_t d2h_bytes;
  int64_t rec_bytes;
  double stage_ms;
  double plan_ms;
  double wait_ms;
  double scatter_ms;
  int64_t direct_chunks;
  int64_t bcp_bytes;
  int64_t allocs;
  int64_t placed[5];
  int64_t placed_launches[5];
} dp_stats;
int dp_get_stats(dp_ctx* ctx, dp_stats* out, int32_t reset);
int dp_get_device_stats(dp_ctx* ctx, int32_t device, dp_stats* out, int32_t reset);

typedef struct dp_resident dp_resident;
int dp_upload(dp_ctx* ctx, const dp_batch* b, dp_resident** out);
int dp_run(dp_ctx* ctx, dp_resident* r);
int dp_launch(dp_ctx* ctx, dp_resident* r);
int dp_wait(dp_ctx* ctx, dp_resident* r);
int dp_download(dp_ctx* ctx, dp_resident* r, dp_result* res);
void dp_resident_free(dp_ctx* ctx, dp_resident* r);
int dp_upload_traced(dp_ctx* ctx, const dp_batch* b, int32_t trace_cap, dp_resident** out);
int dp_download_trace(dp_ctx* ctx, dp_resident* r, int32_t* trace, int32_t* trace_len);
int dp_solve_traced(dp_ctx* ctx, const dp_batch* b, int32_t trace_cap, dp_result* res,
                    int32_t* trace, int32_t* trace_len);

int dp_device_bytes(const dp_batch* b, int32_t opt_flags, int64_t* rec_bytes, int64_t* img_bytes);

int dp_stage_roundtrip(const dp_batch* b, int32_t opt_flags, int32_t chunk_problems, int64_t chunk_bytes,
                       int32_t* out_rec, int32_t* chunk_first, int32_t cap);
int dp_stitch_selftest(const dp_batch* b, int32_t chunk_problems, dp_result* res);
int dp_partition(const int64_t* rec_off, int32_t n_problems, int32_t nd, int32_t* cut);
enum dp_place {
  DP_PLACE_LDS = 0,
  DP_PLACE_SPLIT = 1,
  DP_PLACE_HBM = 2,
  DP_PLACE_SPLIT4 = 3,
  DP_PLACE_LDSG = 4,
  DP_PLACE_MALFORMED = -1,
  DP_PLACE_TOO_LARGE = -2
};
int dp_plan_placements(const dp_batch* b, int32_t opt_flags, int8_t* place);
int dp_plan_order(const dp_batch* b, int32_t opt_flags, int32_t* order, int32_t* launch_first);

int dp_last_kernel_ms(const dp_ctx* ctx, double* ms);


typedef struct dp_gen dp_gen;
dp_gen* dp_gen_catalogs(int32_t config, int32_t n_problems, uint64_t base_seed);
const dp_wire* dp_gen_wire(const dp_gen* g);
void dp_gen_free(dp_gen* g);

const char* dp_build_info(void);

#ifdef __cplusplus
}
#endif
#endif
```

Before: 30.30 million.

## Evict CDCL learnt-clause arrays from LDS to global scratch in LDS mode

Moves the d_mark, l_off and l_lits arrays of the single-wave LDS solve mode out of shared memory into a per-problem global scratch region. The aim is to shrink the LDS footprint so more blocks fit per CU. Placement and density decisions now count LDS plus scratch bytes, and a new scratch buffer is allocated per launch. This adds global-memory traffic and waitcnt drains on conflict analysis, and also exposes footprint and occupancy query APIs.

```diff
diff --git a/deppy_amd/_lib.py b/deppy_amd/_lib.py
--- a/deppy_amd/_lib.py
+++ b/deppy_amd/_lib.py
@@ -72,6 +72,7 @@
     "dp_gen_free", "dp_upload_traced", "dp_download_trace", "dp_solve_traced", "dp_lowered_errors",
     "dp_device_bytes", "dp_lower_into", "dp_lowered_new", "dp_lowered_exact_count", "dp_lowered_pinned", "dp_rec_widen", "dp_submit", "dp_job_wait", "dp_get_stats", "dp_stage_roundtrip",
     "dp_stitch_selftest", "dp_partition", "dp_build_info", "dp_get_device_stats", "dp_plan_placements",
+    "dp_plan_footprints", "dp_lds_occupancy",
     "dp_plan_order", "dp_dlower_new", "dp_dlower_free", "dp_lower_device", "dp_dlower_host_count",
     "dp_host_alloc", "dp_host_free",
 ]
@@ -250,6 +251,8 @@
     L.dp_host_alloc.restype = vp
     L.dp_host_free.argtypes = [vp]
     L.dp_plan_placements.argtypes = [ctypes.POINTER(Batch), ctypes.c_int32, c_i8p]
+    L.dp_plan_footprints.argtypes = [ctypes.POINTER(Batch), ctypes.c_int32, c_i32p, c_i32p]
+    L.dp_lds_occupancy.argtypes = [ctypes.c_int32, ctypes.c_int32]
     L.dp_plan_order.argtypes = [ctypes.POINTER(Batch), ctypes.c_int32, c_i32p, c_i32p]
     _lib = L
     return L
@@ -756,6 +759,24 @@
     return place[:len(rec_off) - 1]
 
 
+def plan_footprints(rec_off, rec, flags: int = 0):
+    rec_off = np.ascontiguousarray(rec_off, np.int64)
+    rec = np.ascontiguousarray(rec if len(rec) else np.zeros(1, np.int32), np.int32)
+    n = len(rec_off) - 1
+    lds = np.zeros(max(n, 1), np.int32)
+    scratch = np.zeros(max(n, 1), np.int32)
+    if lib().dp_plan_footprints(ctypes.byref(_batch(rec_off, rec)), flags, _p(lds, c_i32p), _p(scratch, c_i32p)) != 0:
+        raise RuntimeError("dp_plan_footprints failed")
+    return lds[:n], scratch[:n]
+
+
+def lds_occupancy(lds_bytes: int, capped: bool = False) -> int:
+    r = lib().dp_lds_occupancy(int(lds_bytes), int(bool(capped)))
+    if r < 0:
+        raise RuntimeError("dp_lds_occupancy failed")
+    return r
+
+
 def plan_order(rec_off, rec, flags: int = 0):
     rec_off = np.ascontiguousarray(rec_off, np.int64)
     rec = np.ascontiguousarray(rec if len(rec) else np.zeros(1, np.int32), np.int32)
diff --git a/deppy_amd/csrc/kernel_api.hpp b/deppy_amd/csrc/kernel_api.hpp
--- a/deppy_amd/csrc/kernel_api.hpp
+++ b/deppy_amd/csrc/kernel_api.hpp
@@ -35,6 +35,8 @@
   int64_t budget;
   int32_t* scratch;
   const int64_t* scratch_off;
+  int64_t lds_scratch_off;
+  int64_t lds_scratch_stride;
   int64_t* stamps;
   int32_t* trace;
   int32_t* trace_len;
@@ -46,7 +48,9 @@
 };
 constexpr int kQueueWords = 64;
 
-hipError_t launch_solve(const KernelArgs& a, int mode, int n_blocks, int lds_bytes, hipStream_t stream);
+hipError_t launch_solve(const KernelArgs& a, int mode, int n_blocks, int lds_bytes, bool dense, hipStream_t stream);
+bool lds_dense(int full_bytes);
+int lds_occupancy(int lds_bytes, bool dense);
 hipError_t launch_watch_build(const KernelArgs& a, int mode, int n_items, hipStream_t stream);
 hipError_t configure_solve_kernel(int max_lds_bytes);
 
diff --git a/deppy_amd/csrc/layout.hpp b/deppy_amd/csrc/layout.hpp
--- a/deppy_amd/csrc/layout.hpp
+++ b/deppy_amd/csrc/layout.hpp
@@ -17,6 +17,7 @@
                   (int)M_SPLIT4 == DP_PLACE_SPLIT4 && (int)M_LDSG == DP_PLACE_LDSG,
               "enum dp_place (include/deppy_hip.h) names the placements");
 __host__ __device__ constexpr bool mode_n16(int mode) { return mode == M_LDS || mode == M_LDSG; }
+__host__ __device__ constexpr bool mode_evict(int mode) { return mode == M_LDS; }
 #ifndef DP_BIG_WAVES
 #define DP_BIG_WAVES 8
 #endif
@@ -123,6 +124,19 @@
   const int64_t body = (int64_t)h[DP_H_WORDS] - DP_H_SIZE;
   const int64_t w = narrow ? DP_H_SIZE + (body + 1) / 2 : (int64_t)img_layout(h).words;
   return (w + 3) & ~3LL;
+}
+
+struct CdclLayout {
+  int32_t d_mark, l_off, l_lits, bytes;
+};
+__host__ __device__ inline CdclLayout cdcl_layout(int32_t nv) {
+  CdclLayout C;
+  int32_t o = 0;
+  C.d_mark = o; o += (nv * 2 + 15) & ~15;
+  C.l_off = o;  o += ((L_MAX + 1) * 2 + 15) & ~15;
+  C.l_lits = o; o += ((nv + 64) * 2 + 15) & ~15;
+  C.bytes = o;
+  return C;
 }
 
 struct Layout {
@@ -173,8 +187,9 @@
   return c;
 }
 
-template <int MODE>
+template <int MODE, bool EV = mode_evict(MODE)>
 __host__ __device__ inline Layout layout_hc(const int32_t* h, int32_t hc) {
+  static_assert(!EV || mode_evict(MODE), "only an evicting mode has the evicting layout");
   constexpr bool N16 = mode_n16(MODE);
   using IX = typename std::conditional<N16, uint16_t, int32_t>::type;
   Layout L;
@@ -182,6 +197,9 @@
   const int32_t nbv = bits_words(nv), nbi = bits_words(nid);
   const int32_t ix = (int32_t)sizeof(IX);
   int32_t og = 0, ol = 0;
+  static_assert(!EV || N16, "cdcl_layout is the 16-bit image's");
+  const CdclLayout C = cdcl_layout(nv);
+  enum { COLD = 0, HOT = 1, WORK = 2 };
   auto take = [&](int32_t nbytes, int kind) {
     const bool lds = N16 || kind == 2 || (kind == 1 && (MODE == M_SPLIT || MODE == M_SPLIT4));
     int32_t& o = lds ? ol : og;
@@ -189,7 +207,6 @@
     o += (nbytes + 15) & ~15;
     return at;
   };
-  enum { COLD = 0, HOT = 1, WORK = 2 };
   L.cap = h[DP_H_NA] + h[DP_H_NCH] + 2;
   L.lcap = nv + 64;
   const ImgLayout X = img_layout(h);
@@ -227,22 +244,22 @@
   L.rs = take(nv * ix, COLD);
   L.trail = take(nv * ix, COLD);
   L.touched = take(2 * nv * ix, COLD);
-  L.d_mark = take(nv * ix, COLD);
+  L.d_mark = EV ? C.d_mark : take(nv * ix, COLD);
   L.imp = take(2 * nv * (N16 ? 2 : 4), COLD);
-  L.l_off = take((L_MAX + 1) * ix, COLD);
-  L.l_lits = take(L.lcap * ix, COLD);
+  L.l_off = EV ? C.l_off : take((L_MAX + 1) * ix, COLD);
+  L.l_lits = EV ? C.l_lits : take(L.lcap * ix, COLD);
   L.dq = take(2 * L.cap * ix, COLD);
   L.stk = take(3 * L.cap * ix, COLD);
   L.wl = !N16 && h[DP_H_FMT] == DP_FMT_I32 ? take((2 * nv + 2) * 4 + (h[DP_H_NCL] + h[DP_H_NKL]) * 8, COLD) : 0;
-  L.bytes = og;
+  L.bytes = EV ? C.bytes : og;
   L.lds_bytes = ol;
   return L;
 }
 
 constexpr int32_t kLdsLimitBytes = 160 * 1024;
-template <int MODE>
+template <int MODE, bool EV = mode_evict(MODE)>
 __host__ __device__ inline Layout layout(const int32_t* h) {
-  if (!mode_lds_rounds(MODE)) return layout_hc<MODE>(h, 0);
+  if (!mode_lds_rounds(MODE)) return layout_hc<MODE, EV>(h, 0);
   int32_t hc = round_slots(h[DP_H_NV]);
   Layout L = layout_hc<MODE>(h, hc);
   while (hc > 64 && L.lds_bytes > kLdsLimitBytes) L = layout_hc<MODE>(h, hc >>= 1);
diff --git a/deppy_amd/csrc/lower_device.hip b/deppy_amd/csrc/lower_device.hip
--- a/deppy_amd/csrc/lower_device.hip
+++ b/deppy_amd/csrc/lower_device.hip
@@ -460,7 +460,8 @@
   h[DP_H_NKL] = nkl;
   h[DP_H_NCHL] = nchl;
   h[DP_H_WORDS] = DP_H_SIZE + (nc + 1) + ncl + nc + (nk + 1) + nkl + 2 * nk + (nv + 1) + (nch + 1) + nchl + na;
-  if (!fits16_dev(h) || (int64_t)dp::layout<dp::M_LDS>(h).lds_bytes > a.group_above) return give_up();
+  const dp::Layout wl = dp::layout<dp::M_LDS>(h);
+  if (!fits16_dev(h) || (int64_t)wl.lds_bytes + wl.bytes > a.group_above) return give_up();
   auto put_header = [&]() {
     for (int i = lane; i < DL_SLOT; i += DL_T) S.rec[i] = 0u;
     __syncthreads();
diff --git a/deppy_amd/csrc/placement.hpp b/deppy_amd/csrc/placement.hpp
--- a/deppy_amd/csrc/placement.hpp
+++ b/deppy_amd/csrc/placement.hpp
@@ -22,7 +22,9 @@
 }
 
 inline bool one_wave(const int32_t* h) {
-  return fits16(h) && (int64_t)layout<M_LDS>(h).lds_bytes <= group_above();
+  if (!fits16(h)) return false;
+  const Layout L = layout<M_LDS>(h);
+  return (int64_t)L.lds_bytes + L.bytes <= group_above();
 }
 
 constexpr int32_t kLdsgMaxProblems = 256;
diff --git a/deppy_amd/csrc/runtime.cpp b/deppy_amd/csrc/runtime.cpp
--- a/deppy_amd/csrc/runtime.cpp
+++ b/deppy_amd/csrc/runtime.cpp
@@ -95,6 +95,7 @@
 struct Launch {
   int first, count, mode, lds;
   bool dev_lists;
+  bool dense = false;
 };
 
 struct Head {
@@ -105,6 +106,7 @@
   int32_t lds, inst_words, nid;
   int64_t sw, rec_bytes;
   uint8_t cls;
+  int32_t scratch;
 };
 
 constexpr int32_t kPlanBlock = 512;
@@ -113,6 +115,8 @@
   int64_t img = 0, inst = 0, core = 0, rbytes = 0, other = 0;
   int32_t ndirect = 0, nother = 0, nok = 0;
   int32_t bcount[kNBuckets] = {}, bmax[kNBuckets] = {};
+  int32_t smax = 0;
+  int32_t bfull[kNBuckets] = {};
 };
 
 struct Plan {
@@ -124,6 +128,7 @@
   std::vector<Launch> launches;
   int big_base = 0;
   std::vector<int64_t> scratch_off;
+  int64_t lds_scratch_base = 0, lds_scratch_stride = 0, lds_first = 0;
   int64_t scratch_words = 0;
   std::vector<int32_t> skip;
   std::vector<int32_t> skip_flags;
@@ -160,8 +165,10 @@
   bool nar = false;
   if (dp::fits16(h)) {
     if (!forced_of(opt_flags)) {
-      H.lds = layout<M_LDS>(h).lds_bytes;
-      nar = H.lds <= dp::group_above();
+      const Layout Y = layout<M_LDS>(h);
+      H.lds = Y.lds_bytes;
+      H.scratch = Y.bytes;
+      nar = (int64_t)Y.lds_bytes + Y.bytes <= dp::group_above();
     }
     if (!nar && (!forced_of(opt_flags) || (opt_flags & DP_OPT_FORCE_LDSG)) && dp::ldsg_fits(h)) {
       if (opt_flags & DP_OPT_FORCE_LDSG) {
@@ -212,6 +219,7 @@
   P.scratch_words = P.core_cap = P.rec_bytes = P.other_words = 0;
   P.n_direct = 0;
   P.big_base = 0;
+  P.lds_scratch_base = P.lds_scratch_stride = P.lds_first = 0;
   Head* head = P.head.data();
   const int32_t nblk = (n + kPlanBlock - 1) / kPlanBlock;
   P.blk.resize((size_t)std::max(nblk, 1));
@@ -261,6 +269,8 @@
       if (H.place == M_LDS) {
         B.bcount[H.bucket]++;
         B.bmax[H.bucket] = std::max(B.bmax[H.bucket], H.lds);
+        B.smax = std::max(B.smax, H.scratch);
+        B.bfull[H.bucket] = std::max(B.bfull[H.bucket], H.lds + H.scratch);
       } else {
         B.nother++;
       }
@@ -273,8 +283,9 @@
     }
   });
   for (auto& v : P.big) v.clear();
-  int32_t bcount[kNBuckets] = {}, bmax[kNBuckets] = {};
+  int32_t bcount[kNBuckets] = {}, bmax[kNBuckets] = {}, bfull[kNBuckets] = {};
   int64_t img = 0, inst = 0;
+  int32_t smax = 0;
   bool others = false;
   for (int32_t b = 0; b < nblk; ++b) {
     PlanBlock& B = P.blk[(size_t)b];
@@ -288,9 +299,11 @@
     P.core_cap += B.core;
     P.rec_bytes += B.rbytes;
     others |= B.nother > 0;
+    smax = std::max(smax, B.smax);
     for (int k = 0; k < kNBuckets; ++k) {
       bcount[k] += B.bcount[k];
       bmax[k] = std::max(bmax[k], B.bmax[k]);
+      bfull[k] = std::max(bfull[k], B.bfull[k]);
     }
   }
   P.dev_off.resize((size_t)n);
@@ -371,6 +384,7 @@
   int group_of[kNBuckets];
   Launch bl[kNBuckets];
   int64_t gsize[kNBuckets] = {};
+  int32_t gfull[kNBuckets] = {};
   int ng = 0;
   for (int k = kNBuckets - 1; k >= 0; --k) {
     if (!bcount[k]) continue;
@@ -380,7 +394,13 @@
     if (!join) bl[ng++] = Launch{0, 0, M_LDS, bmax[k]};
     group_of[k] = ng - 1;
     gsize[ng - 1] += bcount[k];
-  }
+    gfull[ng - 1] = std::max(gfull[ng - 1], bfull[k]);
+  }
+  for (int g = 0; g < ng; ++g)
+    if (dp::lds_dense(gfull[g])) {
+      bl[g].dense = true;
+      bl[g].lds = gfull[g];
+    }
   int ix[kNBuckets];
   for (int g = 0; g < ng; ++g) ix[g] = g;
   std::stable_sort(ix, ix + ng, [&](int x, int y) { return gsize[x] > gsize[y]; });
@@ -392,6 +412,12 @@
     o += gsize[g];
   }
   P.order.resize((size_t)o);
+  if (ng > 0) {
+    P.lds_first = bl[ix[0]].first;
+    P.lds_scratch_stride = ((int64_t)smax + 15) / 16 * 4;
+    P.lds_scratch_base = P.scratch_words;
+    P.scratch_words += (o - P.lds_first) * P.lds_scratch_stride;
+  }
   static const int64_t xcd_order = env_i64("DEPPY_XCD_ORDER", kMaxLdsBytes);
   static const bool anchor_order = env_i64("DEPPY_ANCHOR_ORDER", 1) != 0;
   if (ng > 0) {
@@ -842,6 +868,7 @@
   hipStream_t s = nullptr;
   hipEvent_t done = nullptr;
   Buf h_in{nullptr, 0, true}, h_out{nullptr, 0, true};
+  Buf scratch;
   Plan plan;
   std::vector<uint8_t> bad;
 };
@@ -1000,6 +1027,8 @@
     }
     dp::KernelArgs a = base;
     a.items = base.items + L.first;
+    a.lds_scratch_off = P.lds_scratch_base + (L.first - P.lds_first) * P.lds_scratch_stride;
+    a.lds_scratch_stride = P.lds_scratch_stride;
     if (L.mode != dp::M_LDS) {
       a.scratch_off = base.scratch_off + (L.first - P.big_base);
       a.queue = no_queue ? nullptr : base.scratch + q;
@@ -1009,7 +1038,7 @@
       ++q;
       if (L.dev_lists) HIP_OK(dp::launch_watch_build(a, L.mode, L.count, s));
     }
-    HIP_OK(dp::launch_solve(a, L.mode, L.count, L.lds, t));
+    HIP_OK(dp::launch_solve(a, L.mode, L.count, L.lds, L.dense, t));
     if (t != s) {
       HIP_OK(hipEventRecord(sp->fin[nf], t));
       HIP_OK(hipStreamWaitEvent(s, sp->fin[nf], 0));
@@ -1385,13 +1414,16 @@
   if (hipSetDevice(D.ordinal) != hipSuccess) return 1;
   const InLayout il = in_layout(P);
   const OutLayout ol = out_layout(P);
-  if (F.h_in.reserve(il.end) != hipSuccess || F.h_out.reserve(ol.end) != hipSuccess) return 1;
+  if (F.h_in.reserve(il.end) != hipSuccess || F.h_out.reserve(ol.end) != hipSuccess ||
+      F.scratch.reserve((size_t)std::max<int64_t>(P.scratch_words, 1) * 4) != hipSuccess)
+    return 1;
   int32_t* img = at<int32_t>(F.h_in.p, il.img);
   for (int32_t i = 0; i < n; ++i)
     if (!dp::stage_one(P, b->rec, b->rec_off, 0, i, img, true)) F.bad[(size_t)i] = 1;
   fill_in_tables(P, il, F.h_in.p);
   *at<int32_t>(F.h_out.p, ol.pool_len) = 0;
-  dp::KernelArgs a = kernel_args(il, ol, F.h_in.dev, F.h_out.dev, nullptr, ctx->budget);
+  dp::KernelArgs a = kernel_args(il, ol, F.h_in.dev, F.h_out.dev, reinterpret_cast<int32_t*>(F.scratch.p),
+                                 ctx->budget);
   dp_stats st{};
   if (enqueue_launches(ctx, P, a, F.s, st) || hipEventRecord(F.done, F.s) != hipSuccess) return api_fail(ctx);
   hipError_t e;
@@ -1548,6 +1580,7 @@
     if (D.fast.s) (void)hipStreamSynchronize(D.fast.s);
     D.fast.h_in.release();
     D.fast.h_out.release();
+    D.fast.scratch.release();
     if (D.fast.done) (void)hipEventDestroy(D.fast.done);
     if (D.fast.s) (void)hipStreamDestroy(D.fast.s);
   }
@@ -1623,6 +1656,38 @@
   for (int32_t i = 0; i < b->n_problems; ++i) place[i] = (int8_t)P.head[(size_t)i].place;
   return 0;
 }
+
+int dp_plan_footprints(const dp_batch* b, int32_t opt_flags, int32_t* lds_bytes, int32_t* scratch_bytes) {
+  if (!b || !lds_bytes || !scratch_bytes || b->n_problems < 0 || (b->n_problems > 0 && (!b->rec || !b->rec_off)))
+    return -1;
+  static thread_local Plan P;
+  dp::plan_chunk(P, b->rec, b->rec_off, 0, b->n_problems, opt_flags, nullptr, &dp::host_pool());
+  for (int32_t i = 0; i < b->n_problems; ++i) {
+    const auto& H = P.head[(size_t)i];
+    const int32_t* h = b->rec + b->rec_off[i];
+    dp::Layout Y{};
+    switch (H.place) {
+      case dp::M_LDS: Y.lds_bytes = H.lds; Y.bytes = H.scratch; break;
+      case dp::M_LDSG: Y = dp::layout<dp::M_LDSG>(h); break;
+      case dp::M_SPLIT: Y = dp::layout<dp::M_SPLIT>(h); break;
+      case dp::M_SPLIT4: Y = dp::layout<dp::M_SPLIT4>(h); break;
+      case dp::M_HBM: Y = dp::layout<dp::M_HBM>(h); break;
+      default: break;
+    }
+    lds_bytes[i] = Y.lds_bytes;
+    scratch_bytes[i] = Y.bytes;
+  }
+  for (const auto& L : P.launches)
+    if (L.mode == dp::M_LDS && L.dense)
+      for (int t = L.first; t < L.first + L.count; ++t) {
+        const int32_t i = P.order[(size_t)t];
+        lds_bytes[i] += scratch_bytes[i];
+        scratch_bytes[i] = 0;
+      }
+  return 0;
+}
+
+int dp_lds_occupancy(int32_t lds_bytes, int32_t capped) { return dp::lds_occupancy(lds_bytes, capped != 0); }
 
 
 int dp_submit(dp_ctx* ctx, const dp_batch* b, dp_result* res, dp_job** out) {
diff --git a/deppy_amd/csrc/solve_kernel.hpp b/deppy_amd/csrc/solve_kernel.hpp
--- a/deppy_amd/csrc/solve_kernel.hpp
+++ b/deppy_amd/csrc/solve_kernel.hpp
@@ -126,6 +126,24 @@
     if constexpr (MODE != M_HBM) return *p;
     else return __hip_atomic_load(p, __ATOMIC_RELAXED, __HIP_MEMORY_SCOPE_AGENT);
   }
+  static constexpr bool EV = mode_evict(MODE) && MINW == 1;
+  __device__ __forceinline__ static void cd_drain() {
+    if constexpr (EV) __builtin_amdgcn_s_waitcnt(0);
+  }
+  bool cd_ready;
+  char* cdb;
+  template <class T>
+  __device__ __forceinline__ T* cd_at(int32_t off) const {
+    uint64_t x = reinterpret_cast<uint64_t>(cdb);
+    asm volatile("" : "+s"(x));
+    using gchar = __attribute__((address_space(1))) char;
+    return (T*)((gchar*)x + off);
+  }
+#define DP_CD_ARRAY(T, name)                                        \
+  __device__ __forceinline__ T* a_##name() const {                  \
+    if constexpr (EV) return cd_at<T>(cdcl_layout(nv).name);        \
+    else return name;                                               \
+  }
 
   int nv, nc, nk, nid, nrows, nbv, nbi, na, nch, ncl, nkl, nchl;
   const IX *clause_off, *clause_lits, *clause_id;
@@ -158,6 +176,10 @@
   IX *reason, *rs, *trail, *touched, *d_mark, *l_off, *l_lits, *dq, *stk;
   IMP* imp;
   uint32_t *d_flip, *inS, *extra, *seen, *model, *used, *en, *en2, *crit, *dset, *fg;
+  DP_CD_ARRAY(IX, d_mark)
+  DP_CD_ARRAY(IX, l_off)
+  DP_CD_ARRAY(IX, l_lits)
+#undef DP_CD_ARRAY
   IX *wbuf, *cardq;
   int32_t* scal;
   static constexpr bool LR = mode_lds_rounds(MODE);
@@ -305,7 +327,7 @@
 #ifdef DP_STAMPS
     const int64_t ti0 = stamp();
 #endif
-    const Layout L = layout<MODE>(h);
+    const Layout L = layout<MODE, EV>(h);
     const dp_rec_layout R = rec_layout(h);
     const ImgLayout X = img_layout(h);
     scal = reinterpret_cast<int32_t*>(lds + L.scal);
@@ -394,12 +416,13 @@
     dthr = nrows + L_MAX;
     char* hot = MODE == M_HBM ? hbm : lds;
     char* cold = N16 ? lds : hbm;
+    cdb = hbm;
     val = reinterpret_cast<int8_t*>(hot + L.val);
     reason = reinterpret_cast<IX*>(cold + L.reason);
     rs = reinterpret_cast<IX*>(cold + L.rs);
     trail = reinterpret_cast<IX*>(cold + L.trail);
     touched = reinterpret_cast<IX*>(cold + L.touched);
-    d_mark = reinterpret_cast<IX*>(cold + L.d_mark);
+    d_mark = EV ? nullptr : reinterpret_cast<IX*>(cold + L.d_mark);
     imp = reinterpret_cast<IMP*>(cold + L.imp);
     w8 = nullptr;
     d_flip = reinterpret_cast<uint32_t*>(hot + L.d_flip);
@@ -414,8 +437,8 @@
     en2 = reinterpret_cast<uint32_t*>(hot + L.en2);
     crit = reinterpret_cast<uint32_t*>(hot + L.crit);
     idt = reinterpret_cast<uint32_t*>(lds + L.idt);
-    l_off = reinterpret_cast<IX*>(cold + L.l_off);
-    l_lits = reinterpret_cast<IX*>(cold + L.l_lits);
+    l_off = EV ? nullptr : reinterpret_cast<IX*>(cold + L.l_off);
+    l_lits = EV ? nullptr : reinterpret_cast<IX*>(cold + L.l_lits);
     dq = reinterpret_cast<IX*>(cold + L.dq);
     stk = reinterpret_cast<IX*>(cold + L.stk);
     wbuf = reinterpret_cast<IX*>(lds + L.wbuf);
@@ -495,9 +518,10 @@
     }
     for (int i = tid; i < mode_nscal(MODE); i += NT) scal[i] = 0;
     if (tid == 0) {
-      l_off[0] = 0;
+      if constexpr (!EV) l_off[0] = 0;
       scal[S_POSROWS] = h[DP_H_NVU] > 0;
     }
+    cd_ready = !EV;
     gsync();
     return true;
   }
@@ -1064,7 +1088,8 @@
     }
     if (r < nc) return eval_clause(r, clause_lits, clause_off[r], clause_off[r + 1], crow);
     const int j = r - nrows;
-    return eval_clause(r, l_lits, DP_CHK((int)l_off[j], 0, lcap + 1, 33), DP_CHK((int)l_off[j + 1], 0, lcap + 1, 34), crow);
+    const IX* lo = a_l_off();
+    return eval_clause(r, a_l_lits(), DP_CHK((int)lo[j], 0, lcap + 1, 33), DP_CHK((int)lo[j + 1], 0, lcap + 1, 34), crow);
   }
 
   __device__ __forceinline__ void card_serial(int r, int& crow) {
@@ -1580,17 +1605,18 @@
   __device__ __forceinline__ void ante_serial(int r, int u, int bound) {
     r = DP_CHK(r, 0, nrows + nl, 15);
     if (r < nc || r >= nrows) {
-      const IX* lits = clause_lits;
-      int a, b;
-      if (r < nc) { a = clause_off[r]; b = clause_off[r + 1]; set_bit_atomic(used, row_key(r)); }
-      else {
-        lits = l_lits;
-        a = DP_CHK((int)l_off[r - nrows], 0, lcap + 1, 35);
-        b = DP_CHK((int)l_off[r - nrows + 1], 0, lcap + 1, 36);
-      }
-      for (int j = a; j < b; ++j) {
-        const int v = (int)lits[j] >> 1;
-        if (v != u) mark_push(v);
+      auto mark_row = [&](const IX* lits, int a, int b) {
+        for (int j = a; j < b; ++j) {
+          const int v = (int)lits[j] >> 1;
+          if (v != u) mark_push(v);
+        }
+      };
+      if (r < nc) {
+        set_bit_atomic(used, row_key(r));
+        mark_row(clause_lits, clause_off[r], clause_off[r + 1]);
+      } else {
+        const IX* lo = a_l_off();
+        mark_row(a_l_lits(), DP_CHK((int)lo[r - nrows], 0, lcap + 1, 35), DP_CHK((int)lo[r - nrows + 1], 0, lcap + 1, 36));
       }
     } else {
       const int k = r - nc;
@@ -1615,6 +1641,13 @@
   }
   __device__ __forceinline__ void analyze_() {
 #endif
+    if constexpr (EV) {
+      if (!cd_ready) {
+        if (tid == 0) a_l_off()[0] = 0;
+        cd_ready = true;
+        cd_drain();
+      }
+    }
     gsync();
     if (tid == 0) {
       scal[S_NWORK] = 0;
@@ -1747,7 +1780,7 @@
   }
 
   __device__ __forceinline__ int dlit(int i) const {
-    return (int)trail[(int)d_mark[i]] ^ (int)getb(d_flip, i);
+    return (int)trail[(int)a_d_mark()[i]] ^ (int)getb(d_flip, i);
   }
 
   __device__ __forceinline__ int dpll() {
@@ -1760,7 +1793,7 @@
         if (l < 0) { save_model(); r = RS_SAT; break; }
         if (++steps > budget) { budget_hit = true; r = RS_BUDGET; break; }
         if (tid == 0) {
-          d_mark[nd] = enc(tlen);
+          a_d_mark()[nd] = enc(tlen);
           d_flip[nd >> 5] &= ~(1u << (nd & 31));
         }
         assign_one(l, R_DEC, nd);
@@ -1769,6 +1802,7 @@
       if (propagate() >= 0) { decide = true; continue; }
       decide = false;
       clear_bits(dset, nd);
+      cd_drain();
       analyze();
       int h = -1, b = -1, n = 0;
       for (int wi = bits_words(nd) - 1; wi >= 0 && b < 0; --wi) {
@@ -1782,28 +1816,29 @@
       for (int wi = 0; wi < bits_words(nd); ++wi) n += __popc(ld_bits(&dset[wi]));
       if (h < 0) { r = RS_UNSAT; break; }
       if (++steps > budget) { budget_hit = true; r = RS_BUDGET; break; }
-      const int lat = DP_CHK((int)l_off[nl], 0, lcap + 1, 26);
+      const int lat = DP_CHK((int)a_l_off()[nl], 0, lcap + 1, 26);
       if (nl < L_MAX && lat + n <= lcap) {
         int run = lat;
         for (int base = 0; base < nd; base += NT) {
           const int i = base + tid;
           const bool in = i < nd && ((ld_bits(&dset[i >> 5]) >> (i & 31)) & 1u);
           const int at = claim(in, run);
-          if (in) l_lits[DP_CHK(at, 0, lcap, 27)] = enc(dlit(i) ^ 1);
+          if (in) a_l_lits()[DP_CHK(at, 0, lcap, 27)] = enc(dlit(i) ^ 1);
         }
         claim_end(run);
-        if (tid == 0) l_off[nl + 1] = enc(run);
+        if (tid == 0) a_l_off()[nl + 1] = enc(run);
         ++nl;
+        cd_drain();
         gsync();
         const int lh = dlit(h);
         nd = b + 1;
-        truncate_to(DP_CHK((int)d_mark[nd], 0, nv + 1, 24));
+        truncate_to(DP_CHK((int)a_d_mark()[nd], 0, nv + 1, 24));
         assign_one(lh ^ 1, nrows + nl - 1, -1);
       } else {
         while (nd > 0 && getb(d_flip, nd - 1)) --nd;
         if (nd == 0) { r = RS_UNSAT; break; }
         const int lf = dlit(nd - 1);
-        truncate_to(DP_CHK((int)d_mark[nd - 1], 0, nv + 1, 25));
+        truncate_to(DP_CHK((int)a_d_mark()[nd - 1], 0, nv + 1, 25));
         if (tid == 0) d_flip[(nd - 1) >> 5] |= 1u << ((nd - 1) & 31);
         gsync();
         assign_one(lf ^ 1, R_DEC, nd - 1);
@@ -1948,18 +1983,19 @@
       int n = 0;
       for (int wi = tid; wi < nbv; wi += NT) n += __popc(ld_bits(&fg[wi]));
       n = g_sum(n);
-      const int lat = l_off[nl];
+      const int lat = a_l_off()[nl];
       if (nl < L_MAX && lat + n <= lcap) {
         int run = lat;
         for (int b = 0; b < nv; b += NT) {
           const int v = b + tid;
           const bool in = v < nv && ((ld_bits(&fg[v >> 5]) >> (v & 31)) & 1u);
           const int at = claim(in, run);
-          if (in) l_lits[at] = enc(2 * v + 1);
+          if (in) a_l_lits()[at] = enc(2 * v + 1);
         }
         claim_end(run);
-        if (tid == 0) l_off[nl + 1] = enc(run);
+        if (tid == 0) a_l_off()[nl + 1] = enc(run);
         ++nl;
+        cd_drain();
         gsync();
       }
     }
@@ -2393,7 +2429,9 @@
   const int pid = it.pid;
   const int32_t* grec = a.rec + it.rec_off;
   Group<MODE, MINW> W;
-  char* hbm = mode_n16(MODE) ? nullptr : reinterpret_cast<char*>(a.scratch + a.scratch_off[k]);
+  char* hbm = nullptr;
+  if constexpr (Group<MODE, MINW>::EV) hbm = reinterpret_cast<char*>(a.scratch + a.lds_scratch_off + k * a.lds_scratch_stride);
+  else if constexpr (!mode_n16(MODE)) hbm = reinterpret_cast<char*>(a.scratch + a.scratch_off[k]);
   if (!W.init(reinterpret_cast<char*>(lds4), hbm, grec)) {
     if (threadIdx.x == 0) {
       put_out(a.out + pid, DP_ERROR, DP_F_MALFORMED, 0, 0, 0, 0);
@@ -2535,6 +2573,13 @@
                        (size_t)lds_bytes, stream, a);                                       \
     return hipGetLastError();                                                               \
   }                                                                                         \
+  int NAME##_occupancy(int lds_bytes) {    \
+    int per = 0;                                                                            \
+    if (hipOccupancyMaxActiveBlocksPerMultiprocessor(&per, solve_kernel<MODE, MINW>, 64 * mode_waves(MODE), \
+                                                     (size_t)lds_bytes) != hipSuccess)      \
+      return -1;                                                                            \
+    return per;                                                                             \
+  }                                                                                         \
   hipError_t NAME##_configure(int max_lds_bytes) {                                          \
     return hipFuncSetAttribute(reinterpret_cast<const void*>(&solve_kernel<MODE, MINW>),          \
                                hipFuncAttributeMaxDynamicSharedMemorySize, max_lds_bytes);  \
diff --git a/deppy_amd/csrc/solve_launch.cpp b/deppy_amd/csrc/solve_launch.cpp
--- a/deppy_amd/csrc/solve_launch.cpp
+++ b/deppy_amd/csrc/solve_launch.cpp
@@ -17,19 +17,27 @@
 hipError_t launch_split4_configure(int);
 hipError_t launch_hbm_configure(int);
 hipError_t launch_ldsg_configure(int);
+int launch_lds_occupancy(int);
+int launch_lds_dense_occupancy(int);
 
 constexpr int kUnboundedWavesPerCU = 16;
 constexpr int kLdsPerCU = 160 * 1024;
 
-hipError_t launch_solve(const KernelArgs& a, int mode, int n_blocks, int lds_bytes, hipStream_t stream) {
-  if (mode == M_LDS) {
-    static const bool no_dense = [] {
-      const char* e = std::getenv("DEPPY_NO_DENSE");
-      return e && *e && *e != '0';
-    }();
-    const bool dense = !no_dense && lds_bytes > 0 && kLdsPerCU / lds_bytes > kUnboundedWavesPerCU;
+bool lds_dense(int full_bytes) {
+  static const bool no_dense = [] {
+    const char* e = std::getenv("DEPPY_NO_DENSE");
+    return e && *e && *e != '0';
+  }();
+  return !no_dense && full_bytes > 0 && kLdsPerCU / full_bytes > kUnboundedWavesPerCU;
+}
+
+int lds_occupancy(int lds_bytes, bool dense) {
+  return dense ? launch_lds_dense_occupancy(lds_bytes) : launch_lds_occupancy(lds_bytes);
+}
+
+hipError_t launch_solve(const KernelArgs& a, int mode, int n_blocks, int lds_bytes, bool dense, hipStream_t stream) {
+  if (mode == M_LDS)
     return dense ? launch_lds_dense(a, n_blocks, lds_bytes, stream) : launch_lds(a, n_blocks, lds_bytes, stream);
-  }
   if (mode == M_SPLIT) return launch_split(a, n_blocks, lds_bytes, stream);
   if (mode == M_SPLIT4) return launch_split4(a, n_blocks, lds_bytes, stream);
   if (mode == M_LDSG) return launch_ldsg(a, n_blocks, lds_bytes, stream);
diff --git a/include/deppy_hip.h b/include/deppy_hip.h
--- a/include/deppy_hip.h
+++ b/include/deppy_hip.h
@@ -306,6 +306,8 @@
   DP_PLACE_TOO_LARGE = -2
 };
 int dp_plan_placements(const dp_batch* b, int32_t opt_flags, int8_t* place);
+int dp_plan_footprints(const dp_batch* b, int32_t opt_flags, int32_t* lds_bytes, int32_t* scratch_bytes);
+int dp_lds_occupancy(int32_t lds_bytes, int32_t capped);
 int dp_plan_order(const dp_batch* b, int32_t opt_flags, int32_t* order, int32_t* launch_first);
 
 int dp_last_kernel_ms(const dp_ctx* ctx, double* ms);
```

Result: faster. 32.60 million, median of 6 (+7.6%).
